# tensorboy/centerpose

Hardware: AMD Instinct MI355X
Metric: images/sec end-to-end (backbone+decode), DLA-34 512x512 (higher is better)
Workload: dtype f32

## Files before the change

### centerpose_amd/csrc/common.h

```cpp
#pragma once
#include <hip/hip_runtime.h>
#include <stdint.h>

#define CP_WAVE 64

extern "C" const char* cp_last_error(void);
void cp_set_error(const char* fmt, ...);
void cp_note_kernel(const char* fmt, ...);

#define CP_CHECK_ARG(cond, ...)              \
    do {                                     \
        if (!(cond)) {                       \
            cp_set_error(__VA_ARGS__);       \
            return 1;                        \
        }                                    \
    } while (0)

#define CP_CHECK_LAUNCH(name)                                                   \
    do {                                                                        \
        hipError_t e_ = hipGetLastError();                                      \
        if (e_ != hipSuccess) {                                                 \
            cp_set_error("%s: kernel launch failed: %s", name, hipGetErrorString(e_)); \
            return 2;                                                           \
        }                                                                       \
    } while (0)

typedef float f32x4 __attribute__((ext_vector_type(4)));
typedef float f32x16 __attribute__((ext_vector_type(16)));

static inline int cp_cdiv(int a, int b) { return (a + b - 1) / b; }

#include <mutex>
struct CpLdsGuard {
    std::mutex mu;
    int have[16] = {};
    hipError_t ensure(const void* kernel, int bytes) {
        int d = 0;
        (void)hipGetDevice(&d);
        std::lock_guard<std::mutex> lock(mu);
        if (have[d & 15] >= bytes) return hipSuccess;
        const hipError_t e = hipFuncSetAttribute(kernel, hipFuncAttributeMaxDynamicSharedMemorySize, bytes);
        if (e == hipSuccess) have[d & 15] = bytes;
        return e;
    }
};

static inline int cp_num_cus()
{
    static std::mutex mu;
    static int cus[16] = {};
    int d = 0;
    (void)hipGetDevice(&d);
    std::lock_guard<std::mutex> lock(mu);
    int& n = cus[d & 15];
    if (n <= 0 && (hipDeviceGetAttribute(&n, hipDeviceAttributeMultiprocessorCount, d) != hipSuccess || n <= 0)) n = 256;
    return n;
}

#define CP_ACT_NONE_ 0
#define CP_ACT_RELU_ 1
#define CP_ACT_SIGMOID_ 2
#define CP_ACT_HSWISH_ 3
#define CP_ACT_HSIGMOID_ 4
__device__ __forceinline__ float cp_relu(float v)
{
    float r;
    asm("v_max_f32 %0, 0, %1" : "=v"(r) : "v"(v));
    return r;
}
typedef float cp_v2f __attribute__((ext_vector_type(2)));
__device__ __forceinline__ float4 cp_scale_shift4(float4 v, float4 sc, float4 sh)
{
    const cp_v2f lo = __builtin_elementwise_fma((cp_v2f){v.x, v.y}, (cp_v2f){sc.x, sc.y}, (cp_v2f){sh.x, sh.y});
    const cp_v2f hi = __builtin_elementwise_fma((cp_v2f){v.z, v.w}, (cp_v2f){sc.z, sc.w}, (cp_v2f){sh.z, sh.w});
    return make_float4(lo.x, lo.y, hi.x, hi.y);
}
__device__ __forceinline__ float4 cp_relu4(float4 v) { return make_float4(cp_relu(v.x), cp_relu(v.y), cp_relu(v.z), cp_relu(v.w)); }

__device__ __forceinline__ float cp_act(float v, int act)
{
    if (act == CP_ACT_RELU_) return cp_relu(v);
    if (act == CP_ACT_SIGMOID_) return 1.0f / (1.0f + __expf(-v));
    if (act == CP_ACT_HSWISH_) return v * fminf(fmaxf(v + 3.f, 0.f), 6.f) / 6.f;
    if (act == CP_ACT_HSIGMOID_) return fminf(fmaxf(v + 3.f, 0.f), 6.f) / 6.f;
    return v;
}
```

### centerpose_amd/csrc/dcn.hip

```cpp
#include <cstdlib>
#include "igemm.h"

#define DCN_MAX_TAPS 121
typedef float dcn_v2 __attribute__((ext_vector_type(2)));

__device__ __forceinline__ void dcn_blend(dcn_v2& r, dcn_v2 wxy, dcn_v2 wzw, dcn_v2 c00, dcn_v2 c01, dcn_v2 c10, dcn_v2 c11)
{
    asm("v_pk_mul_f32 %0, %1, %2 op_sel_hi:[0,1]" : "=v"(r) : "v"(wxy), "v"(c00));
    asm("v_pk_fma_f32 %0, %1, %2, %0 op_sel:[1,0,0] op_sel_hi:[1,1,1]" : "+v"(r) : "v"(wxy), "v"(c01));
    asm("v_pk_fma_f32 %0, %1, %2, %0 op_sel_hi:[0,1,1]" : "+v"(r) : "v"(wzw), "v"(c10));
    asm("v_pk_fma_f32 %0, %1, %2, %0 op_sel:[1,0,0] op_sel_hi:[1,1,1]" : "+v"(r) : "v"(wzw), "v"(c11));
}

template <int BM, int BN, int WAVES_M, int WAVES_N, int MF>
__global__ __launch_bounds__(IG_THREADS, 3) void dcn_igemm_kernel(const ConvArgs a)
{
    using T = IgTile<BM, BN, WAVES_M, WAVES_N, MF>;
    constexpr int QL = 4;
    constexpr int PPP = IG_THREADS / QL;
    constexpr int ASL = BM / PPP;
    static_assert(ASL >= 1, "BM too small for this gather width");
    extern __shared__ __attribute__((aligned(16))) float smem[];
    const int dg = a.dg;
    const int ntap = a.kh * a.kw;
    float4* s_w = reinterpret_cast<float4*>(smem);
    int* s_code = reinterpret_cast<int*>(s_w + dg * ntap * BM);
    float* As0 = smem + dg * ntap * BM * 5;
    float* Bs0 = As0 + 2 * T::A_FLOATS;

    const int tid = threadIdx.x, lane = tid & 63, wid = tid >> 6;
    const int NT = a.ldw / BN;
    int tile = ig_xcd_remap(blockIdx.x, gridDim.x);
    const int S = a.ksplit, sp = tile % S;
    tile /= S;
    const int nt = tile % NT, mt = tile / NT;
    const int m0 = mt * BM, n0 = nt * BN;
    const int wm0 = (wid / WAVES_N) * T::WM, wn0 = (wid % WAVES_N) * T::WN;
    const int HoWo = a.Ho * a.Wo;
    const int tap0 = sp * ntap / S, tap1 = (sp + 1) * ntap / S;
    const int C = a.srcC[0], ld = a.srcLd[0];
    const float* __restrict__ x = a.src[0];

    {
        static_assert(IG_THREADS % BM == 0, "one pixel per thread");
        constexpr int TS = IG_THREADS / BM;
        const int pl = tid % BM, m = m0 + pl;
        const bool live = m < a.M;
        const int b = live ? m / HoWo : 0, p = m - b * HoWo, oy = p / a.Wo, ox = p - oy * a.Wo;
        const float* omp = a.om + (size_t)(live ? m : 0) * a.omLd;
        const int by = oy * a.sy - a.py, bx = ox * a.sx - a.px, bpix = b * a.H * a.W;
        const float fH = (float)a.H, fW = (float)a.W;
        const unsigned ld4 = (unsigned)ld >> 2;
        for (int g = 0; g < dg; ++g) {
        const int og = g * ntap;
        int t = tap0 + __builtin_amdgcn_readfirstlane(tid / BM);
        int ky = t / a.kw, kx = t - ky * a.kw;
        for (; t < tap1; t += TS) {
            const float offh = omp[2 * (og + t)], offw = omp[2 * (og + t) + 1];
            float mk = omp[a.omMaskOff + og + t];
            if (a.omSigmoid) mk = __builtin_amdgcn_rcpf(1.0f + __expf(-mk));
            const float h_im = (float)(by + ky * a.dily) + offh;
            const float w_im = (float)(bx + kx * a.dilx) + offw;
            const bool valid = live && h_im > -1.f && w_im > -1.f && h_im < fH && w_im < fW;
            const float hf = floorf(h_im), wf = floorf(w_im);
            const float lh = h_im - hf, lw = w_im - wf, hh = 1.f - lh, hw = 1.f - lw;
            const int h_low = (int)hf, w_low = (int)wf;
            const bool t_ok = h_low >= 0, b_ok = h_low < a.H - 1, l_ok = w_low >= 0, r_ok = w_low < a.W - 1;
            const bool dyb = t_ok && b_ok, dxb = l_ok && r_ok;
            const float mv = valid ? mk : 0.f;
            const float top = (t_ok ? hh : lh) * mv, bot = (dyb ? lh : 0.f) * mv;
            const float lft = l_ok ? hw : lw, rgt = dxb ? lw : 0.f;
            const int yl = min(max(h_low, 0), a.H - 1), xl = min(max(w_low, 0), a.W - 1);
            s_w[(g * ntap + t) * BM + pl] = make_float4(top * lft, top * rgt, bot * lft, bot * rgt);
            s_code[(g * ntap + t) * BM + pl] = (int)((unsigned)(bpix + yl * a.W + xl) * ld4) | ((dxb ? 1 : 0) << 29) | ((dyb ? 1 : 0) << 30);
            kx += TS;
            while (kx >= a.kw) { kx -= a.kw; ++ky; }
        }
        }
    }

    typename IgAcc<MF>::type acc[T::TM][T::TN];
#pragma unroll
    for (int i = 0; i < T::TM; ++i)
#pragma unroll
        for (int j = 0; j < T::TN; ++j)
#pragma unroll
            for (int r = 0; r < IgAcc<MF>::N; ++r) acc[i][j][r] = 0.f;

    const int ks0 = tap0 * (C / IG_BK), nk = tap1 * (C / IG_BK);
    const int q = tid % QL;
    float4 br[T::B_SLOTS];
    float4 c00[ASL], c01[ASL], c10[ASL], c11[ASL], wq[ASL];
    int tap = tap0, cl = 0;
    const int cpg = C / dg;
    int gnext = 0, grec = 0;
    __syncthreads();

    const unsigned pixb = (unsigned)ld * 4u, rowb = (unsigned)a.W * pixb;
    unsigned o00[ASL], o01[ASL], o10[ASL], o11[ASL];
    auto load_a = [&]() __attribute__((always_inline)) {
        if (cl == gnext) {
            grec = (cl == 0 ? 0 : grec + ntap);
            gnext = cl + cpg;
#pragma unroll
            for (int s = 0; s < ASL; ++s) {
                const int pl = tid / QL + s * PPP;
                const int code = s_code[(grec + tap) * BM + pl];
                wq[s] = s_w[(grec + tap) * BM + pl];
                o00[s] = (((unsigned)code & 0x0FFFFFFFu) << 4) + (unsigned)q * 16u;
                o01[s] = o00[s] + (((unsigned)code >> 29) & 1u) * pixb;
                o10[s] = o00[s] + (((unsigned)code >> 30) & 1u) * rowb;
                o11[s] = o10[s] + (o01[s] - o00[s]);
            }
        }
        const char* xs = reinterpret_cast<const char*>(x) + (size_t)cl * 4;
#pragma unroll
        for (int s = 0; s < ASL; ++s) {
            c00[s] = ig_ldg4(reinterpret_cast<const float*>(xs + o00[s]));
            c01[s] = ig_ldg4(reinterpret_cast<const float*>(xs + o01[s]));
            c10[s] = ig_ldg4(reinterpret_cast<const float*>(xs + o10[s]));
            c11[s] = ig_ldg4(reinterpret_cast<const float*>(xs + o11[s]));
        }
    };
    auto advance = [&]() __attribute__((always_inline)) { cl += IG_BK; if (cl >= C) { cl = 0; gnext = 0; ++tap; } };
    auto store_a = [&](float* As) __attribute__((always_inline)) {
#pragma unroll
        for (int s = 0; s < ASL; ++s) {
            const int pl = tid / QL + s * PPP;
            const float4 w = wq[s];
            const dcn_v2 wxy = {w.x, w.y}, wzw = {w.z, w.w};
            dcn_v2 lo, hi;
            dcn_blend(lo, wxy, wzw, (dcn_v2){c00[s].x, c00[s].y}, (dcn_v2){c01[s].x, c01[s].y}, (dcn_v2){c10[s].x, c10[s].y}, (dcn_v2){c11[s].x, c11[s].y});
            dcn_blend(hi, wxy, wzw, (dcn_v2){c00[s].z, c00[s].w}, (dcn_v2){c01[s].z, c01[s].w}, (dcn_v2){c10[s].z, c10[s].w}, (dcn_v2){c11[s].z, c11[s].w});
            *reinterpret_cast<float4*>(As + pl * IG_LDK + q * 4) = make_float4(lo.x, lo.y, hi.x, hi.y);
        }
    };

    unsigned boff[T::B_SLOTS];
#pragma unroll
    for (int s = 0; s < T::B_SLOTS; ++s) {
        const int idx = tid + s * IG_THREADS;
        boff[s] = ((unsigned)(n0 + (idx >> 2)) * (unsigned)a.K + (unsigned)(idx & 3) * 4u) * 4u;
    }
    auto load_b = [&](int ks) __attribute__((always_inline)) {
        const char* wb = reinterpret_cast<const char*>(a.w) + (size_t)ks * (IG_BK * 4);
#pragma unroll
        for (int s = 0; s < T::B_SLOTS; ++s)
            if (T::B_F4 % IG_THREADS == 0 || tid + s * IG_THREADS < T::B_F4) br[s] = ig_ldg4(reinterpret_cast<const float*>(wb + boff[s]));
    };
    load_a(); advance();
    load_b(ks0);
    store_a(As0);
    ig_store_b<T>(Bs0, tid, br);
    __syncthreads();
    int cur = 0;
    for (int ks = ks0; ks < nk; ++ks) {
        const bool more = ks + 1 < nk;
        ig_compute<T, MF>(As0 + cur * T::A_FLOATS, Bs0 + cur * T::B_FLOATS, wm0, wn0, lane, acc, [&]() __attribute__((always_inline)) {
            if (more) { load_a(); advance(); load_b(ks + 1); }
        });
        __builtin_amdgcn_sched_barrier(0);
        if (more) {
            store_a(As0 + (cur ^ 1) * T::A_FLOATS);
            ig_store_b<T>(Bs0 + (cur ^ 1) * T::B_FLOATS, tid, br);
        }
        __syncthreads();
        cur ^= 1;
    }
    if (S > 1) {
        ConvArgs e = a;
        e.out = a.out + (size_t)sp * a.M * a.outLd;
        ig_epilogue<T, BM, BN, MF>(e, smem, m0, n0, wm0, wn0, lane, tid, acc);
    } else ig_epilogue<T, BM, BN, MF>(a, smem, m0, n0, wm0, wn0, lane, tid, acc);
}


template <int BM, int BN, int WAVES_M, int WAVES_N, int MF>
static int launch_dcn(const ConvArgs& a, hipStream_t s)
{
    using T = IgTile<BM, BN, WAVES_M, WAVES_N, MF>;
    auto kern = dcn_igemm_kernel<BM, BN, WAVES_M, WAVES_N, MF>;
    if (a.srcC[0] % IG_BK != 0) { cp_set_error("dcn: C=%d is not a multiple of %d", a.srcC[0], IG_BK); return 1; }
    if (a.ldw % BN != 0) { cp_set_error("dcn: ldw=%d is not a multiple of the N tile %d", a.ldw, BN); return 1; }
    if ((a.srcC[0] / a.dg) % IG_BK != 0) { cp_set_error("dcn: C / deformable_group = %d is not a multiple of %d", a.srcC[0] / a.dg, IG_BK); return 1; }
    const int main_bytes = T::MAIN_BYTES + a.dg * a.kh * a.kw * BM * 20;
    if (main_bytes > 160 * 1024) { cp_set_error("dcn: %d x %d taps x %d deformable group(s) need %d B of LDS for the sampling records", a.kh, a.kw, a.dg, main_bytes); return 1; }
    const int epi = a.outNCHW ? T::EPI_BYTES : T::EPV_BYTES;
    const int smem = epi > main_bytes ? epi : main_bytes;
    static CpLdsGuard guard;
    if (smem > 64 * 1024) {
        const hipError_t e = guard.ensure((const void*)kern, smem);
        if (e != hipSuccess) { cp_set_error("dcn_v2: cannot reserve %d B LDS: %s", smem, hipGetErrorString(e)); return 2; }
    }
    const int grid = cp_cdiv(a.M, BM) * (a.ldw / BN) * a.ksplit;
    hipLaunchKernelGGL(kern, dim3(grid), dim3(IG_THREADS), smem, s, a);
    cp_note_kernel("dcn_igemm_kernel<%d, %d, %d, %d, %d>", BM, BN, WAVES_M, WAVES_N, MF);
    return 0;
}

struct cp_dcn_desc {
    int B, H, W, C, srcLd;
    int Ho, Wo;
    int kh, kw, sy, sx, py, px, dily, dilx;
    int K, ldw, Cout;
    int omLd, omSigmoid;
    int outLd, outNCHW, act;
    int tile;
    int ksplit;
    int dg;
};

extern "C" int cp_sizeof_dcn_desc(void) { return (int)sizeof(cp_dcn_desc); }

extern "C" int cp_dcn_v2_f32(const cp_dcn_desc* d, const float* x, const float* om, const float* w, const float* scale,
                             const float* shift, float* out, void* stream)
{
    CP_CHECK_ARG(d && x && om && w && scale && shift && out, "dcn_v2: null pointer");
    CP_CHECK_ARG(d->kh > 0 && d->kw > 0 && d->kh * d->kw <= DCN_MAX_TAPS, "dcn_v2: 1..%d taps (kh=%d kw=%d)", DCN_MAX_TAPS, d->kh, d->kw);
    CP_CHECK_ARG(d->sy > 0 && d->sx > 0 && d->dily > 0 && d->dilx > 0 && d->py >= 0 && d->px >= 0, "dcn_v2: stride / dilation > 0, pad >= 0");
    CP_CHECK_ARG(d->C % 16 == 0 && d->srcLd % 4 == 0 && d->srcLd >= d->C, "dcn_v2: C%%16==0, ld%%4==0 required");
    CP_CHECK_ARG(d->K == d->kh * d->kw * d->C, "dcn_v2: K=%d != kh*kw*C", d->K);
    CP_CHECK_ARG(d->ldw % 16 == 0 && d->ldw >= d->Cout, "dcn_v2: ldw=%d Cout=%d", d->ldw, d->Cout);
    const int dgv = d->dg > 1 ? d->dg : 1;
    CP_CHECK_ARG(d->C % dgv == 0 && (d->C / dgv) % 16 == 0, "dcn_v2: C=%d must split into %d deformable groups of a multiple of 16 channels", d->C, dgv);
    CP_CHECK_ARG(d->omLd >= 3 * dgv * d->kh * d->kw, "dcn_v2: omLd=%d too small", d->omLd);
    CP_CHECK_ARG((long long)d->B * d->H * d->W < (1ll << 29) && (long long)d->B * d->H * d->W * d->srcLd * 4 < (1ll << 32),
                 "dcn_v2: input too large (pixel index 29 bits, byte offsets 32 bits)");
    ConvArgs a;
    for (int i = 0; i < IG_MAX_SRC; ++i) { a.src[i] = nullptr; a.srcC[i] = 0; a.srcLd[i] = 0; }
    a.src[0] = x; a.srcC[0] = d->C; a.srcLd[0] = d->srcLd; a.nsrc = 1; a.Ctot = d->C;
    a.B = d->B; a.H = d->H; a.W = d->W; a.Ho = d->Ho; a.Wo = d->Wo; a.M = d->B * d->Ho * d->Wo;
    a.kh = d->kh; a.kw = d->kw; a.sy = d->sy; a.sx = d->sx; a.py = d->py; a.px = d->px;
    a.K = d->K; a.w = w; a.ldw = d->ldw; a.scale = scale; a.shift = shift; a.res = nullptr; a.resLd = 0;
    a.out = out; a.outLd = d->outLd; a.Cout = d->Cout; a.outNCHW = d->outNCHW;
    a.OH = d->Ho; a.OW = d->Wo; a.osy = a.osx = 1; a.ooy = a.oox = 0; a.act = d->act;
    a.om = om; a.omLd = d->omLd; a.omMaskOff = 2 * dgv * d->kh * d->kw; a.omSigmoid = d->omSigmoid; a.dg = dgv;
    a.dily = d->dily; a.dilx = d->dilx; a.nsub = 1;
    a.ksplit = d->ksplit > 1 ? d->ksplit : 1;
    CP_CHECK_ARG(a.ksplit <= d->kh * d->kw, "dcn_v2: ksplit=%d exceeds the %d taps", a.ksplit, d->kh * d->kw);
    CP_CHECK_ARG(a.ksplit == 1 || (!d->outNCHW && d->act == CP_ACT_NONE && d->outLd == d->ldw && d->Cout == d->ldw),
                 "dcn_v2: split-K writes raw NHWC partial sums (outLd == Cout == ldw, no activation)");
    hipStream_t s = (hipStream_t)stream;
    int tile = d->tile;
    if (tile == 0) {
        static const int force = getenv("CP_DCN_TILE") ? atoi(getenv("CP_DCN_TILE")) : 0;
        if (force && a.ksplit == 1) tile = force;
    }
    if (tile == 0) {
        if (d->ldw % 64 != 0) tile = (d->ldw % 32 == 0) ? 128032 : 0;
        else {
            tile = 64064;
            if (d->ldw % 128 == 0 && (long long)cp_cdiv(a.M, 64) * (d->ldw / 128) >= 500) tile = 64128;

        }
    }
    int rc = 0;
    switch (tile) {
        case 128032: rc = launch_dcn<128, 32, 4, 1, 32>(a, s); break;
        case 128064: rc = launch_dcn<128, 64, 2, 2, 32>(a, s); break;
        case 64064: rc = launch_dcn<64, 64, 2, 2, 32>(a, s); break;
        case 64032: rc = launch_dcn<64, 32, 4, 1, 16>(a, s); break;
        case 64128: rc = launch_dcn<64, 128, 2, 2, 32>(a, s); break;
        case 6064128: rc = (d->ldw % 128 == 0) ? launch_dcn<64, 128, 2, 2, 32>(a, s) : launch_dcn<64, 64, 2, 2, 32>(a, s); break;
        default: CP_CHECK_ARG(false, "dcn_v2: unsupported tile %d (ldw=%d)", tile, d->ldw);
    }
    if (rc) return rc;
    CP_CHECK_LAUNCH("dcn_igemm_kernel");
    return 0;
}
```

### centerpose_amd/csrc/elementwise.hip

```cpp
#include <cstdlib>
#include "common.h"

#define EW_THREADS 256
static inline int ew_grid(long long n) { long long g = (n + EW_THREADS - 1) / EW_THREADS; return (int)(g > 8192 ? 8192 : (g < 1 ? 1 : g)); }

struct EwRow { int rows, rowElems, C4; unsigned mC4; };
static inline EwRow ew_row(int rows, int Wo, int C4)
{
    EwRow r; r.rows = rows; r.rowElems = Wo * C4; r.C4 = C4;
    r.mC4 = C4 <= 1 ? 0u : (unsigned)(((1ull << 32) + (unsigned)C4 - 1) / (unsigned)C4);
    return r;
}
static inline dim3 ew_row_grid(const EwRow& r)
{
    return dim3((unsigned)((r.rowElems + EW_THREADS - 1) / EW_THREADS), (unsigned)(r.rows > 65535 ? 65535 : r.rows));
}
__device__ __forceinline__ void ew_split(const EwRow& r, int e, int& x, int& c4)
{
    x = r.C4 == 1 ? e : (int)__umulhi((unsigned)e, r.mC4);
    c4 = e - x * r.C4;
}

__global__ void maxpool_nhwc_kernel(const float* __restrict__ in, int inLd, float* __restrict__ out, int outLd, EwRow r,
                                    int H, int W, int Ho, int Wo, int k, int s, int p)
{
    const int e = blockIdx.x * EW_THREADS + threadIdx.x;
    if (e >= r.rowElems) return;
    int ox, c4;
    ew_split(r, e, ox, c4);
    for (int row = blockIdx.y; row < r.rows; row += gridDim.y) {
        const int b = row / Ho, oy = row - b * Ho;
        float4 m = make_float4(-INFINITY, -INFINITY, -INFINITY, -INFINITY);
        for (int ky = 0; ky < k; ++ky) {
            const int iy = oy * s - p + ky;
            if (iy < 0 || iy >= H) continue;
            for (int kx = 0; kx < k; ++kx) {
                const int ix = ox * s - p + kx;
                if (ix < 0 || ix >= W) continue;
                const float4 v = *reinterpret_cast<const float4*>(in + ((size_t)(b * H + iy) * W + ix) * inLd + c4 * 4);
                m.x = fmaxf(m.x, v.x); m.y = fmaxf(m.y, v.y); m.z = fmaxf(m.z, v.z); m.w = fmaxf(m.w, v.w);
            }
        }
        *reinterpret_cast<float4*>(out + ((size_t)row * Wo + ox) * outLd + c4 * 4) = m;
    }
}

extern "C" int cp_maxpool2d_nhwc_f32(const float* in, int inLd, float* out, int outLd, int B, int H, int W, int C, int k,
                                     int s, int p, void* stream)
{
    CP_CHECK_ARG(in && out && C % 4 == 0 && inLd % 4 == 0 && outLd % 4 == 0, "maxpool: C, ld must be multiples of 4");
    const int Ho = (H + 2 * p - k) / s + 1, Wo = (W + 2 * p - k) / s + 1;
    CP_CHECK_ARG((long long)Wo * (C / 4) * (C / 4) < (1ll << 32) && (long long)B * Ho < (1ll << 31), "maxpool: row too large");
    const EwRow r = ew_row(B * Ho, Wo, C / 4);
    hipLaunchKernelGGL(maxpool_nhwc_kernel, ew_row_grid(r), dim3(EW_THREADS), 0, (hipStream_t)stream, in, inLd, out, outLd, r,
                       H, W, Ho, Wo, k, s, p);
    cp_note_kernel("maxpool_nhwc_kernel");
    CP_CHECK_LAUNCH("maxpool_nhwc_kernel");
    return 0;
}

__global__ void dw_deconv_add_kernel(const float* __restrict__ in, int inLd, const float* __restrict__ w,
                                     const float* add, int addLd, float* out, int outLd, EwRow r,
                                     int H, int W, int f, int p)
{
    const int k = 2 * f, Ho = H * f, Wo = W * f, C = r.C4 * 4;
    const int e = blockIdx.x * EW_THREADS + threadIdx.x;
    if (e >= r.rowElems) return;
    int ox, c4;
    ew_split(r, e, ox, c4);
    const int rx = (ox + p) % f;
    for (int row = blockIdx.y; row < r.rows; row += gridDim.y) {
        const int b = row / Ho, oy = row - b * Ho;
        float4 acc = make_float4(0.f, 0.f, 0.f, 0.f);
        const int ry = (oy + p) % f;
#pragma unroll
        for (int ty = 0; ty < 2; ++ty) {
            const int ky = ry + ty * f, iy = (oy + p - ky) / f;
            if (oy + p - ky < 0 || iy >= H) continue;
#pragma unroll
            for (int tx = 0; tx < 2; ++tx) {
                const int kx = rx + tx * f, ix = (ox + p - kx) / f;
                if (ox + p - kx < 0 || ix >= W) continue;
                const float4 v = *reinterpret_cast<const float4*>(in + ((size_t)(b * H + iy) * W + ix) * inLd + c4 * 4);
                const float4 ww = *reinterpret_cast<const float4*>(w + (size_t)(ky * k + kx) * C + c4 * 4);
                acc.x += v.x * ww.x; acc.y += v.y * ww.y; acc.z += v.z * ww.z; acc.w += v.w * ww.w;
            }
        }
        const size_t opix = (size_t)row * Wo + ox;
        if (add) {
            const float4 rr = *reinterpret_cast<const float4*>(add + opix * addLd + c4 * 4);
            acc.x += rr.x; acc.y += rr.y; acc.z += rr.z; acc.w += rr.w;
        }
        *reinterpret_cast<float4*>(out + opix * outLd + c4 * 4) = acc;
    }
}

__global__ __launch_bounds__(EW_THREADS) void dw_deconv2_add_kernel(const float* __restrict__ in, int inLd, const float* __restrict__ w,
                                                                   const float* add, int addLd, float* out,
                                                                   int outLd, EwRow r, int H, int W)
{
    const int C = r.C4 * 4, Wo = 2 * W;
    const int e = blockIdx.x * EW_THREADS + threadIdx.x;
    if (e >= r.rowElems) return;
    int ix, c4;
    ew_split(r, e, ix, c4);
    float4 wt[16];
#pragma unroll
    for (int t = 0; t < 16; ++t) wt[t] = *reinterpret_cast<const float4*>(w + (size_t)t * C + c4 * 4);
    const bool lok = ix > 0, rok = ix + 1 < W;
    const float4 z = make_float4(0.f, 0.f, 0.f, 0.f);
    for (int row = blockIdx.y; row < r.rows; row += gridDim.y) {
        const int b = row / H, iy = row - b * H;
        const float* base = in + ((size_t)row * W + ix) * inLd + c4 * 4;
        const bool tok = iy > 0, bok = iy + 1 < H;
        const size_t rs = (size_t)W * inLd;
        float4 v[3][3];
#pragma unroll
        for (int dy = -1; dy <= 1; ++dy) {
            const bool yok = dy == 0 || (dy < 0 ? tok : bok);
#pragma unroll
            for (int dx = -1; dx <= 1; ++dx) {
                const bool ok = yok && (dx == 0 || (dx < 0 ? lok : rok));
                v[dy + 1][dx + 1] = ok ? *reinterpret_cast<const float4*>(base + dy * (long long)rs + dx * inLd) : z;
            }
        }
#pragma unroll
        for (int a = 0; a < 2; ++a)
#pragma unroll
            for (int bq = 0; bq < 2; ++bq) {
                float4 acc = z;
#pragma unroll
                for (int ty = 0; ty < 2; ++ty) {
                    const int ky = (a == 0 ? 1 : 0) + 2 * ty, dy = a == 0 ? -ty : 1 - ty;
#pragma unroll
                    for (int tx = 0; tx < 2; ++tx) {
                        const int kx = (bq == 0 ? 1 : 0) + 2 * tx, dx = bq == 0 ? -tx : 1 - tx;
                        const float4 vv = v[dy + 1][dx + 1], ww = wt[ky * 4 + kx];
                        acc.x += vv.x * ww.x; acc.y += vv.y * ww.y; acc.z += vv.z * ww.z; acc.w += vv.w * ww.w;
                    }
                }
                const size_t opix = ((size_t)(b * 2 * H + 2 * iy + a)) * Wo + 2 * ix + bq;
                if (add) {
                    const float4 rr = *reinterpret_cast<const float4*>(add + opix * addLd + c4 * 4);
                    acc.x += rr.x; acc.y += rr.y; acc.z += rr.z; acc.w += rr.w;
                }
                *reinterpret_cast<float4*>(out + opix * outLd + c4 * 4) = acc;
            }
    }
}

extern "C" int cp_dw_deconv_add_nhwc_f32(const float* in, int inLd, const float* w, const float* add, int addLd, float* out,
                                         int outLd, int B, int H, int W, int C, int f, void* stream)
{
    CP_CHECK_ARG(in && w && out && C % 4 == 0 && inLd % 4 == 0 && outLd % 4 == 0 && (!add || addLd % 4 == 0),
                 "dw_deconv_add: C, ld must be multiples of 4");
    CP_CHECK_ARG(f >= 1, "dw_deconv_add: f=%d", f);
    CP_CHECK_ARG((long long)W * f * (C / 4) * (C / 4) < (1ll << 32) && (long long)B * H * f < (1ll << 31), "dw_deconv_add: row too large");
    const char* sw = getenv("CP_DWDECONV2");
    if (f == 2 && !(sw && sw[0] == '0') && (long long)W * (C / 4) * (C / 4) < (1ll << 32)) {
        const EwRow r2 = ew_row(B * H, W, C / 4);
        hipLaunchKernelGGL(dw_deconv2_add_kernel, ew_row_grid(r2), dim3(EW_THREADS), 0, (hipStream_t)stream, in, inLd, w, add, addLd, out,
                           outLd, r2, H, W);
        cp_note_kernel("dw_deconv2_add_kernel");
        CP_CHECK_LAUNCH("dw_deconv2_add_kernel");
        return 0;
    }
    const EwRow r = ew_row(B * H * f, W * f, C / 4);
    hipLaunchKernelGGL(dw_deconv_add_kernel, ew_row_grid(r), dim3(EW_THREADS), 0, (hipStream_t)stream, in, inLd, w, add,
                       addLd, out, outLd, r, H, W, f, f / 2);
    cp_note_kernel("dw_deconv_add_kernel");
    CP_CHECK_LAUNCH("dw_deconv_add_kernel");
    return 0;
}

__global__ void splitk_reduce_kernel(const float* __restrict__ ws, int S, long long slice, int ldw4, const float* __restrict__ scale,
                                     const float* __restrict__ shift, int act, float* __restrict__ out, int outLd, int Cout, long long total4)
{
    const long long i = (long long)blockIdx.x * EW_THREADS + threadIdx.x;
    if (i >= total4) return;
    const long long m = i / ldw4;
    const int n = (int)(i - m * ldw4) * 4;
    if (n >= Cout) return;
    float4 acc = *reinterpret_cast<const float4*>(ws + i * 4);
    for (int s = 1; s < S; ++s) {
        const float4 v = *reinterpret_cast<const float4*>(ws + (size_t)s * slice + i * 4);
        acc.x += v.x; acc.y += v.y; acc.z += v.z; acc.w += v.w;
    }
    const float4 sc = *reinterpret_cast<const float4*>(scale + n), sh = *reinterpret_cast<const float4*>(shift + n);
    acc.x = cp_act(acc.x * sc.x + sh.x, act); acc.y = cp_act(acc.y * sc.y + sh.y, act);
    acc.z = cp_act(acc.z * sc.z + sh.z, act); acc.w = cp_act(acc.w * sc.w + sh.w, act);
    *reinterpret_cast<float4*>(out + (size_t)m * outLd + n) = acc;
}

extern "C" int cp_splitk_reduce_f32(const float* ws, int splits, int M, int ldw, const float* scale, const float* shift, int act, float* out,
                                    int outLd, int Cout, void* stream)
{
    CP_CHECK_ARG(ws && scale && shift && out && splits >= 1 && M > 0, "splitk_reduce: bad arguments");
    CP_CHECK_ARG(ldw % 4 == 0 && Cout % 4 == 0 && outLd % 4 == 0 && Cout <= ldw && Cout <= outLd, "splitk_reduce: ldw, Cout, outLd must be multiples of 4 (ldw=%d Cout=%d outLd=%d)", ldw, Cout, outLd);
    const long long total4 = (long long)M * (ldw / 4);
    hipLaunchKernelGGL(splitk_reduce_kernel, dim3((unsigned)((total4 + EW_THREADS - 1) / EW_THREADS)), dim3(EW_THREADS), 0, (hipStream_t)stream,
                       ws, splits, (long long)M * ldw, ldw / 4, scale, shift, act, out, outLd, Cout, total4);
    cp_note_kernel("splitk_reduce_kernel");
    CP_CHECK_LAUNCH("splitk_reduce_kernel");
    return 0;
}

struct SumUpArgs { const float* src[4]; int ld[4]; int sh[4]; int n; };
__global__ void sum_up_kernel(SumUpArgs a, float* __restrict__ out, int outLd, EwRow r, int H, int W, int relu)
{
    const int e = blockIdx.x * EW_THREADS + threadIdx.x;
    if (e >= r.rowElems) return;
    int x, c4;
    ew_split(r, e, x, c4);
    for (int row = blockIdx.y; row < r.rows; row += gridDim.y) {
        const int b = row / H, y = row - b * H;
        float4 acc = make_float4(0.f, 0.f, 0.f, 0.f);
        for (int j = 0; j < a.n; ++j) {
            const int sh = a.sh[j], hs = H >> sh, ws = W >> sh;
            const float4 v = *reinterpret_cast<const float4*>(a.src[j] + ((size_t)(b * hs + (y >> sh)) * ws + (x >> sh)) * a.ld[j] + c4 * 4);
            if (j == 0) acc = v;
            else { acc.x += v.x; acc.y += v.y; acc.z += v.z; acc.w += v.w; }
        }
        if (relu) { acc.x = fmaxf(acc.x, 0.f); acc.y = fmaxf(acc.y, 0.f); acc.z = fmaxf(acc.z, 0.f); acc.w = fmaxf(acc.w, 0.f); }
        *reinterpret_cast<float4*>(out + ((size_t)row * W + x) * outLd + c4 * 4) = acc;
    }
}

extern "C" int cp_sum_up_nhwc_f32(int n, const float* const* src, const int* ld, const int* shift, float* out, int outLd,
                                  int B, int H, int W, int C, int relu, void* stream)
{
    CP_CHECK_ARG(n >= 1 && n <= 4 && src && ld && shift && out && C % 4 == 0, "sum_up: bad arguments");
    SumUpArgs a;
    for (int i = 0; i < 4; ++i) { a.src[i] = i < n ? src[i] : nullptr; a.ld[i] = i < n ? ld[i] : 0; a.sh[i] = i < n ? shift[i] : 0; }
    a.n = n;
    CP_CHECK_ARG((long long)W * (C / 4) * (C / 4) < (1ll << 32) && (long long)B * H < (1ll << 31), "sum_up: row too large");
    const EwRow r = ew_row(B * H, W, C / 4);
    hipLaunchKernelGGL(sum_up_kernel, ew_row_grid(r), dim3(EW_THREADS), 0, (hipStream_t)stream, a, out, outLd, r, H, W, relu);
    cp_note_kernel("sum_up_kernel");
    CP_CHECK_LAUNCH("sum_up_kernel");
    return 0;
}

struct SumUpMember { SumUpArgs a; float* out; int outLd; EwRow r; int H, W, xblocks; };
struct SumUpGroup { SumUpMember m[4]; int first[5]; int n, relu; };
__global__ void sum_up_group_kernel(const SumUpGroup g)
{
    int t = blockIdx.x, k = 0;
    while (k + 1 < g.n && t >= g.first[k + 1]) ++k;
    const SumUpMember& m = g.m[k];
    t -= g.first[k];
    const int row = t / m.xblocks, e = (t - row * m.xblocks) * EW_THREADS + threadIdx.x;
    if (e >= m.r.rowElems) return;
    int x, c4;
    ew_split(m.r, e, x, c4);
    const int H = m.H, W = m.W;
    const int b = row / H, y = row - b * H;
    float4 acc = make_float4(0.f, 0.f, 0.f, 0.f);
    for (int j = 0; j < m.a.n; ++j) {
        const int sh = m.a.sh[j], hs = H >> sh, ws = W >> sh;
        const float4 v = *reinterpret_cast<const float4*>(m.a.src[j] + ((size_t)(b * hs + (y >> sh)) * ws + (x >> sh)) * m.a.ld[j] + c4 * 4);
        if (j == 0) acc = v;
        else { acc.x += v.x; acc.y += v.y; acc.z += v.z; acc.w += v.w; }
    }
    if (g.relu) { acc.x = fmaxf(acc.x, 0.f); acc.y = fmaxf(acc.y, 0.f); acc.z = fmaxf(acc.z, 0.f); acc.w = fmaxf(acc.w, 0.f); }
    *reinterpret_cast<float4*>(m.out + ((size_t)row * W + x) * m.outLd + c4 * 4) = acc;
}

extern "C" int cp_sum_up_group_nhwc_f32(int n, const float* const* src, const int* meta, float* const* out, int relu, void* stream)
{
    CP_CHECK_ARG(n >= 1 && n <= 4 && src && meta && out, "sum_up_group: 1..4 members (got %d)", n);
    SumUpGroup g;
    g.n = n; g.relu = relu;
    long long total = 0;
    for (int k = 0; k < 4; ++k) {
        const int kk = k < n ? k : 0;
        const int* mt = meta + 14 * kk;
        SumUpMember& m = g.m[k];
        const int ns = mt[0], B = mt[10], H = mt[11], W = mt[12], C = mt[13];
        if (k < n) {
            CP_CHECK_ARG(ns >= 1 && ns <= 4 && out[k] && C > 0 && C % 4 == 0 && mt[9] % 4 == 0, "sum_up_group: member %d: bad arguments", k);
            CP_CHECK_ARG((long long)W * (C / 4) * (C / 4) < (1ll << 32) && (long long)B * H < (1ll << 31), "sum_up_group: member %d: row too large", k);
        }
        for (int i = 0; i < 4; ++i) {
            m.a.src[i] = i < ns ? src[4 * kk + i] : nullptr; m.a.ld[i] = i < ns ? mt[1 + i] : 0; m.a.sh[i] = i < ns ? mt[5 + i] : 0;
            if (k < n && i < ns) CP_CHECK_ARG(m.a.src[i] && m.a.ld[i] % 4 == 0, "sum_up_group: member %d source %d", k, i);
        }
        m.a.n = ns;
        m.out = out[kk]; m.outLd = mt[9]; m.H = H; m.W = W;
        m.r = ew_row(B * H, W, C / 4);
        m.xblocks = (m.r.rowElems + EW_THREADS - 1) / EW_THREADS;
        g.first[k] = (int)total;
        if (k < n) total += (long long)m.r.rows * m.xblocks;
    }
    g.first[4] = (int)total;
    for (int k = n; k < 4; ++k) g.first[k] = (int)total;
    CP_CHECK_ARG(total > 0 && total < (1ll << 31), "sum_up_group: grid %lld", total);
    hipLaunchKernelGGL(sum_up_group_kernel, dim3((unsigned)total), dim3(EW_THREADS), 0, (hipStream_t)stream, g);
    cp_note_kernel("sum_up_group_kernel");
    CP_CHECK_LAUNCH("sum_up_group_kernel");
    return 0;
}

__global__ void nchw_to_nhwc_kernel(const float* __restrict__ in, float* __restrict__ out, int C, int HW, int outLd, int cOff)
{
    __shared__ float t[32][33];
    const int b = blockIdx.z, c0 = blockIdx.y * 32, p0 = blockIdx.x * 32;
    const int tx = threadIdx.x & 31, ty = threadIdx.x >> 5;
    for (int r = ty; r < 32; r += 8) {
        const int c = c0 + r, p = p0 + tx;
        t[r][tx] = (c < C && p < HW) ? in[((size_t)b * C + c) * HW + p] : 0.f;
    }
    __syncthreads();
    for (int r = ty; r < 32; r += 8) {
        const int p = p0 + r, c = c0 + tx;
        if (c < C && p < HW) out[((size_t)b * HW + p) * outLd + cOff + c] = t[tx][r];
    }
}
__global__ void nhwc_to_nchw_kernel(const float* __restrict__ in, int inLd, int cOff, float* __restrict__ out, int C, int HW)
{
    __shared__ float t[32][33];
    const int b = blockIdx.z, c0 = blockIdx.y * 32, p0 = blockIdx.x * 32;
    const int tx = threadIdx.x & 31, ty = threadIdx.x >> 5;
    for (int r = ty; r < 32; r += 8) {
        const int p = p0 + r, c = c0 + tx;
        t[r][tx] = (c < C && p < HW) ? in[((size_t)b * HW + p) * inLd + cOff + c] : 0.f;
    }
    __syncthreads();
    for (int r = ty; r < 32; r += 8) {
        const int c = c0 + r, p = p0 + tx;
        if (c < C && p < HW) out[((size_t)b * C + c) * HW + p] = t[tx][r];
    }
}

extern "C" int cp_nchw_to_nhwc_f32(const float* in, float* out, int B, int C, int H, int W, int outLd, int cOff, void* stream)
{
    CP_CHECK_ARG(in && out && outLd >= cOff + C, "nchw_to_nhwc: bad arguments");
    const int HW = H * W;
    hipLaunchKernelGGL(nchw_to_nhwc_kernel, dim3(cp_cdiv(HW, 32), cp_cdiv(C, 32), B), dim3(256), 0, (hipStream_t)stream, in, out,
                       C, HW, outLd, cOff);
    CP_CHECK_LAUNCH("nchw_to_nhwc_kernel");
    return 0;
}
extern "C" int cp_nhwc_to_nchw_f32(const float* in, int inLd, int cOff, float* out, int B, int C, int H, int W, void* stream)
{
// ... 213 lines not shown
```

### centerpose_amd/csrc/igemm.h

```cpp
#pragma once
#include "common.h"

#define IG_BK 16
#define IG_LDK 20
#define IG_THREADS 256
#define IG_MAX_SRC 4

enum { CP_ACT_NONE = 0, CP_ACT_RELU = 1, CP_ACT_SIGMOID = 2 };

struct ConvArgs {
    const float* src[IG_MAX_SRC];
    int srcC[IG_MAX_SRC];
    int srcLd[IG_MAX_SRC];
    int nsrc, Ctot;
    int B, H, W;
    int Ho, Wo, M;
    int kh, kw, sy, sx, py, px;
    int K;
    const float* w;
    int ldw;
    const float* scale;
    const float* shift;
    const float* res;
    int resLd;
    float* out;
    int outLd;
    int Cout;
    int outNCHW;
    int OH, OW;
    int osy, osx, ooy, oox;
    int act;
    const float* om;
    int omLd;
    int omMaskOff;
    int omSigmoid;
    int dily, dilx;
    int ksplit;
    int dg;
    int nsub;
};

int cp_launch_conv3x3_patch(const ConvArgs& a, int in_nchw, hipStream_t s, int variant = 0);
int cp_launch_stem3x3(const ConvArgs& a, hipStream_t s);
int cp_launch_conv3x3_c16(const ConvArgs& a, int in_nchw, hipStream_t s);
int cp_launch_conv3x3_wino(const ConvArgs& a, hipStream_t s, int variant = 0);
int cp_launch_conv3x3_wino24_group(const ConvArgs* a, int n, hipStream_t s);
int cp_launch_head3x3_1x1_w24(const ConvArgs& a, const float* w2, const float* b2, float* out2, int n2, int ld2, int act2, hipStream_t s);
int cp_launch_conv3x3_wino24(const ConvArgs& a, hipStream_t s);
int cp_launch_head3x3_1x1(const ConvArgs& a, const float* w2, const float* b2, float* out2, int n2, int ld2, int act2, hipStream_t s);

int cp_launch_conv_pointwise(const ConvArgs& a, hipStream_t s);
int cp_launch_conv_bf16x3(const ConvArgs& a, int tile, hipStream_t s);

typedef float ig_v4f __attribute__((ext_vector_type(4)));
__device__ __forceinline__ float4 ig_ldg4(const float* p)
{
    const ig_v4f v = *(const __attribute__((address_space(1))) ig_v4f*)(p);
    return make_float4(v.x, v.y, v.z, v.w);
}

__device__ __forceinline__ int ig_xcd_remap(int id, int n)
{
    const int q = n >> 3, r = n & 7, x = id & 7, j = id >> 3;
    return (x < r ? x * (q + 1) : r * (q + 1) + (x - r) * q) + j;
}

template <int MF> struct IgAcc;
template <> struct IgAcc<32> { typedef f32x16 type; static constexpr int N = 16; };
template <> struct IgAcc<16> { typedef f32x4 type; static constexpr int N = 4; };

template <int MF>
__device__ __forceinline__ typename IgAcc<MF>::type ig_mfma(float a, float b, typename IgAcc<MF>::type c)
{
    if constexpr (MF == 32) return __builtin_amdgcn_mfma_f32_32x32x2f32(a, b, c, 0, 0, 0);
    else return __builtin_amdgcn_mfma_f32_16x16x4f32(a, b, c, 0, 0, 0);
}

template <int MF> __device__ __forceinline__ int ig_row(int r, int lane)
{
    if constexpr (MF == 32) return (r & 3) + 8 * (r >> 2) + 4 * (lane >> 5);
    else return (lane >> 4) * 4 + r;
}

template <int BM, int BN, int WAVES_M, int WAVES_N, int MF>
struct IgTile {
    static constexpr int WM = BM / WAVES_M, WN = BN / WAVES_N;
    static constexpr int TM = WM / MF, TN = WN / MF;
    static constexpr int A_SLOTS = BM * 4 / IG_THREADS;
    static constexpr int B_F4 = BN * 4;
    static constexpr int B_SLOTS = (B_F4 + IG_THREADS - 1) / IG_THREADS;
    static constexpr int A_FLOATS = BM * IG_LDK, B_FLOATS = BN * IG_LDK;
    static constexpr int MAIN_BYTES = 2 * (A_FLOATS + B_FLOATS) * 4;
    static constexpr int EPI_BYTES = BN * (BM + 1) * 4;
    static constexpr int EPV_BYTES = BM * (BN + 4) * 4;
    static constexpr int NHWC_BYTES = MAIN_BYTES > EPV_BYTES ? MAIN_BYTES : EPV_BYTES;
    static constexpr int SMEM = MAIN_BYTES > EPI_BYTES ? MAIN_BYTES : EPI_BYTES;
    static_assert(WAVES_M * WAVES_N * 64 == IG_THREADS, "4 waves");
    static_assert(TM >= 1 && TN >= 1, "tile");
    static_assert(A_SLOTS >= 1, "BM >= 64");
};

template <class T>
__device__ __forceinline__ void ig_load_b(const ConvArgs& a, int k0, int n0, int tid, float4 (&br)[T::B_SLOTS], const float* w = nullptr)
{
    if (!w) w = a.w;
#pragma unroll
    for (int s = 0; s < T::B_SLOTS; ++s) {
        const int idx = tid + s * IG_THREADS;
        if constexpr (T::B_F4 % IG_THREADS == 0) br[s] = ig_ldg4(w + (size_t)(n0 + (idx >> 2)) * a.K + k0 + (idx & 3) * 4);
        else if (idx < T::B_F4) br[s] = ig_ldg4(w + (size_t)(n0 + (idx >> 2)) * a.K + k0 + (idx & 3) * 4);
    }
}
template <class T>
__device__ __forceinline__ void ig_store_b(float* Bs, int tid, const float4 (&br)[T::B_SLOTS])
{
#pragma unroll
    for (int s = 0; s < T::B_SLOTS; ++s) {
        const int idx = tid + s * IG_THREADS;
        if (T::B_F4 % IG_THREADS == 0 || idx < T::B_F4) *reinterpret_cast<float4*>(Bs + (idx >> 2) * IG_LDK + (idx & 3) * 4) = br[s];
    }
}

template <class T, int MF, class F>
__device__ __forceinline__ void ig_compute(const float* As, const float* Bs, int wm0, int wn0, int lane,
                                           typename IgAcc<MF>::type (&acc)[T::TM][T::TN], F&& mid)
{
    constexpr int G = 64 / MF;
    constexpr int NH = IG_BK / (4 * G);
    const int g = lane / MF, il = lane % MF;
    float4 af[NH][T::TM], bf[NH][T::TN];
#pragma unroll
    for (int h = 0; h < NH; ++h) {
#pragma unroll
        for (int i = 0; i < T::TM; ++i)
            af[h][i] = *reinterpret_cast<const float4*>(As + (wm0 + i * MF + il) * IG_LDK + h * 4 * G + g * 4);
#pragma unroll
        for (int j = 0; j < T::TN; ++j)
            bf[h][j] = *reinterpret_cast<const float4*>(Bs + (wn0 + j * MF + il) * IG_LDK + h * 4 * G + g * 4);
    }
    constexpr int HALF = NH * T::TM * T::TN / 2;
    __builtin_amdgcn_sched_barrier(0);
#pragma unroll
    for (int h = 0; h < NH; ++h) {
#pragma unroll
        for (int i = 0; i < T::TM; ++i)
#pragma unroll
            for (int j = 0; j < T::TN; ++j) {
                if ((h * T::TM + i) * T::TN + j == HALF) {
                    __builtin_amdgcn_sched_barrier(0);
                    mid();
                    __builtin_amdgcn_sched_barrier(0);
                }
                acc[i][j] = ig_mfma<MF>(af[h][i].x, bf[h][j].x, acc[i][j]);
                acc[i][j] = ig_mfma<MF>(af[h][i].y, bf[h][j].y, acc[i][j]);
                acc[i][j] = ig_mfma<MF>(af[h][i].z, bf[h][j].z, acc[i][j]);
                acc[i][j] = ig_mfma<MF>(af[h][i].w, bf[h][j].w, acc[i][j]);
            }
    }
}

template <class T, int MF>
__device__ __forceinline__ void ig_compute(const float* As, const float* Bs, int wm0, int wn0, int lane,
                                           typename IgAcc<MF>::type (&acc)[T::TM][T::TN])
{
    ig_compute<T, MF>(As, Bs, wm0, wn0, lane, acc, [] {});
}

__device__ __forceinline__ float ig_act(float v, int act) { return cp_act(v, act); }

template <class T, int BM, int BN, int MF>
__device__ __forceinline__ void ig_epilogue(const ConvArgs& a, float* smem, int m0, int n0, int wm0, int wn0,
                                            int lane, int tid, typename IgAcc<MF>::type (&acc)[T::TM][T::TN],
                                            int ooy_add = 0, int oox_add = 0)
{
    const int HoWo = a.Ho * a.Wo;
    const int ooy = a.ooy + ooy_add, oox = a.oox + oox_add;
    const int cl = lane & (MF - 1);
    const bool vec_ok = !a.outNCHW && ((a.outLd | a.Cout) & 3) == 0 && (((size_t)a.out) & 15) == 0 &&
                        (!a.res || ((a.resLd & 3) == 0 && (((size_t)a.res) & 15) == 0));
    if (vec_ok) {
        const bool dense = (a.osy == 1 && a.osx == 1 && ooy == 0 && oox == 0 && a.OH == a.Ho && a.OW == a.Wo);
        const bool relu = a.act == CP_ACT_RELU, sigm = a.act == CP_ACT_SIGMOID;
        float* Cs = smem;
        constexpr int LDC = BN + 4;
        __syncthreads();
#pragma unroll
        for (int i = 0; i < T::TM; ++i)
#pragma unroll
            for (int j = 0; j < T::TN; ++j)
#pragma unroll
                for (int r = 0; r < IgAcc<MF>::N; ++r)
                    Cs[(wm0 + i * MF + ig_row<MF>(r, lane)) * LDC + wn0 + j * MF + cl] = acc[i][j][r];
// ... 83 lines not shown
```

### centerpose_amd/csrc/plan_runtime.cpp

```cpp
#include <cstdio>
#include <cstring>
#include <memory>
#include <string>
#include <vector>
#include "common.h"

extern "C" {
struct cp_conv_desc;
struct cp_dcn_desc;
int cp_abi_version(void);
int cp_conv2d_f32(const cp_conv_desc*, const float* const*, const float*, const float*, const float*, const float*, float*, void*);
int cp_conv3x3_winograd_f32(const cp_conv_desc*, const float*, const float*, const float*, const float*, const float*, float*, void*);
int cp_dcn_v2_f32(const cp_dcn_desc*, const float*, const float*, const float*, const float*, const float*, float*, void*);
int cp_conv3x3_winograd24_group_f32(const cp_conv_desc*, int, const float* const*, const float* const*, const float* const*, const float* const*,
                                    const float* const*, float* const*, void*);
int cp_conv2d_group_f32(const cp_conv_desc*, int, const float* const*, const float* const*, const float* const*, const float* const*,
                        const float* const*, float* const*, void*);
int cp_stem7x7_f32(const float*, const float*, const float*, const float*, float*, int, int, int, int, int, int, int, void*);
int cp_maxpool2d_nhwc_f32(const float*, int, float*, int, int, int, int, int, int, int, int, void*);
int cp_dw_deconv_add_nhwc_f32(const float*, int, const float*, const float*, int, float*, int, int, int, int, int, int, void*);
int cp_sum_up_nhwc_f32(int, const float* const*, const int*, const int*, float*, int, int, int, int, int, int, void*);
int cp_sum_up_group_nhwc_f32(int, const float* const*, const int*, float* const*, int, void*);
int cp_head3x3_1x1_f32(const cp_conv_desc*, const float*, const float*, const float*, const float*, const float*, const float*, float*, int,
                       int, int, void*);
int cp_dwconv2d_nhwc_f32(const float*, int, const float*, const float*, const float*, float*, int, int, int, int, int, int, int, int, int, void*);
int cp_global_avgpool_nhwc_f32(const float*, int, float*, int, int, int, int, void*);
int cp_scale_add_nhwc_f32(const float*, int, const float*, int, const float*, int, float*, int, int, int, int, int, void*);
int cp_shuffle_concat_nhwc_f32(const float*, int, const float*, int, float*, int, long long, int, int, void*);
int cp_multi_pose_decode_f32(const float*, const float*, const float*, const float*, const float*, const float*, int, int, int, int,
                             int, int, float*, float*, int*, void*);
int cp_splitk_reduce_f32(const float*, int, int, int, const float*, const float*, int, float*, int, int, void*);
int cp_sizeof_conv_desc(void);
int cp_sizeof_dcn_desc(void);
int cp_decode_topk_f32(const float*, const float*, int, int, int, int, int, int, float*, int*, void*);
int cp_decode_assign_f32(const float*, const float*, const float*, const float*, const float*, const int*, int, int, int, int, int, float*,
                         void*);
int cp_head_points_f32(const float*, int, const int*, const float*, const float*, const float*, const float*, float*, int, int, int, int, int,
                       int, int, void*);
int cp_flip_merge_pairs_f32(int, const float* const*, float* const*, const int*, int, int, int, int, const int*, void*);
}

namespace {

enum { FN_CONV = 1, FN_WINO = 2, FN_DCN = 3, FN_STEM7 = 4, FN_POOL = 5, FN_UPADD = 6, FN_SUMUP = 7, FN_DWCONV = 8, FN_AVGPOOL = 9,
       FN_SCALEADD = 10, FN_SHUFFLE = 11, FN_HEAD = 12, FN_TOPK = 13, FN_ASSIGN = 14, FN_SPLITK = 15, FN_WINO24G = 16, FN_CONVG = 17, FN_SUMUPG = 18,
       FN_POINTS = 19, FN_FLIPPAIRS = 20 };
enum { REF_NULL = 0, REF_BUF = 1, REF_CONST = 2 };

struct Op {
    uint32_t fn = 0, out_index = 0, stream = 0;
    std::vector<unsigned char> desc;
    std::vector<float*> ptrs;
    std::vector<int> bufid;
    std::vector<int> ints;
};

struct Out { float* p; int shape[4]; int bufid; };

struct ConstPool {
    std::vector<float*> p;
    ~ConstPool() { for (float* q : p) if (q) (void)hipFree(q); }
};

}

struct cp_plan {
    int B = 0, H = 0, W = 0;
    std::vector<float*> bufs;
    std::vector<uint64_t> buf_numel;
    std::shared_ptr<ConstPool> cpool;
    float* input = nullptr;
    int input_buf = -1;
    std::vector<Out> outs;
    std::vector<Op> ops;
    bool use_graph = false, warmed = false;
    hipGraph_t graph = nullptr;
    hipGraphExec_t exec = nullptr;
    hipStream_t cap_stream = nullptr, side_stream = nullptr;
    float* ws_scores = nullptr;
    int* ws_inds = nullptr;
    int ws_K = 0;
};

namespace {

struct Reader {
    const unsigned char* b;
    size_t n, p = 0;
    bool ok = true;
    bool take(void* dst, size_t k) {
        if (p + k > n) { ok = false; return false; }
        memcpy(dst, b + p, k);
        p += k;
        return true;
    }
    uint32_t u32() { uint32_t v = 0; take(&v, 4); return v; }
    uint64_t u64() { uint64_t v = 0; take(&v, 8); return v; }
    void skip_pad8() { p += (8 - (p & 7)) & 7; }
};

struct Ref { uint32_t kind, id; uint64_t off, numel; };

int run_op(const Op& o, hipStream_t s)
{
    const std::vector<float*>& P = o.ptrs;
    const int* I = o.ints.data();
    switch (o.fn) {
        case FN_CONV:
            return cp_conv2d_f32(reinterpret_cast<const cp_conv_desc*>(o.desc.data()), reinterpret_cast<const float* const*>(P.data()), P[4],
                                 P[5], P[6], P[7], P[8], s);
        case FN_WINO:
            return cp_conv3x3_winograd_f32(reinterpret_cast<const cp_conv_desc*>(o.desc.data()), P[0], P[1], P[2], P[3], P[4], P[5], s);
        case FN_DCN:
            return cp_dcn_v2_f32(reinterpret_cast<const cp_dcn_desc*>(o.desc.data()), P[0], P[1], P[2], P[3], P[4], P[5], s);
        case FN_WINO24G:
            return cp_conv3x3_winograd24_group_f32(reinterpret_cast<const cp_conv_desc*>(o.desc.data()), I[0], reinterpret_cast<const float* const*>(P.data()),
                                                   reinterpret_cast<const float* const*>(P.data() + 4), reinterpret_cast<const float* const*>(P.data() + 8),
                                                   reinterpret_cast<const float* const*>(P.data() + 12), reinterpret_cast<const float* const*>(P.data() + 16),
                                                   reinterpret_cast<float* const*>(P.data() + 20), s);
        case FN_CONVG:
            return cp_conv2d_group_f32(reinterpret_cast<const cp_conv_desc*>(o.desc.data()), I[0], reinterpret_cast<const float* const*>(P.data()),
                                       reinterpret_cast<const float* const*>(P.data() + 8), reinterpret_cast<const float* const*>(P.data() + 16),
                                       reinterpret_cast<const float* const*>(P.data() + 24), reinterpret_cast<const float* const*>(P.data() + 32),
                                       reinterpret_cast<float* const*>(P.data() + 40), s);
        case FN_STEM7:
            return cp_stem7x7_f32(P[0], P[1], P[2], P[3], P[4], I[0], I[1], I[2], I[3], I[4], I[5], I[6], s);
        case FN_POOL:
            return cp_maxpool2d_nhwc_f32(P[0], I[0], P[1], I[1], I[2], I[3], I[4], I[5], I[6], I[7], I[8], s);
        case FN_UPADD:
            return cp_dw_deconv_add_nhwc_f32(P[0], I[0], P[1], P[2], I[1], P[3], I[2], I[3], I[4], I[5], I[6], I[7], s);
        case FN_SUMUP:
            return cp_sum_up_nhwc_f32(I[0], reinterpret_cast<const float* const*>(P.data()), I + 1, I + 5, P[4], I[9], I[10], I[11], I[12],
                                      I[13], I[14], s);
        case FN_SUMUPG:
            return cp_sum_up_group_nhwc_f32(I[0], reinterpret_cast<const float* const*>(P.data()), I + 2, reinterpret_cast<float* const*>(P.data() + 16), I[1], s);
        case FN_HEAD:
            return cp_head3x3_1x1_f32(reinterpret_cast<const cp_conv_desc*>(o.desc.data()), P[0], P[1], P[2], P[3], P[4], P[5], P[6], I[0], I[1],
                                      I[2], s);
        case FN_DWCONV:
            return cp_dwconv2d_nhwc_f32(P[0], I[0], P[1], P[2], P[3], P[4], I[1], I[2], I[3], I[4], I[5], I[6], I[7], I[8], I[9], s);
        case FN_AVGPOOL:
            return cp_global_avgpool_nhwc_f32(P[0], I[0], P[1], I[1], I[2], I[3], I[4], s);
        case FN_SCALEADD:
            return cp_scale_add_nhwc_f32(P[0], I[0], P[1], I[1], P[2], I[2], P[3], I[3], I[4], I[5], I[6], I[7], s);
        case FN_SHUFFLE:
            return cp_shuffle_concat_nhwc_f32(P[0], I[0], P[1], I[1], P[2], I[2], (long long)I[3], I[4], I[5], s);
        case FN_SPLITK:
            return cp_splitk_reduce_f32(P[0], I[0], I[1], I[2], P[1], P[2], I[3], P[3], I[4], I[5], s);
        case FN_TOPK:
            return cp_decode_topk_f32(P[0], P[1], I[0], I[1], I[2], I[3], I[4], I[5], P[2], reinterpret_cast<int*>(P[3]), s);
        case FN_ASSIGN:
            return cp_decode_assign_f32(P[0], P[1], P[2], P[3], P[4], reinterpret_cast<const int*>(P[5]), I[0], I[1], I[2], I[3], I[4], P[6], s);
        case FN_POINTS:
            return cp_head_points_f32(P[0], I[0], reinterpret_cast<const int*>(P[1]), P[2], P[3], P[4], P[5], P[6], I[1], I[2], I[3], I[4], I[5],
                                      I[6], I[7], s);
        case FN_FLIPPAIRS:
            return cp_flip_merge_pairs_f32(I[0], reinterpret_cast<const float* const*>(P.data()), reinterpret_cast<float* const*>(P.data() + 4), I + 5,
                                           I[1], I[2], I[3], I[4], reinterpret_cast<const int*>(P[8]), s);
    }
    cp_set_error("plan: unknown launch function %u", o.fn);
    return 1;
}

bool arity_ok(const Op& o)
{
    switch (o.fn) {
        case FN_CONV: return o.ptrs.size() == 9 && (int)o.desc.size() == cp_sizeof_conv_desc();
        case FN_WINO: return o.ptrs.size() == 6 && (int)o.desc.size() == cp_sizeof_conv_desc();
        case FN_DCN: return o.ptrs.size() == 6 && (int)o.desc.size() == cp_sizeof_dcn_desc();
        case FN_WINO24G: return o.ptrs.size() == 25 && o.ints.size() == 1 && o.ints[0] >= 1 && o.ints[0] <= 4 && (int)o.desc.size() == 4 * cp_sizeof_conv_desc();
        case FN_CONVG: return o.ptrs.size() == 49 && o.ints.size() == 1 && o.ints[0] >= 1 && o.ints[0] <= 8 && (int)o.desc.size() == 8 * cp_sizeof_conv_desc();
        case FN_STEM7: return o.ptrs.size() == 5 && o.ints.size() == 7;
        case FN_POOL: return o.ptrs.size() == 2 && o.ints.size() == 9;
        case FN_UPADD: return o.ptrs.size() == 4 && o.ints.size() == 8;
        case FN_SUMUP: return o.ptrs.size() == 5 && o.ints.size() == 15;
        case FN_SUMUPG: return o.ptrs.size() == 21 && o.ints.size() == 58 && o.ints[0] >= 1 && o.ints[0] <= 4;
        case FN_HEAD: return o.ptrs.size() == 7 && o.ints.size() == 3 && (int)o.desc.size() == cp_sizeof_conv_desc();
        case FN_DWCONV: return o.ptrs.size() == 5 && o.ints.size() == 10;
        case FN_AVGPOOL: return o.ptrs.size() == 2 && o.ints.size() == 5;
        case FN_SCALEADD: return o.ptrs.size() == 4 && o.ints.size() == 8;
        case FN_SHUFFLE: return o.ptrs.size() == 3 && o.ints.size() == 6;
        case FN_SPLITK: return o.ptrs.size() == 4 && o.ints.size() == 6;
        case FN_TOPK: return o.ptrs.size() == 4 && o.ints.size() == 6;
        case FN_ASSIGN: return o.ptrs.size() == 7 && o.ints.size() == 5;
        case FN_POINTS: return o.ptrs.size() == 7 && o.ints.size() == 8;
        case FN_FLIPPAIRS: return o.ptrs.size() == 10 && o.ints.size() == 13 && o.ints[0] >= 1 && o.ints[0] <= 4;
    }
    return false;
}

int run_all(cp_plan* pl, hipStream_t s)
{
    for (const Op& o : pl->ops)
        if (int rc = run_op(o, s)) return rc;
    return 0;
}

struct SchedOp { const Op* op; int stream; int buf_base; };

int run_schedule(const std::vector<SchedOp>& ops, size_t nb, hipStream_t main, hipStream_t side, std::vector<hipEvent_t>& ev)
{
    const size_t n = ops.size();
    std::vector<int> last_writer(nb, -1);
    std::vector<std::vector<int>> readers(nb);
    hipStream_t st[2] = {main, side};
    int waited[2] = {-1, -1}, tail[2] = {-1, -1};
    ev.assign(n + 1, nullptr);
    if (hipEventCreateWithFlags(&ev[n], hipEventDisableTiming) != hipSuccess || hipEventRecord(ev[n], main) != hipSuccess ||
        hipStreamWaitEvent(side, ev[n], 0) != hipSuccess) { cp_set_error("plan: fork of the side stream failed"); return 2; }
    for (size_t i = 0; i < n; ++i) {
        const Op& o = *ops[i].op;
        const int me = ops[i].stream ? 1 : 0, other = me ^ 1, base = ops[i].buf_base;
        int need = -1;
        auto follow = [&](int j) { if (j >= 0 && (ops[j].stream ? 1 : 0) == other && j > need) need = j; };
        for (size_t k = 0; k < o.ptrs.size(); ++k) {
            if (o.bufid[k] < 0) continue;
            const int b = base + o.bufid[k];
            follow(last_writer[b]);
            if (k == o.out_index) for (int j : readers[b]) follow(j);
        }
        if (need > waited[me]) {
            if (hipStreamWaitEvent(st[me], ev[need], 0) != hipSuccess) { cp_set_error("plan: event wait failed"); return 2; }
            waited[me] = need;
        }
        if (int rc = run_op(o, st[me])) return rc;
        if (hipEventCreateWithFlags(&ev[i], hipEventDisableTiming) != hipSuccess || hipEventRecord(ev[i], st[me]) != hipSuccess) {
            cp_set_error("plan: event record failed");
            return 2;
        }
        tail[me] = (int)i;
        for (size_t k = 0; k < o.ptrs.size(); ++k) {
            if (o.bufid[k] < 0) continue;
            const int b = base + o.bufid[k];
            if (k == o.out_index) { last_writer[b] = (int)i; readers[b].clear(); }
            else readers[b].push_back((int)i);
        }
    }
    if (tail[1] >= 0 && hipStreamWaitEvent(main, ev[tail[1]], 0) != hipSuccess) { cp_set_error("plan: join of the side stream failed"); return 2; }
    return 0;
}

int run_two_streams(cp_plan* pl, hipStream_t main, hipStream_t side, std::vector<hipEvent_t>& ev)
{
    std::vector<SchedOp> ops;
    for (const Op& o : pl->ops) ops.push_back(SchedOp{&o, (int)o.stream, 0});
    return run_schedule(ops, pl->bufs.size(), main, side, ev);
}

void free_plan(cp_plan* pl)
{
    if (!pl) return;
    if (pl->exec) (void)hipGraphExecDestroy(pl->exec);
    if (pl->graph) (void)hipGraphDestroy(pl->graph);
    if (pl->cap_stream) (void)hipStreamDestroy(pl->cap_stream);
    if (pl->side_stream) (void)hipStreamDestroy(pl->side_stream);
    for (float* p : pl->bufs) if (p) (void)hipFree(p);
    pl->cpool.reset();
    if (pl->ws_scores) (void)hipFree(pl->ws_scores);
    if (pl->ws_inds) (void)hipFree(pl->ws_inds);
    delete pl;
}

#define PLAN_FAIL(...)            \
    do {                          \
        cp_set_error(__VA_ARGS__); \
        free_plan(pl);            \
        return 1;                 \
    } while (0)

}

extern "C" uint32_t cp_fnv1a32(const void* data, size_t bytes)
{
    uint32_t h = 2166136261u;
    const unsigned char* p = static_cast<const unsigned char*>(data);
    for (size_t i = 0; i < bytes; ++i) { h ^= p[i]; h *= 16777619u; }
    return h;
}

extern "C" int cp_plan_create(const void* blob, size_t bytes, int use_graph, cp_plan** out)
{
    CP_CHECK_ARG(blob && out, "plan_create: null pointer");
    *out = nullptr;
    Reader r{static_cast<const unsigned char*>(blob), bytes};
    const bool v4 = bytes >= 48 && memcmp(blob, "CPPLAN04", 8) == 0;
    CP_CHECK_ARG(bytes >= 48 && (v4 || memcmp(blob, "CPPLAN03", 8) == 0 || memcmp(blob, "CPPLAN02", 8) == 0),
                 "plan_create: not a centerpose_amd plan (bad magic)");
    r.p = 8;
    const uint32_t abi = r.u32(), B = r.u32(), H = r.u32(), W = r.u32(), nbuf = r.u32(), nconst = r.u32(), nops = r.u32(),
                   nout = r.u32(), mlen = r.u32();
    const uint32_t want_sum = r.u32();
    if (v4) {
        const uint32_t h = cp_fnv1a32(static_cast<const unsigned char*>(blob) + 48, bytes - 48);
        CP_CHECK_ARG(h == want_sum, "plan_create: checksum mismatch (file %08x, computed %08x): truncated or corrupted plan", want_sum, h);
    }
    CP_CHECK_ARG((int)abi == cp_abi_version(), "plan_create: plan was written for ABI %u, library has %d", abi, cp_abi_version());
    CP_CHECK_ARG(nbuf < (1u << 20) && nconst < (1u << 20) && nops < (1u << 20) && nout <= 64 && mlen < bytes,
                 "plan_create: corrupt header");
    r.p += mlen;
    r.skip_pad8();
    cp_plan* pl = new cp_plan();
    pl->B = (int)B; pl->H = (int)H; pl->W = (int)W;
    pl->use_graph = use_graph != 0;
    std::vector<uint64_t>& buf_numel = pl->buf_numel;
    buf_numel.resize(nbuf);
    for (uint32_t i = 0; i < nbuf; ++i) buf_numel[i] = r.u64();
    struct CI { uint64_t numel, off; };
    std::vector<CI> ci(nconst);
    for (uint32_t i = 0; i < nconst; ++i) { ci[i].numel = r.u64(); ci[i].off = r.u64(); }
    if (!r.ok) PLAN_FAIL("plan_create: truncated file (tables)");
    for (uint32_t i = 0; i < nconst; ++i)
        if (ci[i].off > bytes || ci[i].numel * 4 > bytes - ci[i].off) PLAN_FAIL("plan_create: constant %u lies outside the file", i);
    pl->bufs.assign(nbuf, nullptr);
    pl->cpool = std::make_shared<ConstPool>();
    std::vector<float*>& consts = pl->cpool->p;
    consts.assign(nconst, nullptr);
    for (uint32_t i = 0; i < nbuf; ++i) {
        if (hipMalloc((void**)&pl->bufs[i], buf_numel[i] * 4 + 16) != hipSuccess) PLAN_FAIL("plan_create: hipMalloc of %llu floats failed", (unsigned long long)buf_numel[i]);
        (void)hipMemset(pl->bufs[i], 0, buf_numel[i] * 4);
    }
    for (uint32_t i = 0; i < nconst; ++i) {
        if (hipMalloc((void**)&consts[i], ci[i].numel * 4 + 16) != hipSuccess) PLAN_FAIL("plan_create: hipMalloc (constant) failed");
// ... 313 lines not shown
```

### centerpose_amd/engine.py

```python
import os
import warnings
import weakref

import torch

from . import _lib, nets, ops
from .nets import Act


DECODE_TOPK = "decode.nms_topk"
SPARSE_HEADS = ("wh", "hps", "reg", "hp_offset")
FLIP_PEAKS = "flip.merge_peaks"
FLIP_IDX = ((1, 2), (3, 4), (5, 6), (7, 8), (9, 10), (11, 12), (13, 14), (15, 16))


def normalize_state_dict(sd, arch=None):
    out = {}
    for k, v in sd.items():
        if k.startswith("module") and not k.startswith("module_list"):
            k = k[7:]
        out[nets.internal_key(arch, k) if arch is not None else k] = v
    return out


class BufferPool:

    def __init__(self, device, clock=lambda: 0):
        self.device = device
        self.reuse = os.environ.get("CP_BUFFER_REUSE", "1") != "0"
        self.min_age = int(os.environ.get("CP_BUFFER_MIN_AGE", "12"))
        self.clock = clock
        self.free = []
        self.bytes = 0
        self.bytes_requested = 0

    def take(self, numel):
        self.bytes_requested += numel * 4
        if self.reuse:
            now, best = self.clock(), None
            for i, (t, slot) in enumerate(self.free):
                if now - t >= self.min_age and numel <= slot.numel() <= 2 * numel and \
                        (best is None or slot.numel() < self.free[best][1].numel()):
                    best = i
            if best is not None:
                return self.free.pop(best)[1]
        self.bytes += numel * 4
        return torch.empty((numel,), dtype=torch.float32, device=self.device)

    def give(self, slot):
        if self.reuse:
            self.free.append((self.clock(), slot))


class PlanBuilder(nets.Graph):
    def __init__(self, sd, B, device, sigmoid_heads=True, const_cache=None, dets_only=False):
        super().__init__()
        self.dets_only = dets_only
        self.points = None
        self.sd, self.B, self.dev = sd, B, device
        self.const_cache = const_cache if const_cache is not None else {}
        self.pool = BufferPool(device, lambda: len(self.launches))
        if isinstance(sigmoid_heads, bool):
            sigmoid_heads = ("hm", "hm_hp") if sigmoid_heads else ()
        self.sigmoid_heads = tuple(sigmoid_heads)
        self.launches = []
        self.winograd = os.environ.get("CP_WINOGRAD", "1") != "0"
        self.dcn_splitk = os.environ.get("CP_DCN_SPLITK", "1") != "0"
        self.wino_splitc = os.environ.get("CP_WINO_SPLITC", "1") != "0"
        self.conv_splitk = os.environ.get("CP_CONV_SPLITK", "1") != "0"
        self.fuse_heads = os.environ.get("CP_FUSE_HEADS", "1") != "0"
        self._pool_cache = {}
        self.outputs = None

    @property
    def bytes_alloc(self):
        return self.pool.bytes

    def buf(self, H, W, C, split=None):
        Cp = 2 * split[1] if split else ops.round_up(C, 16)
        slot = self.pool.take(self.B * H * W * Cp)
        act = Act(H, W, C, slot[: self.B * H * W * Cp].view(self.B, H, W, Cp), split)
        weakref.finalize(act, self.pool.give, slot)
        return act

    @staticmethod
    def cmap(a):
        if a.split:
            h, hp = a.split
            return list(range(h)) + list(range(hp, hp + h))
        return list(range(a.C))

    def expand_in(self, w, xs):
        if all(a.t.shape[3] == a.C and not a.split for a in xs):
            return w
        out = torch.zeros((w.shape[0], sum(a.t.shape[3] for a in xs)) + tuple(w.shape[2:]), dtype=w.dtype, device=w.device)
        lo = po = 0
        for a in xs:
            idx = torch.tensor(self.cmap(a), device=w.device) + po
            out[:, idx] = w[:, lo:lo + a.C]
            lo, po = lo + a.C, po + a.t.shape[3]
        return out

    def expand_vec(self, v, a, fill=0.0):
        out = torch.full((a.t.shape[3],), fill, dtype=torch.float32, device=v.device)
        out[torch.tensor(self.cmap(a), device=v.device)] = v.float()
        return out

    @staticmethod
    def act_code(relu):
        return {False: ops.ACT_NONE, None: ops.ACT_NONE, True: ops.ACT_RELU, "relu": ops.ACT_RELU, "hswish": ops.ACT_HSWISH,
                "hsigmoid": ops.ACT_HSIGMOID}[relu]

    def w(self, key):
        hit = self.const_cache.get(("w", key))
        if hit is None:
            hit = self.const_cache[("w", key)] = self.sd[key].to(self.dev, torch.float32)
        return hit

    def bn(self, name):
        return tuple(self.w("%s.%s" % (name, s)) for s in ("weight", "bias", "running_mean", "running_var"))

    def wino(self, wp, cin, cout, k=3, stride=1, pad=1, nsrc=1, key=None, hw=None):
        if self.winograd and hw is not None and ops.wino_eligible(cin, k, stride, pad, nsrc) and \
                ops.wino24_wanted(self.B, hw[0], hw[1], cin, cout):
            ck = ("u24", key, cin, cout)
            hit = self.const_cache.get(ck) if key is not None else None
            if hit is None:
                hit = ops.pack_wino24_weight(wp, cin, cout)
                if key is not None:
                    self.const_cache[ck] = hit
            return ("wino24", hit)
        if self.winograd and ops.wino_eligible(cin, k, stride, pad, nsrc):
            ck = ("u", key, cin, cout)
            hit = self.const_cache.get(ck) if key is not None else None
            if hit is None:
                hit = ops.pack_wino_weight(wp, cin, cout)
                if key is not None:
                    self.const_cache[ck] = hit
            return hit
        return None

    def add(self, kind, name, flops, launch):
        self.launches.append((kind, name, flops * self.B, launch))

    def unit_scale(self, n):
        hit = self.const_cache.get(("unit", n))
        if hit is None:
            hit = self.const_cache[("unit", n)] = (torch.ones(n, device=self.dev), torch.zeros(n, device=self.dev))
        return hit

    def add_wino(self, name, flops, x, wp, u, sc, sh, out, cout, act, res=None):
        B, H, W, cin = x.shape
        if isinstance(u, tuple):
            self.add("wino24", name, flops, ops.conv2d_launch([x], wp, sc, sh, out, kh=3, kw=3, stride=1, pad=1, cout=cout, act=act,
                                                              res=res, wino=u[1], tile=ops.WINO24))
            return
        S = ops.wino_ksplit(B, H, W, cin, cout) if (self.wino_splitc and res is None) else 1
        if S > 1:
            ld, M = out.shape[3], B * H * W
            ws = self.pool.take(S * M * ld)
            wst = ws[: S * M * ld].view(S, M, ld)
            ones, zeros = self.unit_scale(sc.numel())
            self.add("wino", name, flops, ops.conv2d_launch([x], wp, ones, zeros, wst, kh=3, kw=3, stride=1, pad=1, cout=cout, wino=u,
                                                            ksplit=S))
            self.add("sum", name + ".splitc", 0, ops.splitk_reduce_launch(wst, sc, sh, out, cout=cout, act=act))
            self.pool.give(ws)
            return
        self.add("wino", name, flops, ops.conv2d_launch([x], wp, sc, sh, out, kh=3, kw=3, stride=1, pad=1, cout=cout, act=act, res=res,
                                                        wino=u))

    def emit_conv(self, xs, conv, bn, bias, co, k, stride, pad, relu, res, stem):
        x = xs[0]
        Ho, Wo = (x.H + 2 * pad - k) // stride + 1, (x.W + 2 * pad - k) // stride + 1
        out = self.buf(Ho, Wo, co)
        if stem and k == 7 and pad == 3 and co in (16, 64) and res is None and bn and relu in (True, False):
            wp7 = ops.pack_stem7_weight(self.w(conv + ".weight"))
            sc7, sh7 = ops.fold_bn(co, self.bn(bn), self.w(conv + ".bias") if bias else None, self.dev)
            self.add("conv", conv, 2 * Ho * Wo * co * 3 * 49, ops.stem7x7_launch(xs[0].t, wp7, sc7, sh7, out.t, stride, relu))
            return out
        w = self.w(conv + ".weight")
        wp = ops.pack_conv_weight(w if stem else self.expand_in(w, xs), stem=stem)
        sc, sh = ops.fold_bn(co, self.bn(bn) if bn else None, self.w(conv + ".bias") if bias else None, self.dev)
        srcs = [a.t for a in xs]
        rt = res.t if res is not None else None
        ci = sum(a.C for a in xs)
        cip = ci if stem else sum(a.t.shape[3] for a in xs)
        u = None if stem else self.wino(wp, cip, co, k, stride, pad, len(xs), key=conv, hw=(x.H, x.W))
        flops = 2 * Ho * Wo * co * ci * k * k
        if u is not None:
            self.add_wino(conv, flops, srcs[0], wp, u, sc, sh, out.t, out.t.shape[3], self.act_code(relu), rt)
            return out
        S = ops.conv_ksplit(ops.rule_batch(self.B) * Ho * Wo, wp.shape[0], wp.shape[1]) \
            if (self.conv_splitk and not stem and len(xs) == 1 and res is None and not (k == 3 and stride == 1 and pad == 1)) else 1
        if S > 1:
            ldw, M = wp.shape[0], self.B * Ho * Wo
            ws = self.pool.take(S * M * ldw)
            wst = ws[: S * M * ldw].view(S, M, ldw)
            ones, zeros = self.unit_scale(ldw)
            self.add("conv", conv, flops, ops.conv2d_launch(srcs, wp, ones, zeros, wst, kh=k, kw=k, stride=stride, pad=pad, cout=ldw, ksplit=S))
            self.add("sum", conv + ".splitk", 0, ops.splitk_reduce_launch(wst, sc, sh, out.t, cout=out.t.shape[3], act=self.act_code(relu)))
            self.pool.give(ws)
            return out
        self.add("conv", conv, flops,
                 ops.conv2d_launch(srcs, wp, sc, sh, out.t, kh=k, kw=k, stride=stride, pad=pad, cout=out.t.shape[3],
                                   act=self.act_code(relu), res=rt, in_nchw=stem))
        return out

    def emit_conv_group(self, members):
        ok = self.winograd and os.environ.get("CP_GROUP", "1") != "0" and os.environ.get("CP_WINO24", "1") != "0" and 2 <= len(members) <= 4 and \
            all(ops.wino_eligible(x.t.shape[3], 3, 1, 1, 1) and not x.split for x, *_ in members)
        if not ok:
            return super().emit_conv_group(members)
        sizes = [self.B * x.H * x.W * ops.round_up(co, 16) for x, _, _, co, _, _ in members]
        slot = self.pool.take(sum(sizes))
        holder = Act(1, 1, 1, slot)
        weakref.finalize(holder, self.pool.give, slot)
        outs, recs, off, flops = [], [], 0, 0
        for (x, conv, bn, co, relu, res), n in zip(members, sizes):
            cp = ops.round_up(co, 16)
            out = Act(x.H, x.W, co, slot[off:off + n].view(self.B, x.H, x.W, cp), parent=holder)
            off += n
            wp = ops.pack_conv_weight(self.expand_in(self.w(conv + ".weight"), [x]))
            sc, sh = ops.fold_bn(co, self.bn(bn), None, self.dev)
            cin = x.t.shape[3]
            ck = ("u24", conv, cin, co)
            u24 = self.const_cache.get(ck)
            if u24 is None:
                u24 = self.const_cache[ck] = ops.pack_wino24_weight(wp, cin, co)
            recs.append(dict(x=x.t, wp=wp, u24=u24, scale=sc, shift=sh, out=out.t, cout=cp, act=self.act_code(relu),
                             res=res.t if res is not None else None))
            flops += 2 * x.H * x.W * co * x.C * 9
            outs.append(out)
        self.add("wino24", "group:" + members[0][1], flops, ops.conv3x3_group_launch(recs, slot[:off]))
        return outs

    def emit_conv_batch(self, members):
        ok = os.environ.get("CP_GROUP", "1") != "0" and os.environ.get("CP_FUSE_GROUP", "1") != "0" and len(members) >= 2 and \
            all(not x.split and x.t.shape[3] % 16 == 0 and not ops.wino_eligible(x.t.shape[3], k, stride, pad, 1) and not (k == 3 and x.t.shape[3] == 16)
                for x, _, _, _, k, stride, pad, _ in members)
        if not ok:
            return super().emit_conv_batch(members)
        outs = []
        for c0 in range(0, len(members), ops.GROUP_MAX):
            chunk = members[c0:c0 + ops.GROUP_MAX]
            if len(chunk) == 1:
                outs += super().emit_conv_batch(chunk)
                continue
            dims = [((x.H + 2 * pad - k) // stride + 1, (x.W + 2 * pad - k) // stride + 1) for x, _, _, _, k, stride, pad, _ in chunk]
            sizes = [self.B * h * w * ops.round_up(m[3], 16) for (h, w), m in zip(dims, chunk)]
            slot = self.pool.take(sum(sizes))
            holder = Act(1, 1, 1, slot)
            weakref.finalize(holder, self.pool.give, slot)
            recs, off, flops = [], 0, 0
            for (x, conv, bn, co, k, stride, pad, relu), (h, w), n in zip(chunk, dims, sizes):
                cp = ops.round_up(co, 16)
                out = Act(h, w, co, slot[off:off + n].view(self.B, h, w, cp), parent=holder)
                off += n
                wp = ops.pack_conv_weight(self.expand_in(self.w(conv + ".weight"), [x]))
                sc, sh = ops.fold_bn(co, self.bn(bn), None, self.dev)
                ldw = ops.round_up(wp.shape[0], 64)
                recs.append(dict(x=x.t, wp=ops.pad_rows(wp, ldw), scale=ops.pad_vec(sc, ldw), shift=ops.pad_vec(sh, ldw), out=out.t, cout=cp,
                                 k=k, stride=stride, pad=pad, act=self.act_code(relu)))
                flops += 2 * h * w * co * x.C * k * k
                outs.append(out)
            self.add("conv", "group:" + chunk[0][1], flops, ops.conv2d_group_launch(recs, slot[:off]))
        return outs

    def emit_maxpool(self, x, k, s, p):
        key = (id(x), k, s, p)
        hit = self._pool_cache.get(key)
        if hit is not None and hit[0]() is x and hit[1]() is not None:
            return hit[1]()
        out = self.buf((x.H + 2 * p - k) // s + 1, (x.W + 2 * p - k) // s + 1, x.C)
        self.add("pool", "maxpool%dx%d" % (k, k), 0, ops.maxpool2d_launch(x.t, out.t, k, s, p))
        self._pool_cache[key] = (weakref.ref(x), weakref.ref(out))
        return out

    def emit_dcn(self, x, conv, bn, co):
        om = self.buf(x.H, x.W, 32)
        wom = ops.pack_conv_weight(self.expand_in(self.w(conv + ".conv_offset_mask.weight"), [x]))
        som, hom = ops.fold_bn(27, None, self.w(conv + ".conv_offset_mask.bias"), self.dev)
        som[27:] = 0.0
        out = self.buf(x.H, x.W, co)
        wp = ops.pack_conv_weight(self.expand_in(self.w(conv + ".weight"), [x]))
        sc, sh = ops.fold_bn(co, self.bn(bn), self.w(conv + ".bias"), self.dev)
        uom = self.wino(wom, x.t.shape[3], 32, key=conv + ".conv_offset_mask", hw=(x.H, x.W))
        if uom is not None:
            self.add_wino(conv + ".conv_offset_mask", 2 * x.H * x.W * 27 * x.C * 9, x.t, wom, uom, som, hom, om.t, 32, ops.ACT_NONE)
        else:
            self.add("conv", conv + ".conv_offset_mask", 2 * x.H * x.W * 27 * x.C * 9,
                     ops.conv2d_launch([x.t], wom, som, hom, om.t, kh=3, kw=3, stride=1, pad=1, cout=32))
        flops = 2 * x.H * x.W * co * x.C * 9
        S = ops.dcn_ksplit(ops.rule_batch(self.B) * x.H * x.W, wp.shape[0]) if self.dcn_splitk else 1
        if S > 1:
            ldw = wp.shape[0]
            ws = self.pool.take(S * self.B * x.H * x.W * ldw)
            wst = ws[: S * self.B * x.H * x.W * ldw].view(S, self.B * x.H * x.W, ldw)
            ones, zeros = self.unit_scale(ldw)
            self.add("dcn", conv, flops, ops.dcn_v2_launch(x.t, om.t, wp, ones, zeros, wst, cout=ldw, om_sigmoid=True, ksplit=S))
            self.add("sum", conv + ".splitk", 0, ops.splitk_reduce_launch(wst, sc, sh, out.t, cout=out.t.shape[3], act=ops.ACT_RELU))
            self.pool.give(ws)
            return out
        self.add("dcn", conv, flops,
                 ops.dcn_v2_launch(x.t, om.t, wp, sc, sh, out.t, cout=out.t.shape[3], om_sigmoid=True, act=ops.ACT_RELU))
        return out

    def emit_up_add(self, x, wname, f, add):
        out = self.buf(x.H * f, x.W * f, x.C)
        wk = ops.pack_dw_deconv_weight(self.w(wname + ".weight"))
        if wk.shape[1] != x.t.shape[3]:
            wk = torch.cat([wk, wk.new_zeros((wk.shape[0], x.t.shape[3] - wk.shape[1]))], 1).contiguous()
        self.add("up", wname, 2 * out.H * out.W * x.C * 4, ops.dw_deconv_add_launch(x.t, wk, add.t, out.t, f))
        return out

    def emit_dwconv(self, x, conv, bn, k, stride, act):
        Ho, Wo = (x.H + 2 * (k // 2) - k) // stride + 1, (x.W + 2 * (k // 2) - k) // stride + 1
        out = self.buf(Ho, Wo, x.C, x.split)
        g, b, mean, var = self.bn(bn)
        scale = g / torch.sqrt(var + ops.BN_EPS)
        shift = b - mean * scale
        wk = ops.pack_dw_weight(self.w(conv + ".weight"))
        wkp = torch.stack([self.expand_vec(row, x) for row in wk], 0).contiguous()
        self.add("dw", conv, 2 * Ho * Wo * x.C * k * k,
                 ops.dwconv2d_launch(x.t, wkp, self.expand_vec(scale, x), self.expand_vec(shift, x), out.t, k, stride, k // 2,
                                     self.act_code(act)))
        return out

    def emit_se(self, x, p, red):
        pooled = self.buf(1, 1, x.C)
        self.add("pool", p + ".0", 0, ops.global_avgpool_launch(x.t, pooled.t))
        mid = self.emit_conv([pooled], p + ".1", p + ".2", False, red, 1, 1, 0, True, None, False)
        return self.emit_conv([mid], p + ".4", p + ".5", False, x.C, 1, 1, 0, "hsigmoid", None, False)

    def emit_scale_add(self, x, se, add):
        out = self.buf(x.H, x.W, x.C)
        self.add("se", "se.scale", 0, ops.scale_add_launch(x.t, se.t, add.t if add is not None else None, out.t))
        return out

    def emit_half(self, x, which):
        h, hp = x.split
        return Act(x.H, x.W, h, x.t[..., which * hp:(which + 1) * hp], parent=x)

    def emit_shuffle(self, x1, x2):
        h = x1.C
        hp = ops.round_up(h, 16)
        out = self.buf(x1.H, x1.W, 2 * h, (h, hp))
        self.add("shuffle", "channel_shuffle", 0, ops.shuffle_concat_launch(x1.t, x2.t, out.t, h, hp))
        return out

    def emit_deconv4(self, x, wname, bn, co):
        out = self.buf(x.H * 2, x.W * 2, co)
        w = self.w(wname + ".weight")
        sc, sh = ops.fold_bn(co, self.bn(bn), None, self.dev)
        H, W = x.H, x.W
        wp = torch.cat([ops.pack_deconv4_subpixel(w, py, px) for py in range(2) for px in range(2)], 0).contiguous()
        self.add("conv", wname, 4 * 2 * H * W * co * x.C * 4,
                 ops.conv2d_launch([x.t], wp, sc, sh, out.t, kh=2, kw=2, stride=1, pad=0, pad_yx=(1, 1), cout=co, act=ops.ACT_RELU,
                                   Ho=H, Wo=W, out_scatter=(2, 2, 0, 0), nsub=4))
        return out

    def emit_sum_up(self, xs, shifts, relu):
        out = self.buf(xs[0].H, xs[0].W, xs[0].C)
        self.add("sum", "fuse", 0, ops.sum_up_launch([a.t for a in xs], shifts, out.t, relu))
        return out

    def emit_sum_up_batch(self, members, relu):
        ok = os.environ.get("CP_GROUP", "1") != "0" and os.environ.get("CP_SUM_GROUP", "1") != "0" and 2 <= len(members) <= 4 and \
            all(len(xs) <= 4 and not any(a.split for a in xs) for xs, _ in members)
        if not ok:
            return super().emit_sum_up_batch(members, relu)
        sizes = [self.B * xs[0].H * xs[0].W * xs[0].t.shape[3] for xs, _ in members]
        slot = self.pool.take(sum(sizes))
        holder = Act(1, 1, 1, slot)
        weakref.finalize(holder, self.pool.give, slot)
        outs, recs, off = [], [], 0
        for (xs, shifts), n in zip(members, sizes):
            out = Act(xs[0].H, xs[0].W, xs[0].C, slot[off:off + n].view(self.B, xs[0].H, xs[0].W, xs[0].t.shape[3]), parent=holder)
            off += n
            recs.append(([a.t for a in xs], shifts, out.t))
            outs.append(out)
        self.add("sum", "group:fuse", 0, ops.sum_up_group_launch(recs, slot[:off], relu))
        return outs

    def emit_head(self, feat, p, hc):
        H, W = feat.H, feat.W
        if self.dets_only:
            self.points = self.head_points_consts(feat, p, hc)
        per_head = ops.rule_batch(self.B) * H * W * hc * 4 <= 300 * (1 << 20) and hc >= 64
        ft = feat.t
        outs = []
        if per_head:
            mid = self.buf(H, W, hc)
        else:
            mid = self.buf(H, W, 6 * hc)
            w3 = self.expand_in(torch.cat([self.w("%s.%s.0.weight" % (p, h)) for h, _ in nets.HEADS], 0), [feat])
            b3 = torch.cat([self.w("%s.%s.0.bias" % (p, h)) for h, _ in nets.HEADS], 0)
            wp3 = ops.pack_conv_weight(w3)
            sc3, sh3 = ops.fold_bn(6 * hc, None, b3, self.dev)
            u3 = self.wino(wp3, feat.t.shape[3], 6 * hc, key=p + ".*.0")
            self.add("wino" if u3 is not None else "conv", p + ".*.0", 2 * H * W * 6 * hc * feat.C * 9,
                     ops.conv2d_launch([ft], wp3, sc3, sh3, mid.t, kh=3, kw=3, stride=1, pad=1, cout=6 * hc, act=ops.ACT_RELU, wino=u3))
        for i, (h, n) in enumerate(nets.HEADS):
            if self.dets_only and h in SPARSE_HEADS:
                outs.append(None)
                continue
            o = torch.empty((self.B, n, H, W), dtype=torch.float32, device=self.dev)
            wp = ops.pack_conv_weight(self.w("%s.%s.2.weight" % (p, h)))
            sc, sh = ops.fold_bn(n, None, self.w("%s.%s.2.bias" % (p, h)), self.dev)
            act = ops.ACT_SIGMOID if h in self.sigmoid_heads else ops.ACT_NONE
            if per_head:
                wp3h = ops.pack_conv_weight(self.expand_in(self.w("%s.%s.0.weight" % (p, h)), [feat]))
                sc3h, sh3h = ops.fold_bn(hc, None, self.w("%s.%s.0.bias" % (p, h)), self.dev)
                fused_ok = self.fuse_heads and ops.head3x3_1x1_eligible(ft, hc, n)
                u3h = self.wino(wp3h, feat.t.shape[3], hc, key="%s.%s.0" % (p, h), hw=None if fused_ok else (H, W))
                if u3h is not None and fused_ok:
                    h24 = ops.head_wino24_wanted(ft, n)
                    if h24:
                        ck = ("u24", "%s.%s.0" % (p, h), feat.t.shape[3], hc)
                        u3h = self.const_cache.get(ck)
                        if u3h is None:
                            u3h = self.const_cache[ck] = ops.pack_wino24_weight(wp3h, feat.t.shape[3], hc)
                    w2 = self.w("%s.%s.2.weight" % (p, h)).reshape(n, hc).contiguous()
                    self.add("wino24" if h24 else "wino", "%s.%s.0+2" % (p, h), 2 * H * W * (hc * feat.C * 9 + n * hc),
                             ops.head3x3_1x1_launch(ft, u3h, sc3h, sh3h, w2, self.w("%s.%s.2.bias" % (p, h)), o, hc=hc, act2=act, wino24=h24))
                    outs.append(o)
                    continue
                if isinstance(u3h, tuple):
                    self.add("wino24", "%s.%s.0" % (p, h), 2 * H * W * hc * feat.C * 9,
                             ops.conv2d_launch([ft], wp3h, sc3h, sh3h, mid.t, kh=3, kw=3, stride=1, pad=1, cout=hc, act=ops.ACT_RELU,
                                               wino=u3h[1], tile=ops.WINO24))
                else:
                    self.add("wino" if u3h is not None else "conv", "%s.%s.0" % (p, h), 2 * H * W * hc * feat.C * 9,
                             ops.conv2d_launch([ft], wp3h, sc3h, sh3h, mid.t, kh=3, kw=3, stride=1, pad=1, cout=hc, act=ops.ACT_RELU,
                                               wino=u3h))
                sl = mid.t
            else:
                sl = mid.t[..., i * hc:(i + 1) * hc]
            self.add("conv", "%s.%s.2" % (p, h), 2 * H * W * n * hc,
                     ops.conv2d_launch([sl], wp, sc, sh, o, kh=1, kw=1, cout=n, act=act, out_nchw=True))
            outs.append(o)
        self.outputs = outs
        return outs

    def head_points_consts(self, feat, p, hc):
        if hc % 32 or hc > 512 or feat.t.shape[3] > 512:
            raise ValueError("dets_only: the points kernel needs head_conv % 32 == 0 and <= 512 (got %d) and <= 512 head input channels" % hc)
        w1 = torch.cat([ops.pack_head_points_weight(self.expand_in(self.w("%s.%s.0.weight" % (p, h)), [feat])) for h in SPARSE_HEADS])
        b1 = torch.cat([self.w("%s.%s.0.bias" % (p, h)).float() for h in SPARSE_HEADS]).contiguous()
        w2 = torch.cat([self.w("%s.%s.2.weight" % (p, h)).reshape(-1, hc).float() for h in SPARSE_HEADS]).contiguous()
        b2 = torch.cat([self.w("%s.%s.2.bias" % (p, h)).float() for h in SPARSE_HEADS]).contiguous()
        return dict(feat=feat, hc=hc, w1=w1, b1=b1, w2=w2, b2=b2)


def list_schedule(deps, durations, nstreams=2, prefer=None):
    n = len(deps)
    assert len(durations) == n and all(all(0 <= j < i for j in d) for i, d in enumerate(deps))
    children = [[] for _ in range(n)]
    for i, d in enumerate(deps):
        for j in d:
            children[j].append(i)
    blevel = [0.0] * n
    for i in reversed(range(n)):
        blevel[i] = durations[i] + max([blevel[c] for c in children[i]], default=0.0)
    indeg = [len(set(d)) for d in deps]
    ready = [i for i in range(n) if indeg[i] == 0]
    free = [0.0] * nstreams
    start, finish, assign = [0.0] * n, [0.0] * n, [0] * n
    for _ in range(n):
        best = None
        for i in ready:
            est = max([finish[j] for j in deps[i]], default=0.0)
            for p in range(nstreams):
                key = (max(est, free[p]), 0 if prefer is not None and prefer[i] else 1, -blevel[i], p)
                if best is None or key < best[0]:
                    best = (key, i, p)
        (t, _, _, _), i, p = best
        ready.remove(i)
        start[i], finish[i], free[p], assign[i] = t, t + durations[i], t + durations[i], p
        for c in set(children[i]):
            indeg[c] -= 1
            if indeg[c] == 0:
                ready.append(c)
    order = sorted(range(n), key=lambda i: (start[i], i))
    return order, assign, (max(finish) if n else 0.0)


def order_is_topological(deps, order):
    n = len(deps)
    if len(order) != n or sorted(order) != list(range(n)):
        return False
    pos = [0] * n
    for p, i in enumerate(order):
        pos[i] = p
    return all(pos[j] < pos[i] for i, d in enumerate(deps) for j in d)


class Engine:

    def __init__(self, arch, state_dict, batch, height=512, width=512, device="cuda", head_conv=None,
                 sigmoid_heads=True, use_graph=True, decode_k=None, const_cache=None, sched_cache=None, dets_only=False,
                 flip_test=False):
        if dets_only and not decode_k:
            raise ValueError("dets_only=True needs decode_k: the sparse heads are evaluated at the peaks of the plan's own decode")
        if flip_test:
            if batch % 2:
                raise ValueError("flip_test=True needs image / mirrored-twin pairs: an even batch [img0, twin0, img1, twin1, ...], got %d"
                                 % batch)
            if not decode_k:
                raise ValueError("flip_test=True needs decode_k: the merged maps exist only inside the plan, for its own decode")
            if dets_only:
                raise ValueError("flip_test=True does not combine with dets_only=True (the flip merge needs the dense maps)")
        if not torch.cuda.is_available():
            raise _lib.CenterposeHipError("Engine needs a HIP device; there is no CPU fallback")
        _lib.lib()
        self.arch = nets.canonical_arch(arch)
        self.B, self.H, self.W = batch, height, width
        self.device = torch.device(device)
        sd = normalize_state_dict(state_dict, self.arch)
        spec, _ = nets.param_spec(self.arch, height, width, head_conv, internal=True)
        missing = [k for k in spec if k not in sd and not k.endswith("num_batches_tracked")]
        if missing:
            raise KeyError("checkpoint is missing %d parameters, e.g. %s" % (len(missing), missing[:3]))
        for k, shp in spec.items():
            if k in sd and not k.endswith("num_batches_tracked") and tuple(sd[k].shape) != tuple(shp):
                raise ValueError("parameter %s has shape %s, expected %s" % (k, tuple(sd[k].shape), shp))
        with torch.cuda.device(self.device):
            self.input = torch.zeros((batch, 3, height, width), dtype=torch.float32, device=self.device)
            pb = PlanBuilder(sd, batch, self.device, sigmoid_heads, const_cache, dets_only=bool(dets_only))
            pb.network(self.arch, Act(height, width, 3, self.input), head_conv)
        self.launches = pb.launches
        self.emission = pb.launches
        self.outputs = pb.outputs
        self.head_maps = pb.outputs
        self.dets_only = bool(dets_only)
        self.flip_test = bool(flip_test)
        self._points = pb.points
        self.flops_per_image = pb.flops
        self.activation_bytes = pb.bytes_alloc
        self.graph = None
        self.sched_cache = sched_cache
        self.capture_mode = None
        self.use_graph = use_graph
        self.dets, self.decode_k = None, None
        if decode_k:
            self._add_decode(int(decode_k), sigmoid_heads)
        self._points = None

    def _add_decode(self, K, sigmoid_heads):
        if sigmoid_heads is not True and set(sigmoid_heads) != {"hm", "hm_hp"}:
            raise ValueError("decode inside the schedule needs the sigmoided hm and hm_hp heads")
        hm, wh, hps, reg, hm_hp, hp_offset = self.outputs
        B, J, H, W = hm.shape[0], hm_hp.shape[1], hm.shape[2], hm.shape[3]
        merges = []
        if self.flip_test:
            hm, wh, hps, reg, hm_hp, hp_offset, merges = self._flip_merges(J)
            B = B // 2
        with torch.cuda.device(self.device):
            ws = torch.zeros((2, B, 1 + J, K), dtype=torch.float32, device=self.device)
            self.dets = torch.zeros((B, K, 5 + 3 * J), dtype=torch.float32, device=self.device)
            if self.dets_only:
                sparse = torch.zeros((B * H * W * (6 + 2 * J),), dtype=torch.float32, device=self.device)
                views, off = [], 0
                for n in (2, 2 * J, 2, 2):
                    views.append(sparse[off:off + B * n * H * W].view(B, n, H, W))
                    off += B * n * H * W
                wh, hps, reg, hp_offset = views
                self.head_maps = [hm, wh, hps, reg, hm_hp, hp_offset]
                self.activation_bytes += 4 * sparse.numel()
        topk, assign = ops.decode_launches(hm, wh, hps, reg, hm_hp, hp_offset, K, ws, self.dets)
        tail = merges[:1] + [("decode", DECODE_TOPK, 0, topk)] + merges[1:]
        if self.dets_only:
            pt = self._points
            hc, C = pt["hc"], pt["feat"].C
            points = ops.head_points_launch(pt["feat"].t, ws[1], pt["w1"], pt["b1"], pt["w2"], pt["b2"], sparse, hc=hc, J=J, K=K)
            flops = K * 2 * (3 * hc * C * 9 + (4 + 2 * J) * hc) + J * K * 2 * (hc * C * 9 + 2 * hc)
            tail.append(("points", "head_points", flops * B, points))
        tail.append(("decode", "decode.pose_assign", 0, assign))
        self.launches = self.emission = self.launches + tail
        self.activation_bytes += 4 * (ws.numel() + self.dets.numel())
        self.decode_k = K

    def _flip_merges(self, J):
        if J != 17:
            raise ValueError("flip_test=True swaps the 17 COCO joints (FLIP_IDX); this plan has %d" % J)
        perm = list(range(J))
        for a, b in FLIP_IDX:
            perm[a], perm[b] = b, a
        modes = ops.FLIP_MODES
        groups = (((0, modes["flip"]), (4, modes["joints"])),
                  ((1, modes["flip"]), (2, modes["offsets"]), (3, modes["copy"]), (5, modes["copy"])))
        merged = [None] * 6
        launches = []
        with torch.cuda.device(self.device):
            permt = torch.tensor(perm, dtype=torch.int32, device=self.device).view(torch.float32)
            for gi, group in enumerate(groups):
                srcs = [self.outputs[i] for i, _ in group]
                N, H, W = srcs[0].shape[0] // 2, srcs[0].shape[2], srcs[0].shape[3]
                whole = torch.zeros((sum(N * s.shape[1] * H * W for s in srcs),), dtype=torch.float32, device=self.device)
                maps, off = [], 0
                for (i, mode), s in zip(group, srcs):
                    n = N * s.shape[1] * H * W
                    merged[i] = whole[off:off + n].view(N, s.shape[1], H, W)
                    maps.append((s, merged[i], mode))
                    off += n
                self.activation_bytes += 4 * whole.numel()
                launches.append(("flip", FLIP_PEAKS if gi == 0 else "flip.merge_regress", 0, ops.flip_pairs_launch(maps, whole, permt)))
        return tuple(merged) + (launches,)

    def process(self, images):
        if self.dets is None:
            raise _lib.CenterposeHipError("this engine was built without decode_k: call forward() and multi_pose_decode()")
        outs = self.forward(images)
        return outs, self.dets

    def save_plan(self, path, deterministic=False):
        from . import plan
        return plan.save_plan(self, path, deterministic)

    @classmethod
    def from_plan(cls, path, device="cuda", use_graph=True):
        from . import plan
        return plan.load_plan(path, device=device, use_graph=use_graph)

    def run_eager(self):
        for _, _, _, launch in self.launches:
            launch.run()

    def dependencies(self, launches=None):
        deps = []
        last_writer, readers = {}, {}
        for i, (_, _, _, launch) in enumerate(self.launches if launches is None else launches):
            rd = {t.untyped_storage().data_ptr() for t in launch.reads}
            wr = {launch.out.untyped_storage().data_ptr()}
            d = set()
            for k in rd:
                if k in last_writer:
                    d.add(last_writer[k])
            for k in wr:
                if k in last_writer:
                    d.add(last_writer[k])
                d.update(readers.get(k, ()))
            d.discard(i)
            for k in rd:
                readers.setdefault(k, []).append(i)
            for k in wr:
                last_writer[k] = i
                readers[k] = []
            deps.append(sorted(d))
        return deps

    def schedule(self, durations=None, nstreams=2):
        order, assign, makespan = self.plan_schedule(durations, nstreams)
        self.launches = [self.launches[i] for i in order]
        self.stream_plan = [assign[i] for i in order]
        return makespan

    def plan_schedule(self, durations=None, nstreams=2, launches=None):
        if durations is None:
            if launches is not None:
                raise ValueError("measured durations belong to the engine's current launch order")
            durations = [r["ms"] for r in self.profile_in_sequence(iters=3)]
        elif isinstance(durations, str) and durations == "model":
            ll = self.launches if launches is None else launches
            durations = [max(f / 100e12, nb / 4e12) * 1e3 + 5e-3 for (_, _, f, _), nb in zip(ll, self.launch_bytes(ll))]
        ll = self.launches if launches is None else launches
        prefer = [(kind, name) in (("decode", DECODE_TOPK), ("flip", FLIP_PEAKS)) for (kind, name, _, _) in ll] if os.environ.get("CP_SCHED_PREFER", "1") != "0" else None
        return list_schedule(self.dependencies(launches), durations, nstreams, prefer)

    def _run_branches(self, main, nstreams, deps, assign=None):
        streams = [main] + [torch.cuda.Stream(device=self.device) for _ in range(nstreams - 1)]
        n = len(self.launches)
        has_child = [False] * n
        for d in deps:
            for j in d:
                has_child[j] = True
        where, tail, events = [0] * n, [None] * len(streams), [None] * n
        fork = torch.cuda.Event()
        fork.record(main)
        joined = [True] + [False] * (len(streams) - 1)
        waited = [[-1] * len(streams) for _ in streams]
        for i, (_, _, _, launch) in enumerate(self.launches):
# ... 188 lines not shown
```

### centerpose_amd/nets.py

```python
from collections import OrderedDict

HEADS = (("hm", 1), ("wh", 2), ("hps", 34), ("reg", 2), ("hm_hp", 17), ("hp_offset", 2))
ARCH_HEAD = {"dla_34": (64, 256), "res_50": (256, 64), "hrnet": (32, 64), "mobilenetv3": (24, 256), "shufflenetV2": (256, 256),
             "resdcn_18": (64, 64), "resdcn_34": (64, 64), "resdcn_50": (64, 64), "resdcn_101": (64, 64)}
RESDCN_SPEC = {18: ("basic", [2, 2, 2, 2]), 34: ("basic", [3, 4, 6, 3]), 50: ("bottleneck", [3, 4, 6, 3]),
               101: ("bottleneck", [3, 4, 23, 3])}


class Act:
    __slots__ = ("H", "W", "C", "t", "split", "parent", "__weakref__")

    def __init__(self, H, W, C, t=None, split=None, parent=None):
        self.H, self.W, self.C, self.t, self.split = H, W, C, t, split
        self.parent = parent


class Graph:

    def __init__(self):
        self.spec = OrderedDict()
        self.flops = 0

    def p_conv(self, name, co, ci, k, bias=False, kw=None):
        self.spec[name + ".weight"] = (co, ci, k, kw or k)
        if bias:
            self.spec[name + ".bias"] = (co,)

    def p_bn(self, name, c):
        for s in ("weight", "bias", "running_mean", "running_var"):
            self.spec["%s.%s" % (name, s)] = (c,)
        self.spec[name + ".num_batches_tracked"] = ()

    def emit_conv(self, xs, conv, bn, bias, co, k, stride, pad, relu, res, stem):
        x = xs[0]
        return Act((x.H + 2 * pad - k) // stride + 1, (x.W + 2 * pad - k) // stride + 1, co)

    def emit_maxpool(self, x, k, s, p):
        return Act((x.H + 2 * p - k) // s + 1, (x.W + 2 * p - k) // s + 1, x.C)

    def emit_conv_group(self, members):
        return [self.emit_conv([x], conv, bn, False, co, 3, 1, 1, relu, res, False) for x, conv, bn, co, relu, res in members]

    def emit_conv_batch(self, members):
        return [self.emit_conv([x], conv, bn, False, co, k, stride, pad, relu, None, False) for x, conv, bn, co, k, stride, pad, relu in members]

    def emit_dcn(self, x, conv, bn, co):
        return Act(x.H, x.W, co)

    def emit_up_add(self, x, wname, f, add):
        return Act(x.H * f, x.W * f, x.C)

    def emit_deconv4(self, x, wname, bn, co):
        return Act(x.H * 2, x.W * 2, co)

    def emit_sum_up(self, xs, shifts, relu):
        return Act(xs[0].H, xs[0].W, xs[0].C)

    def emit_sum_up_batch(self, members, relu):
        return [self.emit_sum_up(xs, shifts, relu) for xs, shifts in members]

    def emit_head(self, feat, p, hc):
        return None

    def emit_dwconv(self, x, conv, bn, k, stride, act):
        return Act((x.H + 2 * (k // 2) - k) // stride + 1, (x.W + 2 * (k // 2) - k) // stride + 1, x.C, split=x.split)

    def emit_se(self, x, p, red):
        return Act(1, 1, x.C)

    def emit_scale_add(self, x, se, add):
        return Act(x.H, x.W, x.C)

    def emit_shuffle(self, x1, x2):
        return Act(x1.H, x1.W, 2 * x1.C, split=(x1.C, (x1.C + 15) // 16 * 16))

    def emit_half(self, x, which):
        return Act(x.H, x.W, x.split[0])

    def conv(self, xs, name, bn, co, k, stride=1, pad=0, relu=False, res=None, bias=False, stem=False):
        xs = xs if isinstance(xs, (list, tuple)) else [xs]
        ci = sum(x.C for x in xs)
        self.p_conv(name, co, ci, k, bias)
        if bn:
            self.p_bn(bn, co)
        out = self.emit_conv(xs, name, bn, bias, co, k, stride, pad, relu, res, stem)
        self.flops += 2 * out.H * out.W * co * ci * k * k
        return out

    def deform(self, x, name, co):
        return self.dcn_bn_relu(x, name + ".conv", name + ".actf.0", co)

    def dcn_bn_relu(self, x, conv, bn, co):
        self.p_bn(bn, co)
        self.p_conv(conv, co, x.C, 3, True)
        self.p_conv(conv + ".conv_offset_mask", 27, x.C, 3, True)
        out = self.emit_dcn(x, conv, bn, co)
        self.flops += 2 * x.H * x.W * x.C * 9 * (27 + co)
        return out

    def dwconv(self, x, name, bn, k, stride, act=None):
        self.spec[name + ".weight"] = (x.C, 1, k, k)
        self.p_bn(bn, x.C)
        out = self.emit_dwconv(x, name, bn, k, stride, act)
        self.flops += 2 * out.H * out.W * x.C * k * k
        return out

    def up_add(self, x, wname, f, add):
        self.spec[wname + ".weight"] = (x.C, 1, 2 * f, 2 * f)
        out = self.emit_up_add(x, wname, f, add)
        self.flops += 2 * out.H * out.W * x.C * 4
        return out

    def _dla_block(self, x, p, ci, co, stride, residual):
        h = self.conv(x, p + ".conv1", p + ".bn1", co, 3, stride, 1, relu=True)
        return self.conv(h, p + ".conv2", p + ".bn2", co, 3, 1, 1, relu=True, res=residual)

    def _dla_tree(self, x, p, levels, ci, co, stride, level_root, root_dim=0, children=None, top=True):
        children = [] if children is None else children
        if root_dim == 0:
            root_dim = 2 * co
        if level_root:
            root_dim += ci
        bottom = self.emit_maxpool(x, stride, stride, 0) if stride > 1 else x
        if ci != co:
            self.p_conv(p + ".project.0", co, ci, 1)
            self.p_bn(p + ".project.1", co)
        if level_root:
            children.append(bottom)
        if levels == 1:
            residual = bottom
            if ci != co:
                residual = self.emit_conv([bottom], p + ".project.0", p + ".project.1", False, co, 1, 1, 0, False, None, False)
                self.flops += 2 * residual.H * residual.W * co * ci
            x1 = self._dla_block(x, p + ".tree1", ci, co, stride, residual)
            x2 = self._dla_block(x1, p + ".tree2", co, co, 1, x1)
            return self.conv([x2, x1] + children, p + ".root.conv", p + ".root.bn", co, 1, relu=True)
        x1 = self._dla_tree(x, p + ".tree1", levels - 1, ci, co, stride, False)
        children.append(x1)
        return self._dla_tree(x1, p + ".tree2", levels - 1, co, co, 1, False, root_dim + co, children)

    def dla34(self, x, p="backbone_model"):
        ch, lv = [16, 32, 64, 128, 256, 512], [1, 1, 1, 2, 2, 1]
        b = p + ".base"
        y = []
        x = self.conv(x, b + ".base_layer.0", b + ".base_layer.1", 16, 7, 1, 3, relu=True, stem=True)
        x = self.conv(x, b + ".level0.0", b + ".level0.1", 16, 3, 1, 1, relu=True)
        y.append(x)
        x = self.conv(x, b + ".level1.0", b + ".level1.1", 32, 3, 2, 1, relu=True)
        y.append(x)
        for i in range(2, 6):
            x = self._dla_tree(x, "%s.level%d" % (b, i), lv[i], ch[i - 1], ch[i], 2, i > 2)
            y.append(x)
        layers = list(y)
        out = [layers[-1]]
        for i in range(3):
            o = ch[-i - 2]
            self._ida_up("%s.dla_up.ida_%d" % (p, i), layers, len(layers) - i - 2, len(layers), o)
            out.insert(0, layers[-1])
        yy = [out[0], out[1], out[2]]
        self._ida_up(p + ".ida_up", yy, 0, 3, 64, up_f=[1, 2, 4])
        return yy[-1]

    def _ida_up(self, p, layers, startp, endp, o, up_f=None):
        for i in range(startp + 1, endp):
            j = i - startp
            f = 2 if up_f is None else up_f[j]
            t = self.deform(layers[i], "%s.proj_%d" % (p, j), o)
            u = self.up_add(t, "%s.up_%d" % (p, j), f, layers[i - 1])
            layers[i] = self.deform(u, "%s.node_%d" % (p, j), o)

    def res50(self, x, p="backbone_model"):
        x = self.conv(x, p + ".conv1", p + ".bn1", 64, 7, 2, 3, relu=True, stem=True)
        x = self.emit_maxpool(x, 3, 2, 1)
        inpl = 64
        for li, (planes, n, stride) in enumerate(zip([64, 128, 256, 512], [3, 4, 6, 3], [1, 2, 2, 2]), start=1):
            for b in range(n):
                q = "%s.layer%d.%d" % (p, li, b)
                s = stride if b == 0 else 1
                res = x
                if b == 0:
                    res = self.conv(x, q + ".downsample.0", q + ".downsample.1", planes * 4, 1, s, 0)
                h = self.conv(x, q + ".conv1", q + ".bn1", planes, 1, relu=True)
                h = self.conv(h, q + ".conv2", q + ".bn2", planes, 3, s, 1, relu=True)
                x = self.conv(h, q + ".conv3", q + ".bn3", planes * 4, 1, relu=True, res=res)
                inpl = planes * 4
        for i in range(3):
            wname, bn = "%s.deconv_layers.%d" % (p, 3 * i), "%s.deconv_layers.%d" % (p, 3 * i + 1)
            self.spec[wname + ".weight"] = (inpl, 256, 4, 4)
            self.p_bn(bn, 256)
            x_in = x
            x = self.emit_deconv4(x, wname, bn, 256)
            self.flops += 2 * x_in.H * x_in.W * inpl * 256 * 16
            inpl = 256
        return x

    def resdcn(self, x, num_layers, p="backbone_model"):
        kind, reps = RESDCN_SPEC[num_layers]
        exp = 1 if kind == "basic" else 4
        x = self.conv(x, p + ".conv1", p + ".bn1", 64, 7, 2, 3, relu=True, stem=True)
        x = self.emit_maxpool(x, 3, 2, 1)
        inpl = 64
        for li, (planes, n, stride) in enumerate(zip([64, 128, 256, 512], reps, [1, 2, 2, 2]), start=1):
            for b in range(n):
                q = "%s.layer%d.%d" % (p, li, b)
                s = stride if b == 0 else 1
                res = x
                if b == 0 and (s != 1 or inpl != planes * exp):
                    res = self.conv(x, q + ".downsample.0", q + ".downsample.1", planes * exp, 1, s, 0)
                if kind == "basic":
                    h = self.conv(x, q + ".conv1", q + ".bn1", planes, 3, s, 1, relu=True)
                    x = self.conv(h, q + ".conv2", q + ".bn2", planes, 3, 1, 1, relu=True, res=res)
                else:
                    h = self.conv(x, q + ".conv1", q + ".bn1", planes, 1, relu=True)
                    h = self.conv(h, q + ".conv2", q + ".bn2", planes, 3, s, 1, relu=True)
                    x = self.conv(h, q + ".conv3", q + ".bn3", planes * exp, 1, relu=True, res=res)
                inpl = planes * exp
        for d, planes in enumerate([256, 128, 64]):
            q = "%s.deconv_layers." % p
            x = self.dcn_bn_relu(x, q + str(6 * d), q + str(6 * d + 1), planes)
            self.spec[q + str(6 * d + 3) + ".weight"] = (planes, planes, 4, 4)
            self.p_bn(q + str(6 * d + 4), planes)
            x_in = x
            x = self.emit_deconv4(x, q + str(6 * d + 3), q + str(6 * d + 4), planes)
            self.flops += 2 * x_in.H * x_in.W * planes * planes * 16
        return x

    def _hr_basic(self, x, p):
        h = self.conv(x, p + ".conv1", p + ".bn1", x.C, 3, 1, 1, relu=True)
        return self.conv(h, p + ".conv2", p + ".bn2", x.C, 3, 1, 1, relu=True, res=x)

    def _hr_module(self, xs, p, chans, multi_scale_output):
        nb = len(chans)
        xs = list(xs)
        for i in range(nb):
            for b in range(4):
                q = "%s.branches.%d.%d" % (p, i, b)
                for cv, bn in ((".conv1", ".bn1"), (".conv2", ".bn2")):
                    self.p_conv(q + cv, chans[i], chans[i], 3)
                    self.p_bn(q + bn, chans[i])
                    self.flops += 2 * xs[i].H * xs[i].W * chans[i] * chans[i] * 9
        for b in range(4):
            q = ["%s.branches.%d.%d" % (p, i, b) for i in range(nb)]
            hs = self.emit_conv_group([(xs[i], q[i] + ".conv1", q[i] + ".bn1", chans[i], True, None) for i in range(nb)])
            xs = self.emit_conv_group([(hs[i], q[i] + ".conv2", q[i] + ".bn2", chans[i], True, xs[i]) for i in range(nb)])
        nout = nb if multi_scale_output else 1
        chains = {}
        for i in range(nout):
            for j in range(nb):
                if j > i:
                    q = "%s.fuse_layers.%d.%d" % (p, i, j)
                    chains[(i, j)] = [(q + ".0", q + ".1", chans[j], chans[i], 1, 1, 0, False)]
                elif j < i:
                    chains[(i, j)] = []
                    for k in range(i - j):
                        q = "%s.fuse_layers.%d.%d.%d" % (p, i, j, k)
                        last = k == i - j - 1
                        chains[(i, j)].append((q + ".0", q + ".1", chans[j], chans[i] if last else chans[j], 3, 2, 1, not last))
                if (i, j) in chains:
                    h, w = xs[j].H, xs[j].W
                    for conv, bn, ci, co, k, st, pd, _ in chains[(i, j)]:
                        self.p_conv(conv, co, ci, k)
                        self.p_bn(bn, co)
                        h, w = (h + 2 * pd - k) // st + 1, (w + 2 * pd - k) // st + 1
                        self.flops += 2 * h * w * co * ci * k * k
        cur = {ij: xs[ij[1]] for ij in chains}
        for lvl in range(max([len(c) for c in chains.values()] or [0])):
            todo = [ij for ij in sorted(chains) if len(chains[ij]) > lvl]
            res = self.emit_conv_batch([(cur[ij],) + tuple(chains[ij][lvl][q] for q in (0, 1, 3, 4, 5, 6, 7)) for ij in todo])
            for ij, r in zip(todo, res):
                cur[ij] = r
        return self.emit_sum_up_batch([([xs[j] if j == i else cur[(i, j)] for j in range(nb)], [j - i if j > i else 0 for j in range(nb)])
                                       for i in range(nout)], True)

    def hrnet_w32(self, x, p="backbone_model"):
        x = self.conv(x, p + ".conv1", p + ".bn1", 64, 3, 2, 1, relu=True, stem=True)
        x = self.conv(x, p + ".conv2", p + ".bn2", 64, 3, 2, 1, relu=True)
        for b in range(4):
            q = "%s.layer1.%d" % (p, b)
            res = x if b else self.conv(x, q + ".downsample.0", q + ".downsample.1", 256, 1)
            h = self.conv(x, q + ".conv1", q + ".bn1", 64, 1, relu=True)
            h = self.conv(h, q + ".conv2", q + ".bn2", 64, 3, 1, 1, relu=True)
            x = self.conv(h, q + ".conv3", q + ".bn3", 256, 1, relu=True, res=res)
        pre, ys = [256], [x]
        for si, (nmod, chans) in enumerate([(1, [32, 64]), (4, [32, 64, 128]), (3, [32, 64, 128, 256])], start=1):
            xs = []
            for i, c in enumerate(chans):
                q = "%s.transition%d.%d" % (p, si, i)
                if i < len(pre):
                    xs.append(self.conv(ys[i], q + ".0", q + ".1", c, 3, 1, 1, relu=True) if c != pre[i] else ys[i])
                else:
                    t = ys[-1]
                    for j in range(i + 1 - len(pre)):
                        co = c if j == i - len(pre) else pre[-1]
                        t = self.conv(t, "%s.%d.0" % (q, j), "%s.%d.1" % (q, j), co, 3, 2, 1, relu=True)
                    xs.append(t)
            for m in range(nmod):
                last = (si == 3 and m == nmod - 1)
                xs = self._hr_module(xs, "%s.stage%d.%d" % (p, si + 1, m), chans, not last)
            ys, pre = xs, chans
        return ys[0]

    def _mb_block(self, x, p, k, cin, cexp, cout, act, se, stride):
        h = self.conv(x, p + ".conv1", p + ".bn1", cexp, 1, relu=act)
        h = self.dwconv(h, p + ".conv2", p + ".bn2", k, stride, act)
        sc = None
        if stride == 1:
            sc = x if cin == cout else self.conv(x, p + ".shortcut.0", p + ".shortcut.1", cout, 1)
        if not se:
            return self.conv(h, p + ".conv3", p + ".bn3", cout, 1, res=sc)
        h = self.conv(h, p + ".conv3", p + ".bn3", cout, 1)
        red = cout // 4
        self.p_conv(p + ".se.se.1", red, cout, 1); self.p_bn(p + ".se.se.2", red)
        self.p_conv(p + ".se.se.4", cout, red, 1); self.p_bn(p + ".se.se.5", cout)
        self.flops += 2 * 2 * cout * red
        g = self.emit_se(h, p + ".se.se", red)
        return self.emit_scale_add(h, g, sc)

    def mobilenetv3(self, x, p="backbone_model"):
        x = self.conv(x, p + ".conv1", p + ".bn1", 16, 3, 2, 1, relu="hswish", stem=True)
        R, HS = "relu", "hswish"
# ... 109 lines not shown
```

### centerpose_amd/ops.py

```python
import ctypes
import os

import torch

from . import _lib

ACT_NONE, ACT_RELU, ACT_SIGMOID, ACT_HSWISH, ACT_HSIGMOID = 0, 1, 2, 3, 4
BN_EPS = 1e-5


class ConvDesc(ctypes.Structure):
    _fields_ = [(n, ctypes.c_int) for n in ("nsrc",)] + [("srcC", ctypes.c_int * 4), ("srcLd", ctypes.c_int * 4)] + \
        [(n, ctypes.c_int) for n in ("B", "H", "W", "Ho", "Wo", "kh", "kw", "sy", "sx", "py", "px", "K", "ldw", "Cout",
                                     "resLd", "outLd", "outNCHW", "OH", "OW", "osy", "osx", "ooy", "oox", "act",
                                     "inNCHW", "tile", "nsub", "ksplit")]


class DcnDesc(ctypes.Structure):
    _fields_ = [(n, ctypes.c_int) for n in ("B", "H", "W", "C", "srcLd", "Ho", "Wo", "kh", "kw", "sy", "sx", "py", "px",
                                            "dily", "dilx", "K", "ldw", "Cout", "omLd", "omSigmoid", "outLd",
                                            "outNCHW", "act", "tile", "ksplit", "dg")]


def round_up(x, m):
    return (x + m - 1) // m * m


class Launch:
    __slots__ = ("fn", "desc", "tensors", "ints", "out_index", "kernel", "_cfn", "_args")

    def __init__(self, fn, desc, tensors, ints=(), out_index=-1):
        self.fn, self.desc, self.tensors, self.ints = fn, desc, list(tensors), [int(i) for i in ints]
        self.out_index = out_index % len(self.tensors)
        self.kernel = None
        self._cfn = None
        self._args = None

    @property
    def out(self):
        return self.tensors[self.out_index]

    @property
    def reads(self):
        return [t for i, t in enumerate(self.tensors) if t is not None and i != self.out_index]

    def bind(self):
        L = _lib.lib()
        self._cfn = getattr(L, self.fn)
        ptrs = [_lib.vptr(t) if t is not None else _lib.c_void_p(0) for t in self.tensors]
        self._args = marshal(self.fn, self.desc, ptrs, self.ints)

    def run(self, stream=None):
        if self._cfn is None:
            self.bind()
        _lib.check(self._cfn(*self._args, stream if stream is not None else _lib.stream()), self.fn)
        if self.kernel is None:
            self.kernel = _lib.lib().cp_last_kernel().decode()


def marshal(fn, desc, ptrs, ints):
    d = ctypes.byref(desc) if desc is not None else None
    if fn == "cp_conv2d_f32":
        srcs = (ctypes.c_void_p * 4)(*[p.value for p in ptrs[:4]])
        return [d, srcs] + ptrs[4:]
    if fn in ("cp_conv3x3_winograd_f32", "cp_dcn_v2_f32"):
        return [d] + ptrs
    if fn == "cp_conv3x3_winograd24_group_f32":
        arr = lambda k: (ctypes.c_void_p * 4)(*[p.value for p in ptrs[4 * k:4 * k + 4]])
        return [d, ints[0]] + [arr(k) for k in range(6)]
    if fn == "cp_conv2d_group_f32":
        arr = lambda k: (ctypes.c_void_p * 8)(*[p.value for p in ptrs[8 * k:8 * k + 8]])
        return [d, ints[0]] + [arr(k) for k in range(6)]
    if fn == "cp_head3x3_1x1_f32":
        return [d] + ptrs + ints
    if fn == "cp_stem7x7_f32":
        return ptrs + ints
    if fn == "cp_maxpool2d_nhwc_f32":
        return [ptrs[0], ints[0], ptrs[1]] + ints[1:]
    if fn == "cp_dw_deconv_add_nhwc_f32":
        return [ptrs[0], ints[0], ptrs[1], ptrs[2], ints[1], ptrs[3]] + ints[2:]
    if fn == "cp_sum_up_nhwc_f32":
        srcs = (ctypes.c_void_p * 4)(*[p.value for p in ptrs[:4]])
        lds = (ctypes.c_int * 4)(*ints[1:5])
        shs = (ctypes.c_int * 4)(*ints[5:9])
        return [ints[0], srcs, lds, shs, ptrs[4]] + ints[9:]
    if fn == "cp_sum_up_group_nhwc_f32":
        srcs = (ctypes.c_void_p * 16)(*[p.value for p in ptrs[:16]])
        outs = (ctypes.c_void_p * 4)(*[p.value for p in ptrs[16:20]])
        meta = (ctypes.c_int * 56)(*ints[2:58])
        return [ints[0], srcs, meta, outs, ints[1]]
    if fn == "cp_dwconv2d_nhwc_f32":
        return [ptrs[0], ints[0], ptrs[1], ptrs[2], ptrs[3], ptrs[4]] + ints[1:]
    if fn == "cp_global_avgpool_nhwc_f32":
        return [ptrs[0], ints[0], ptrs[1]] + ints[1:]
    if fn == "cp_scale_add_nhwc_f32":
        return [ptrs[0], ints[0], ptrs[1], ints[1], ptrs[2], ints[2], ptrs[3]] + ints[3:]
    if fn == "cp_shuffle_concat_nhwc_f32":
        return [ptrs[0], ints[0], ptrs[1], ints[1], ptrs[2], ints[2], ctypes.c_longlong(ints[3]), ints[4], ints[5]]
    if fn == "cp_splitk_reduce_f32":
        return [ptrs[0], ints[0], ints[1], ints[2], ptrs[1], ptrs[2], ints[3], ptrs[3], ints[4], ints[5]]
    if fn == "cp_decode_topk_f32":
        return ptrs[:2] + ints + ptrs[2:]
    if fn == "cp_decode_assign_f32":
        return ptrs[:6] + ints + [ptrs[6]]
    if fn == "cp_head_points_f32":
        return [ptrs[0], ints[0]] + ptrs[1:] + ints[1:]
    if fn == "cp_flip_merge_pairs_f32":
        ins = (ctypes.c_void_p * 4)(*[p.value for p in ptrs[:4]])
        outs = (ctypes.c_void_p * 4)(*[p.value for p in ptrs[4:8]])
        meta = (ctypes.c_int * 8)(*ints[5:13])
        return [ints[0], ins, outs, meta] + ints[1:5] + [ptrs[8]]
    raise ValueError("unknown launch function %r" % fn)


FN_IDS = {"cp_conv2d_f32": 1, "cp_conv3x3_winograd_f32": 2, "cp_dcn_v2_f32": 3, "cp_stem7x7_f32": 4,
          "cp_maxpool2d_nhwc_f32": 5, "cp_dw_deconv_add_nhwc_f32": 6, "cp_sum_up_nhwc_f32": 7, "cp_dwconv2d_nhwc_f32": 8,
          "cp_global_avgpool_nhwc_f32": 9, "cp_scale_add_nhwc_f32": 10, "cp_shuffle_concat_nhwc_f32": 11, "cp_head3x3_1x1_f32": 12,
          "cp_decode_topk_f32": 13, "cp_decode_assign_f32": 14, "cp_splitk_reduce_f32": 15, "cp_conv3x3_winograd24_group_f32": 16, "cp_conv2d_group_f32": 17,
          "cp_sum_up_group_nhwc_f32": 18, "cp_head_points_f32": 19,
          "cp_flip_merge_pairs_f32": 20}


def pad_rows(t, ldw):
    Co, K = t.shape
    if Co == ldw:
        return t.contiguous()
    out = torch.zeros((ldw, K), dtype=t.dtype, device=t.device)
    out[:Co] = t
    return out


def pad_vec(v, ldw, fill=0.0):
    out = torch.full((ldw,), fill, dtype=torch.float32, device=v.device)
    out[: v.numel()] = v
    return out


def ldw_for(cout):
    if cout <= 16:
        return 16
    if cout <= 32:
        return 32
    return round_up(cout, 64)


def pack_conv_weight(w, stem=False):
    Co, Ci, kh, kw = w.shape
    if stem:
        wp = w.reshape(Co, Ci * kh * kw)
        K = round_up(Ci * kh * kw, 16)
        if K != wp.shape[1]:
            wp = torch.cat([wp, torch.zeros((Co, K - wp.shape[1]), dtype=w.dtype, device=w.device)], 1)
    else:
        wp = w.permute(0, 2, 3, 1).reshape(Co, kh * kw * Ci)
    return pad_rows(wp.float(), ldw_for(Co))


def fold_bn(cout, bn=None, bias=None, device=None):
    if bn is not None:
        g, b, mean, var = bn
        scale = g / torch.sqrt(var + BN_EPS)
        shift = b - mean * scale
        if bias is not None:
            shift = shift + bias * scale
    else:
        device = bias.device if bias is not None else device
        scale = torch.ones(cout, dtype=torch.float32, device=device)
        shift = bias.clone() if bias is not None else torch.zeros(cout, dtype=torch.float32, device=device)
    ldw = ldw_for(cout)
    return pad_vec(scale.float(), ldw, 0.0), pad_vec(shift.float(), ldw, 0.0)


def _ld(t):
    assert t.dim() == 4 and t.stride(3) == 1 and t.stride(1) == t.shape[2] * t.stride(2) and \
        t.stride(0) == t.shape[1] * t.stride(1), "NHWC tensor with dense pixels expected"
    return t.stride(2)


BATCH_INVARIANT = os.environ.get("CP_BATCH_INVARIANT", "0") == "1"


def rule_batch(B):
    return 1 if BATCH_INVARIANT else B


SPLIT_BF16 = os.environ.get("CP_SPLIT_BF16", "0") == "1"
SPLIT_BF16_TILES = ((128, 128), (128, 64), (64, 128), (64, 64))


def split_bf16_weight(wp, ldw):
    L = _lib.lib()
    rows, K = wp.shape
    assert rows % ldw == 0 and K % 16 == 0 and wp.is_contiguous()
    L.cp_split_bf16_weight_floats.restype = ctypes.c_size_t
    wb = torch.empty((L.cp_split_bf16_weight_floats(rows, K),), dtype=torch.float32, device=wp.device)
    _lib.check(L.cp_split_bf16_weights_f32(_lib.ptr(wp), rows, ldw, K, _lib.ptr(wb), _lib.stream()), "cp_split_bf16_weights_f32")
    return wb


def split_bf16_tile(M, ldw, nsub=1, ksplit=1, force=False, K=None):
    if ldw % 64:
        return None
    code = lambda bm, bn: 3000000 + bm * 1000 + bn
    forced = os.environ.get("CP_SPLIT_BF16_TILE")
    if forced:
        bm, bn = (int(v) for v in forced.split("x")) if "x" in forced else (128, int(forced))
        return code(bm, bn if ldw % bn == 0 else 64)
    blocks = lambda bm, bn: ((M + bm - 1) // bm) * max(1, nsub) * max(1, ksplit) * (ldw // bn)
    floor = 0 if force else int(os.environ.get("CP_SPLIT_BF16_MINBLOCKS", "512"))
    if floor == 0:
        return code(128, 128) if ldw % 128 == 0 and blocks(128, 128) >= 256 else code(128, 64)
    if ksplit > 1:
        return None
    order = ((64, 64),) if K is not None and K <= 64 else ((128, 128), (64, 128), (64, 64))
    for bm, bn in order:
        if ldw % bn == 0 and blocks(bm, bn) >= floor:
            return code(bm, bn)
    return None


def conv2d(srcs, wp, scale, shift, out, **kw):
    conv2d_launch(srcs, wp, scale, shift, out, **kw).run()
    return out


def conv2d_launch(srcs, wp, scale, shift, out, *, kh, kw, stride=1, pad=0, cout, act=ACT_NONE, res=None, out_nchw=False,
                  in_nchw=False, Ho=None, Wo=None, pad_yx=None, out_scatter=None, tile=0, wino=None, nsub=1, ksplit=0, split_bf16=None):
    d = ConvDesc()
    d.nsrc = len(srcs)
    if in_nchw:
        x = srcs[0]
        B, C, H, W = x.shape
        d.srcC[0], d.srcLd[0] = C, 0
        assert x.is_contiguous()
    else:
        B, H, W, _ = srcs[0].shape
        for i, s in enumerate(srcs):
            assert s.shape[:3] == srcs[0].shape[:3]
            d.srcC[i], d.srcLd[i] = s.shape[3], _ld(s)
    py, px = pad_yx if pad_yx is not None else (pad, pad)
    if Ho is None:
        Ho = (H + 2 * py - kh) // stride + 1
        Wo = (W + 2 * px - kw) // stride + 1
    d.B, d.H, d.W, d.Ho, d.Wo = B, H, W, Ho, Wo
    d.kh, d.kw, d.sy, d.sx, d.py, d.px = kh, kw, stride, stride, py, px
    assert wp.shape[0] % nsub == 0
    d.K, d.ldw, d.Cout, d.nsub = wp.shape[1], wp.shape[0] // nsub, cout, nsub
    d.resLd = _ld(res) if res is not None else 0
    d.outNCHW = 1 if out_nchw else 0
    d.ksplit = ksplit
    if ksplit > 1:
        assert res is None and act == ACT_NONE and not out_nchw and out.is_contiguous() and (wino is not None or (len(srcs) == 1 and not in_nchw and nsub == 1))
        assert tuple(out.shape[:2]) == (ksplit, B * Ho * Wo) and out.shape[2] >= cout and out.shape[2] % 4 == 0
        d.OH, d.OW, d.outLd = Ho, Wo, out.shape[2]
    elif out_nchw:
        d.OH, d.OW, d.outLd = out.shape[2], out.shape[3], 0
        assert out.is_contiguous() and out.shape[1] == cout
    else:
        d.OH, d.OW, d.outLd = out.shape[1], out.shape[2], _ld(out)
    d.osy, d.osx, d.ooy, d.oox = out_scatter if out_scatter is not None else (1, 1, 0, 0)
    d.act, d.inNCHW, d.tile = act, 1 if in_nchw else 0, tile
    for t in (wp, scale, shift, wino):
        assert t is None or t.is_contiguous()
    if wino is not None:
        assert len(srcs) == 1 and not in_nchw
        return Launch("cp_conv3x3_winograd_f32", d, [srcs[0], wino, scale, shift, res, out])
    if (SPLIT_BF16 if split_bf16 is None else split_bf16) and tile == 0 and not in_nchw:
        code = split_bf16_tile(rule_batch(B) * Ho * Wo, d.ldw, nsub, ksplit, force=split_bf16 is True, K=d.K)
        c16 = kh == 3 and kw == 3 and len(srcs) == 1 and srcs[0].shape[3] == 16 and cout <= 32
        if code is not None and not c16 and all(s.data_ptr() % 16 == 0 for s in srcs):
            d.tile = code
            wp = split_bf16_weight(wp, d.ldw)
    return Launch("cp_conv2d_f32", d, list(srcs) + [None] * (4 - len(srcs)) + [wp, scale, shift, res, out])


ConvDesc4 = ConvDesc * 4


def conv3x3_group_launch(members, whole):
    assert 1 <= len(members) <= 4
    members = sorted(members, key=lambda mm: -mm["x"].shape[3])
    d = ConvDesc4()
    cols = [[None] * 4 for _ in range(6)]
    for i, mm in enumerate(members):
        one = conv2d_launch([mm["x"]], mm["wp"], mm["scale"], mm["shift"], mm["out"], kh=3, kw=3, stride=1, pad=1, cout=mm["cout"],
                            act=mm["act"], res=mm["res"], wino=mm["u24"], tile=WINO24)
        ctypes.memmove(ctypes.addressof(d[i]), ctypes.addressof(one.desc), ctypes.sizeof(ConvDesc))
        for k, t in enumerate((mm["x"], mm["u24"], mm["scale"], mm["shift"], mm["res"], mm["out"])):
            cols[k][i] = t
            assert t is None or k in (0, 4, 5) or t.is_contiguous()
        assert mm["out"].untyped_storage().data_ptr() == whole.untyped_storage().data_ptr()
    return Launch("cp_conv3x3_winograd24_group_f32", d, [t for col in cols for t in col] + [whole], [len(members)])


ConvDesc8 = ConvDesc * 8
GROUP_MAX = 8


def conv2d_group_launch(members, whole):
    assert 1 <= len(members) <= GROUP_MAX
    members = sorted(members, key=lambda mm: -mm["wp"].shape[1])
    d = ConvDesc8()
    cols = [[None] * GROUP_MAX for _ in range(6)]
    for i, mm in enumerate(members):
        assert mm["wp"].shape[0] % 64 == 0
        one = conv2d_launch([mm["x"]], mm["wp"], mm["scale"], mm["shift"], mm["out"], kh=mm["k"], kw=mm["k"], stride=mm["stride"],
                            pad=mm["pad"], cout=mm["cout"], act=mm["act"], res=mm.get("res"), split_bf16=False)
        ctypes.memmove(ctypes.addressof(d[i]), ctypes.addressof(one.desc), ctypes.sizeof(ConvDesc))
        for k, t in enumerate((mm["x"], mm["wp"], mm["scale"], mm["shift"], mm.get("res"), mm["out"])):
            cols[k][i] = t
            assert t is None or k in (0, 4, 5) or t.is_contiguous()
        assert mm["out"].untyped_storage().data_ptr() == whole.untyped_storage().data_ptr()
    return Launch("cp_conv2d_group_f32", d, [t for col in cols for t in col] + [whole], [len(members)])


def head3x3_1x1_eligible(x, hc, n2):
    B, H, W, C = x.shape
    B = rule_batch(B)
    return C == 64 and hc % 32 == 0 and hc >= 128 and 1 <= n2 <= 34 and B * ((H + 7) // 8) * ((W + 15) // 16) >= 512


def head_wino24_wanted(x, n2):
    B, H, W, _ = x.shape
    B = rule_batch(B)
    mode = os.environ.get("CP_HEAD24", "1")
    if mode == "0" or B * ((H + 15) // 16) * ((W + 15) // 16) < 256:
        return False
    return mode == "all" or n2 <= 32


def head3x3_1x1_launch(x, u, scale, shift, w2, b2, out2, *, hc, act2=ACT_NONE, wino24=False):
    B, H, W, C = x.shape
    n2, ld2 = w2.shape
    assert out2.is_contiguous() and tuple(out2.shape) == (B, n2, H, W) and w2.is_contiguous() and b2.numel() >= n2
    d = ConvDesc()
    d.nsrc = 1
    d.srcC[0], d.srcLd[0] = C, _ld(x)
    d.B, d.H, d.W, d.Ho, d.Wo = B, H, W, H, W
    d.kh, d.kw, d.sy, d.sx, d.py, d.px = 3, 3, 1, 1, 1, 1
    d.K, d.ldw, d.Cout = 9 * C, round_up(hc, 64), hc
    d.resLd, d.outLd, d.outNCHW = 0, hc, 0
    d.OH, d.OW, d.osy, d.osx, d.ooy, d.oox = H, W, 1, 1, 0, 0
    d.act, d.inNCHW, d.tile, d.nsub = ACT_RELU, 0, WINO24 if wino24 else 0, 1
    return Launch("cp_head3x3_1x1_f32", d, [x, u, scale, shift, w2, b2, out2], [n2, ld2, act2])


def wino_eligible(cin, k, stride, pad, nsrc=1):
    return k == 3 and stride == 1 and pad == 1 and nsrc == 1 and cin % 16 == 0 and cin >= 32


def pack_wino_weight(wp, cin, cout):
    L = _lib.lib()
    assert wp.shape[1] == 9 * cin and wp.shape[0] >= cout and wp.is_contiguous()
    L.cp_winograd_weight_floats.restype = ctypes.c_size_t
    n = L.cp_winograd_weight_floats(cin, cout)
    assert n > 0, "winograd: C must be a multiple of 16"
    u = torch.empty((n,), dtype=torch.float32, device=wp.device)
    _lib.check(L.cp_winograd_pack_f32(_lib.ptr(wp), _lib.ptr(u), cin, cout, _lib.stream()), "cp_winograd_pack_f32")
    return u


def pack_wino24_weight(wp, cin, cout):
    L = _lib.lib()
    assert wp.shape[1] == 9 * cin and wp.shape[0] >= cout and wp.is_contiguous()
    L.cp_winograd24_weight_floats.restype = ctypes.c_size_t
    n = L.cp_winograd24_weight_floats(cin, cout)
    assert n > 0, "winograd: C must be a multiple of 16"
    u = torch.empty((n,), dtype=torch.float32, device=wp.device)
    _lib.check(L.cp_winograd24_pack_f32(_lib.ptr(wp), _lib.ptr(u), cin, cout, _lib.stream()), "cp_winograd24_pack_f32")
    return u


WINO24 = 24


def wino24_wanted(B, H, W, cin, cout):
    if os.environ.get("CP_WINO24", "1") == "0" or cin % 16 or cin < 32:
        return False
    minc, mincout, minblocks = (int(v) for v in os.environ.get("CP_WINO24_RULE", "32,16,256").split(","))
    blocks = rule_batch(B) * ((H + 15) // 16) * ((W + 15) // 16) * ((cout + 31) // 32)
    return cin >= minc and cout >= mincout and blocks >= minblocks


def dcn_v2(x, om, wp, scale, shift, out, **kw):
    dcn_v2_launch(x, om, wp, scale, shift, out, **kw).run()
    return out


def _pair(v):
    return (int(v[0]), int(v[1])) if isinstance(v, (tuple, list)) else (int(v), int(v))


def dcn_v2_launch(x, om, wp, scale, shift, out, *, cout, kh=3, kw=3, stride=1, pad=1, dil=1, om_sigmoid=True,
                  act=ACT_NONE, out_nchw=False, tile=0, ksplit=0, dg=1):
    B, H, W, C = x.shape
    d = DcnDesc()
    (sy, sx), (py, px), (dy, dx) = _pair(stride), _pair(pad), _pair(dil)
    Ho = (H + 2 * py - (dy * (kh - 1) + 1)) // sy + 1
    Wo = (W + 2 * px - (dx * (kw - 1) + 1)) // sx + 1
    assert om.shape[:3] == (B, Ho, Wo)
    d.B, d.H, d.W, d.C, d.srcLd, d.Ho, d.Wo = B, H, W, C, _ld(x), Ho, Wo
    d.kh, d.kw, d.sy, d.sx, d.py, d.px, d.dily, d.dilx = kh, kw, sy, sx, py, px, dy, dx
    d.K, d.ldw, d.Cout = wp.shape[1], wp.shape[0], cout
    d.omLd, d.omSigmoid = _ld(om), 1 if om_sigmoid else 0
    d.outNCHW = 1 if out_nchw else 0
    d.act, d.tile, d.ksplit, d.dg = act, tile, ksplit, dg
    if ksplit > 1:
        assert tuple(out.shape) == (ksplit, B * Ho * Wo, wp.shape[0]) and out.is_contiguous() and cout == wp.shape[0] and act == ACT_NONE
        d.outLd = wp.shape[0]
    else:
        d.outLd = 0 if out_nchw else _ld(out)
    return Launch("cp_dcn_v2_f32", d, [x, om, wp, scale, shift, out])


def wino_ksplit(B, H, W, cin, cout):
    blocks = rule_batch(B) * ((H + 7) // 8) * ((W + 15) // 16) * ((cout + 31) // 32)
    stages = cin // 16
    S = 1
    while blocks * S < 512 and stages // (2 * S) >= 4:
        S *= 2
    return S if blocks < 256 else 1


def conv_ksplit(M, ldw, K):
    if ldw % 64 != 0:
        return 1
    blocks = ((M + 63) // 64) * (ldw // 64)
    if blocks >= 400:
        return 1
    for S in (2, 3, 4):
        if blocks * S >= 512 and (K // 16) // S >= 16:
            return S
    return 1


def dcn_ksplit(M, ldw, taps=9):
    if ldw % 64 != 0 or taps < 3:
        return 1
    blocks = -(-M // 64) * (ldw // 64)
    return 3 if blocks < 512 else 1


def splitk_reduce_launch(ws, scale, shift, out, *, cout, act=ACT_NONE):
    S, M, ldw = ws.shape
    assert ws.is_contiguous() and out.shape[0] * out.shape[1] * out.shape[2] == M and scale.numel() >= ldw and shift.numel() >= ldw
    return Launch("cp_splitk_reduce_f32", None, [ws, scale, shift, out], [S, M, ldw, act, _ld(out), cout])


def maxpool2d_launch(x, out, k, s, p):
    B, H, W, C = x.shape
    return Launch("cp_maxpool2d_nhwc_f32", None, [x, out], [_ld(x), _ld(out), B, H, W, C, k, s, p])


def maxpool2d(x, out, k, s, p):
    maxpool2d_launch(x, out, k, s, p).run()
    return out


def pack_dw_deconv_weight(w):
    C, _, k, _ = w.shape
    return w.reshape(C, k * k).t().contiguous().float()


def dw_deconv_add_launch(x, wk, add, out, f):
    B, H, W, C = x.shape
    assert wk.is_contiguous()
    return Launch("cp_dw_deconv_add_nhwc_f32", None, [x, wk, add, out],
                  [_ld(x), _ld(add) if add is not None else 0, _ld(out), B, H, W, C, f])


def dw_deconv_add(x, wk, add, out, f):
    dw_deconv_add_launch(x, wk, add, out, f).run()
    return out


def pack_dw_weight(w):
    C, _, k, _ = w.shape
    return w.reshape(C, k * k).t().contiguous().float()


def dwconv2d_launch(x, wk, scale, shift, out, k, stride, pad, act=ACT_NONE):
    B, H, W, C = x.shape
    assert wk.shape == (k * k, C) and wk.is_contiguous() and scale.numel() >= C and shift.numel() >= C
    return Launch("cp_dwconv2d_nhwc_f32", None, [x, wk, scale, shift, out], [_ld(x), _ld(out), B, H, W, C, k, stride, pad, act])


def dwconv2d(x, wk, scale, shift, out, k, stride, pad, act=ACT_NONE):
    dwconv2d_launch(x, wk, scale, shift, out, k, stride, pad, act).run()
    return out


def global_avgpool_launch(x, out):
    B, H, W, C = x.shape
    return Launch("cp_global_avgpool_nhwc_f32", None, [x, out], [_ld(x), _ld(out), B, H * W, C])


def global_avgpool(x, out):
    global_avgpool_launch(x, out).run()
    return out


def scale_add_launch(x, se, add, out):
    B, H, W, C = x.shape
    return Launch("cp_scale_add_nhwc_f32", None, [x, se, add, out], [_ld(x), _ld(se), _ld(add) if add is not None else 0, _ld(out), B, H, W, C])


def scale_add(x, se, add, out):
    scale_add_launch(x, se, add, out).run()
    return out


def shuffle_concat_launch(x1, x2, out, h, hp):
    B, H, W, _ = out.shape
    assert out.shape[3] >= 2 * hp and x1.shape[:3] == out.shape[:3] == x2.shape[:3]
    return Launch("cp_shuffle_concat_nhwc_f32", None, [x1, x2, out], [_ld(x1), _ld(x2), _ld(out), B * H * W, h, hp])


def shuffle_concat(x1, x2, out, h, hp):
    shuffle_concat_launch(x1, x2, out, h, hp).run()
    return out


def sum_up_launch(srcs, shifts, out, relu):
    B, H, W, C = out.shape
    n = len(srcs)
    return Launch("cp_sum_up_nhwc_f32", None, list(srcs) + [None] * (4 - n) + [out],
                  [n] + [_ld(s) for s in srcs] + [0] * (4 - n) + list(shifts) + [0] * (4 - n) + [_ld(out), B, H, W, C, 1 if relu else 0])


def sum_up_group_launch(members, whole, relu):
    n = len(members)
    assert 1 <= n <= 4
    ptrs, outs, meta = [], [], []
    for srcs, shifts, out in members:
        B, H, W, C = out.shape
        k = len(srcs)
        assert 1 <= k <= 4 and out.untyped_storage().data_ptr() == whole.untyped_storage().data_ptr()
        ptrs += list(srcs) + [None] * (4 - k)
        outs.append(out)
        meta += [k] + [_ld(t) for t in srcs] + [0] * (4 - k) + list(shifts) + [0] * (4 - k) + [_ld(out), B, H, W, C]
    ptrs += [None] * (4 * (4 - n))
    outs += [None] * (4 - n)
    meta += [0] * (14 * (4 - n))
    return Launch("cp_sum_up_group_nhwc_f32", None, ptrs + outs + [whole], [n, 1 if relu else 0] + meta)


def sum_up(srcs, shifts, out, relu):
    sum_up_launch(srcs, shifts, out, relu).run()
    return out


def nchw_to_nhwc(x, out=None, c_off=0):
    B, C, H, W = x.shape
    if out is None:
        out = torch.empty((B, H, W, C), dtype=torch.float32, device=x.device)
    rc = _lib.lib().cp_nchw_to_nhwc_f32(_lib.ptr(_lib.f32(x.contiguous())), _lib.vptr(out), B, C, H, W, _ld(out), c_off,
                                        _lib.stream())
    _lib.check(rc, "cp_nchw_to_nhwc_f32")
    return out


def nhwc_to_nchw(x, C=None, c_off=0):
    B, H, W, Cx = x.shape
    C = Cx if C is None else C
    out = torch.empty((B, C, H, W), dtype=torch.float32, device=x.device)
    rc = _lib.lib().cp_nhwc_to_nchw_f32(_lib.vptr(x), _ld(x), c_off, _lib.ptr(out), B, C, H, W, _lib.stream())
    _lib.check(rc, "cp_nhwc_to_nchw_f32")
    return out


def pack_deconv4_subpixel(w, py, px):
    Ci, Co = w.shape[:2]
    kys = [3 - py - 2 * t for t in range(2)]
    kxs = [3 - px - 2 * t for t in range(2)]
    sub = w[:, :, kys][:, :, :, kxs]
    wp = sub.permute(1, 2, 3, 0).reshape(Co, 4 * Ci)
    return pad_rows(wp.float().contiguous(), ldw_for(Co))


def pack_stem7_weight(w):
    Co, Ci, kh, kw = w.shape
    assert (Ci, kh, kw) == (3, 7, 7)
    wp = torch.zeros((Co, 22, 8), dtype=torch.float32, device=w.device)
    wp[:, :21, :7] = w.reshape(Co, 21, 7)
    return wp.reshape(Co, 176).contiguous()


def stem7x7_launch(x, wp, scale, shift, out, stride, relu=True):
    B, C, H, W = x.shape
    assert C == 3 and x.is_contiguous() and wp.is_contiguous()
    return Launch("cp_stem7x7_f32", None, [x, wp, scale, shift, out], [B, H, W, wp.shape[0], stride, _ld(out), 1 if relu else 0])


def stem7x7(x, wp, scale, shift, out, stride, relu=True):
    stem7x7_launch(x, wp, scale, shift, out, stride, relu).run()
    return out


def decode_launches(hm, wh, hps, reg, hm_hp, hp_offset, K, ws, dets):
    B, cat, H, W = hm.shape
    J = hps.shape[1] // 2
    assert ws.dtype == torch.float32 and tuple(ws.shape) == (2, B, 1 + J, K) and tuple(dets.shape) == (B, K, 5 + 3 * J)
    for t in (hm, wh, hps, reg, hm_hp, hp_offset, ws, dets):
        assert t is None or t.is_contiguous()
    topk = Launch("cp_decode_topk_f32", None, [hm, hm_hp, ws[0], ws[1]], [B, cat, J, H, W, K], out_index=2)
    assign = Launch("cp_decode_assign_f32", None, [wh, hps, reg, hp_offset, ws[0], ws[1], dets], [B, J, H, W, K], out_index=6)
    return topk, assign


def pack_head_points_weight(w3):
    hc, C = w3.shape[:2]
    assert C % 16 == 0 and hc % 32 == 0
    wk = w3.float().permute(2, 3, 1, 0).reshape(9 * C // 8, 2, 4, hc)
    return wk.permute(0, 1, 3, 2).contiguous().reshape(-1)


def head_points_launch(feat, inds, w1, b1, w2, b2, out, *, hc, J, K):
    B, H, W, C = feat.shape
    assert tuple(inds.shape) == (B, 1 + J, K) and inds.is_contiguous() and out.is_contiguous() and out.numel() == B * H * W * (6 + 2 * J)
    assert w1.numel() == 4 * 9 * C * hc and b1.numel() == 4 * hc and tuple(w2.shape) == (6 + 2 * J, hc) and b2.numel() == 6 + 2 * J
    for t in (w1, b1, w2, b2):
# ... 26 lines not shown
```

### centerpose_amd/plan.py

```python
import ctypes
import json
import struct

import numpy as np
import torch

from . import _lib, ops

MAGIC = b"CPPLAN04"
MAGIC_V3 = b"CPPLAN03"
MAGIC_V2 = b"CPPLAN02"


def checksum(data):
    mv = memoryview(data).cast("B")
    n = len(mv)
    if n == 0:
        return 2166136261
    buf = (ctypes.c_ubyte * n).from_buffer_copy(mv) if mv.readonly else (ctypes.c_ubyte * n).from_buffer(mv)
    L = _lib.lib()
    L.cp_fnv1a32.restype = ctypes.c_uint32
    L.cp_fnv1a32.argtypes = [ctypes.c_void_p, ctypes.c_size_t]
    return int(L.cp_fnv1a32(ctypes.addressof(buf), n))


REF_NULL, REF_BUF, REF_CONST = 0, 1, 2
FN_NAMES = {v: k for k, v in ops.FN_IDS.items()}
DESC_TYPES = {"cp_conv2d_f32": ops.ConvDesc, "cp_conv3x3_winograd_f32": ops.ConvDesc, "cp_dcn_v2_f32": ops.DcnDesc,
              "cp_conv3x3_winograd24_group_f32": ops.ConvDesc4, "cp_conv2d_group_f32": ops.ConvDesc8,
              "cp_head3x3_1x1_f32": ops.ConvDesc}


def _pad8(b):
    return b + b"\0" * (-len(b) % 8)


def _storage_key(t):
    return t.untyped_storage().data_ptr()


class _Encoder:

    def __init__(self, buffer_storages):
        self.buf_ids = {}
        self.buf_numel = []
        self.const_ids = {}
        self.consts = []
        self.buffer_storages = buffer_storages

    def ref(self, t):
        if t is None:
            return (REF_NULL, 0, 0, 0)
        assert t.dtype == torch.float32, "plan tensors are float32"
        key = _storage_key(t)
        if key in self.buffer_storages:
            if key not in self.buf_ids:
                self.buf_ids[key] = len(self.buf_numel)
                self.buf_numel.append(t.untyped_storage().nbytes() // 4)
            return (REF_BUF, self.buf_ids[key], (t.data_ptr() - key) // 4, t.numel())
        assert t.is_contiguous(), "plan constants are contiguous"
        ck = (t.data_ptr(), t.numel())
        if ck not in self.const_ids:
            self.const_ids[ck] = len(self.consts)
            self.consts.append(t.detach().reshape(-1).cpu())
        return (REF_CONST, self.const_ids[ck], 0, t.numel())


def _pack_ref(r):
    return struct.pack("<IIQQ", *r)


def serialize(launches, meta, inp, outputs, abi, streams=None):
    streams = list(streams) if streams is not None else [0] * len(launches)
    assert len(streams) == len(launches) and all(x in (0, 1) for x in streams)
    written = {_storage_key(inp)} | {_storage_key(l.out) for _, _, _, l in launches}
    enc = _Encoder(written)
    in_ref = enc.ref(inp)
    op_blobs = []
    for (_, _, _, l), st in zip(launches, streams):
        desc = bytes(l.desc) if l.desc is not None else b""
        refs = b"".join(_pack_ref(enc.ref(t)) for t in l.tensors)
        ints = _pad8(struct.pack("<%di" % len(l.ints), *l.ints))
        op_blobs.append(struct.pack("<IIIIII", ops.FN_IDS[l.fn], len(desc), len(l.tensors), len(l.ints), l.out_index, st)
                        + _pad8(desc) + refs + ints)
    out_blob = b"".join(_pack_ref(enc.ref(o)) + struct.pack("<4I", *o.shape) for o in outputs)
    mj = dict(meta)
    mj["ops"] = [{"kind": k, "name": n, "flops": int(f)} for k, n, f, _ in launches]
    mjs = json.dumps(mj).encode()
    B, _, H, W = inp.shape
    head = MAGIC + struct.pack("<IIIIIIIIII", abi, B, H, W, len(enc.buf_numel), len(enc.consts), len(launches), len(outputs), len(mjs), 0)
    assert len(head) == 48
    head += _pad8(mjs) + struct.pack("<%dQ" % len(enc.buf_numel), *enc.buf_numel)
    body = _pack_ref(in_ref) + out_blob + b"".join(op_blobs)
    table_len = 16 * len(enc.consts)
    pos = len(head) + table_len + len(body)
    table, data = b"", []
    for c in enc.consts:
        pos += -pos % 64
        table += struct.pack("<QQ", c.numel(), pos)
        data.append((pos, c))
        pos += 4 * c.numel()
    out = bytearray(head + table + body)
    for off, c in data:
        out += b"\0" * (off - len(out))
        out += c.numpy().tobytes()
    struct.pack_into("<I", out, 44, checksum(memoryview(out)[48:]))
    return bytes(out)


def plan_blob(engine, deterministic=False):
    import os
    launches, streams = engine.launches, getattr(engine, "stream_plan", None)
    can_schedule = os.environ.get("CP_SCHED", "1") != "0" and os.environ.get("CP_STREAMS", "2") == "2"
    if deterministic:
        if not can_schedule:
            raise ValueError("save_plan(deterministic=True) writes the two-stream model schedule: unset CP_SCHED=0 / CP_STREAMS")
        base = getattr(engine, "emission", None)
        if base is None:
            raise ValueError("save_plan(deterministic=True): this engine was loaded from a plan file and has no emission order")
        order, assign, _ = engine.plan_schedule("model", launches=base)
        launches, streams = [base[i] for i in order], [assign[i] for i in order]
    elif streams is None and can_schedule:
        if engine.graph is None:
            engine.schedule()
            launches, streams = engine.launches, engine.stream_plan
        else:
            order, assign, _ = engine.plan_schedule(None)
            launches, streams = [engine.launches[i] for i in order], [assign[i] for i in order]
    meta = {"arch": engine.arch, "flops_per_image": int(engine.flops_per_image)}
    if getattr(engine, "dets_only", False):
        meta["dets_only"] = True
    if getattr(engine, "flip_test", False):
        meta["flip_test"] = True
    return serialize(launches, meta, engine.input, getattr(engine, "head_maps", engine.outputs), int(_lib.lib().cp_abi_version()), streams)


def save_plan(engine, path, deterministic=False):
    blob = plan_blob(engine, deterministic)
    with open(path, "wb") as f:
        f.write(blob)
    return len(blob)


def compile_state_dict(arch, state_dict, B, H, W, head_conv=None, decode_k=None):
    from . import engine as _engine
    sd = {k: (v if torch.is_tensor(v) else torch.as_tensor(v)) for k, v in dict(state_dict).items()}
    eng = _engine.Engine(arch, sd, int(B), int(H), int(W), head_conv=head_conv, sigmoid_heads=("hm", "hm_hp"), use_graph=False,
                         decode_k=int(decode_k) if decode_k else None)
    return plan_blob(eng, deterministic=True)


class _Reader:
    def __init__(self, blob):
        self.b, self.p = blob, 0

    def take(self, fmt):
        v = struct.unpack_from(fmt, self.b, self.p)
        self.p += struct.calcsize(fmt)
        return v

    def raw(self, n, pad=True):
        v = bytes(self.b[self.p:self.p + n])
        self.p += n + ((-n % 8) if pad else 0)
        return v

    def ref(self):
        return self.take("<IIQQ")


def parse(blob):
    if len(blob) < 48 or bytes(blob[:8]) not in (MAGIC, MAGIC_V3, MAGIC_V2):
        raise ValueError("not a centerpose_amd plan file (magic %r)" % bytes(blob[:8]))
    r = _Reader(blob)
    r.p = 8
    abi, B, H, W, nbuf, nconst, nops, nout, mlen, csum = r.take("<IIIIIIIIII")
    if bytes(blob[:8]) == MAGIC and checksum(memoryview(blob)[48:]) != csum:
        raise ValueError("plan file: checksum mismatch (truncated or corrupted)")
    try:
        meta = json.loads(r.raw(mlen).decode())
    except ValueError:
        raise ValueError("plan file: corrupt meta block")
# ... 86 lines not shown
```

### include/centerpose_hip.h

```cpp
#ifndef CENTERPOSE_HIP_H
#define CENTERPOSE_HIP_H
#include <stddef.h>
#ifdef __cplusplus
extern "C" {
#endif

int cp_abi_version(void);
const char* cp_target_arch(void);
const char* cp_last_error(void);
const char* cp_last_kernel(void);

enum { CP_ACT_NONE = 0, CP_ACT_RELU = 1, CP_ACT_SIGMOID = 2,
       CP_ACT_HSWISH = 3, CP_ACT_HSIGMOID = 4 };

typedef struct cp_conv_desc {
    int nsrc;
    int srcC[4], srcLd[4];
    int B, H, W;
    int Ho, Wo;
    int kh, kw, sy, sx, py, px;
    int K, ldw;
    int Cout;
    int resLd, outLd;
    int outNCHW;
    int OH, OW, osy, osx, ooy, oox;
    int act;
    int inNCHW;
    int tile;
    int nsub;
    int ksplit;
} cp_conv_desc;
int cp_conv2d_f32(const cp_conv_desc* d, const float* const* src, const float* w, const float* scale, const float* shift,
                  const float* res, float* out, void* stream);

int cp_conv2d_group_f32(const cp_conv_desc* d, int n, const float* const* src, const float* const* w, const float* const* scale,
                        const float* const* shift, const float* const* res, float* const* out, void* stream);

size_t cp_split_bf16_weight_floats(int rows, int K);
int cp_split_bf16_weights_f32(const float* w, int rows, int ldw, int K, float* wb, void* stream);

size_t cp_winograd_weight_floats(int C, int Cout);
int cp_winograd_pack_f32(const float* w, float* u, int C, int Cout, void* stream);
size_t cp_winograd24_weight_floats(int C, int Cout);
int cp_winograd24_pack_f32(const float* w, float* u, int C, int Cout, void* stream);
int cp_conv3x3_winograd_f32(const cp_conv_desc* d, const float* src, const float* u, const float* scale, const float* shift,
                            const float* res, float* out, void* stream);

int cp_conv3x3_winograd24_group_f32(const cp_conv_desc* d, int n, const float* const* src, const float* const* u,
                                    const float* const* scale, const float* const* shift, const float* const* res,
                                    float* const* out, void* stream);

int cp_head3x3_1x1_f32(const cp_conv_desc* d, const float* src, const float* u, const float* scale, const float* shift,
                       const float* w2, const float* b2, float* out2, int n2, int ld2, int act2, void* stream);

typedef struct cp_dcn_desc {
    int B, H, W, C, srcLd;
    int Ho, Wo;
    int kh, kw, sy, sx, py, px, dily, dilx;
    int K, ldw, Cout;
    int omLd, omSigmoid;
    int outLd, outNCHW, act;
    int tile;
    int ksplit;
    int dg;
} cp_dcn_desc;
int cp_dcn_v2_f32(const cp_dcn_desc* d, const float* x, const float* om, const float* w, const float* scale,
                  const float* shift, float* out, void* stream);
int cp_dcn_pack_weights_f32(const float* w, const float* bias, int Co, int C, int kh, int kw, int dg, int Cp, int ldw, float* wp,
                            float* scale, float* shift, void* stream);
int cp_sizeof_conv_desc(void);
int cp_sizeof_dcn_desc(void);

int cp_splitk_reduce_f32(const float* ws, int splits, int M, int ldw, const float* scale, const float* shift, int act, float* out,
                         int outLd, int Cout, void* stream);

int cp_stem7x7_f32(const float* x, const float* w, const float* scale, const float* shift, float* out, int B, int H, int W,
                   int Cout, int stride, int outLd, int relu, void* stream);

int cp_maxpool2d_nhwc_f32(const float* in, int inLd, float* out, int outLd, int B, int H, int W, int C, int k, int s, int p,
                          void* stream);
int cp_dw_deconv_add_nhwc_f32(const float* in, int inLd, const float* w, const float* add, int addLd, float* out, int outLd,
                              int B, int H, int W, int C, int f, void* stream);
int cp_sum_up_nhwc_f32(int n, const float* const* src, const int* ld, const int* shift, float* out, int outLd, int B, int H,
                       int W, int C, int relu, void* stream);
int cp_sum_up_group_nhwc_f32(int n, const float* const* src, const int* meta, float* const* out, int relu, void* stream);
int cp_dwconv2d_nhwc_f32(const float* in, int inLd, const float* w, const float* scale, const float* shift, float* out, int outLd,
                         int B, int H, int W, int C, int k, int s, int p, int act, void* stream);
int cp_global_avgpool_nhwc_f32(const float* in, int inLd, float* out, int outLd, int B, int HW, int C, void* stream);
int cp_scale_add_nhwc_f32(const float* x, int xLd, const float* se, int seLd, const float* add, int addLd, float* out, int outLd,
                          int B, int H, int W, int C, void* stream);
int cp_shuffle_concat_nhwc_f32(const float* x1, int ld1, const float* x2, int ld2, float* out, int outLd, long long npix, int h, int hp,
                               void* stream);
int cp_nchw_to_nhwc_f32(const float* in, float* out, int B, int C, int H, int W, int outLd, int cOff, void* stream);
int cp_nhwc_to_nchw_f32(const float* in, int inLd, int cOff, float* out, int B, int C, int H, int W, void* stream);
int cp_fill_f32(float* p, float v, long long n, void* stream);
int cp_flip_merge_f32(const float* in, float* out, int C, int H, int W, int mode, const int* perm, void* stream);
int cp_flip_merge_pairs_f32(int n, const float* const* in, float* const* out, const int* meta, int N, int H, int W, int J,
                            const int* perm, void* stream);

int cp_resize_u8(const unsigned char* src, int H, int W, unsigned char* dst, int NH, int NW, void* stream);
int cp_preprocess_u8_f32(const unsigned char* img, int H, int W, const double* M, float* out, int OH, int OW, const float* mean,
                         const float* std_, int flip, void* stream);
int cp_transform_dets_f32(const float* dets, float* out, const double* trans, int B, int K, int J, float scale, void* stream);

int cp_decode_workspace_bytes(int B, int J, int K, size_t* scores_bytes, size_t* inds_bytes);
int cp_multi_pose_decode_f32(const float* heat, const float* wh, const float* kps, const float* reg,
                             const float* hm_hp, const float* hp_offset, int B, int cat, int J, int H,
                             int W, int K, float* dets, float* ws_scores, int* ws_inds, void* stream);
int cp_decode_topk_f32(const float* heat, const float* hm_hp, int B, int cat, int J, int H, int W, int K, float* ws_scores,
                       int* ws_inds, void* stream);
int cp_decode_assign_f32(const float* wh, const float* kps, const float* reg, const float* hp_offset, const float* ws_scores,
                         const int* ws_inds, int B, int J, int H, int W, int K, float* dets, void* stream);

int cp_head_points_f32(const float* feat, int featLd, const int* ws_inds, const float* w1, const float* b1, const float* w2,
                       const float* b2, float* out, int B, int H, int W, int C, int J, int K, int hc, void* stream);

typedef struct cp_plan cp_plan;
unsigned int cp_fnv1a32(const void* data, size_t bytes);
int cp_plan_load(const char* path, int use_graph, cp_plan** out);
int cp_plan_create(const void* blob, size_t bytes, int use_graph, cp_plan** out);
int cp_plan_info(const cp_plan* plan, int* B, int* H, int* W, int* n_outputs, int* n_launches);
float* cp_plan_input(const cp_plan* plan);
int cp_plan_output(const cp_plan* plan, int i, float** dev_ptr, int shape[4]);
int cp_plan_forward(cp_plan* plan, const float* images, void* stream);
int cp_plan_process(cp_plan* plan, const float* images, int K, float* dets, void* stream);
int cp_plan_destroy(cp_plan* plan);
int cp_plan_dets_only(const cp_plan* plan);
int cp_plan_flip_test(const cp_plan* plan);

typedef struct cp_pipeline cp_pipeline;
int cp_plan_clone(const cp_plan* plan, cp_plan** out);
int cp_pipeline_create(cp_plan* const* plans, int depth, cp_pipeline** out);
int cp_pipeline_process(cp_pipeline* pipe, const float* const* images, int K, float* const* dets, void* stream);
int cp_pipeline_destroy(cp_pipeline* pipe);
int cp_memcpy_d2d(void* dst, const void* src, size_t bytes, void* stream);

int cp_soft_nms_39(float* boxes, int N, float sigma, float Nt, float threshold, int method, int* keep, int* n_keep);

#ifdef __cplusplus
}
#endif
#endif
```

Baseline: 2237.

## Fold split-K partial-sum reduction into DCN offset gather and depthwise deconv consumers

When the offset/mask convolution runs split-K, the DCN kernel can now read the raw partial slices itself, sum them, and apply the offset conv's scale and shift, so the separate split-K reduce pass is skipped. The depthwise deconv-add kernels get a templated split mode that sums partial slices and applies scale, shift and activation at load time, which lets a split-K DCN output feed the up-add directly. This removes reduce launches and a round trip of the intermediate through memory, in exchange for repeated slice reads where consumers touch the same pixel several times (the 3x3 deconv neighbourhood). It also lowers the DCN max-tap limit to match the LDS budget.

```diff
diff --git a/centerpose_amd/csrc/common.h b/centerpose_amd/csrc/common.h
--- a/centerpose_amd/csrc/common.h
+++ b/centerpose_amd/csrc/common.h
@@ -85,3 +85,57 @@
     if (act == CP_ACT_HSIGMOID_) return fminf(fmaxf(v + 3.f, 0.f), 6.f) / 6.f;
     return v;
 }
+
+template <int S>
+__device__ __forceinline__ float cp_splitk_sum_n(const float* p, size_t slice)
+{
+    float v[S];
+#pragma unroll
+    for (int s = 0; s < S; ++s) v[s] = p[(size_t)s * slice];
+    float acc = v[0];
+#pragma unroll
+    for (int s = 1; s < S; ++s) acc += v[s];
+    return acc;
+}
+__device__ __forceinline__ float cp_splitk_sum(const float* p, int S, size_t slice)
+{
+    switch (S) {
+        case 2: return cp_splitk_sum_n<2>(p, slice);
+        case 3: return cp_splitk_sum_n<3>(p, slice);
+        case 4: return cp_splitk_sum_n<4>(p, slice);
+        case 8: return cp_splitk_sum_n<8>(p, slice);
+    }
+    float acc = p[0];
+    for (int s = 1; s < S; ++s) acc += p[(size_t)s * slice];
+    return acc;
+}
+__device__ __forceinline__ float cp_splitk_finish(float sum, float sc, float sh, int act) { return cp_act(__builtin_fmaf(sum, sc, sh), act); }
+template <int S>
+__device__ __forceinline__ float4 cp_splitk_sum4_n(const float* p, size_t slice)
+{
+    float4 v[S];
+#pragma unroll
+    for (int s = 0; s < S; ++s) v[s] = *reinterpret_cast<const float4*>(p + (size_t)s * slice);
+    float4 acc = v[0];
+#pragma unroll
+    for (int s = 1; s < S; ++s) { acc.x += v[s].x; acc.y += v[s].y; acc.z += v[s].z; acc.w += v[s].w; }
+    return acc;
+}
+__device__ __forceinline__ float4 cp_splitk_load4(const float* p, int S, size_t slice, float4 sc, float4 sh, int act)
+{
+    float4 acc;
+    switch (S) {
+        case 2: acc = cp_splitk_sum4_n<2>(p, slice); break;
+        case 3: acc = cp_splitk_sum4_n<3>(p, slice); break;
+        case 4: acc = cp_splitk_sum4_n<4>(p, slice); break;
+        case 8: acc = cp_splitk_sum4_n<8>(p, slice); break;
+        default:
+            acc = *reinterpret_cast<const float4*>(p);
+            for (int s = 1; s < S; ++s) {
+                const float4 v = *reinterpret_cast<const float4*>(p + (size_t)s * slice);
+                acc.x += v.x; acc.y += v.y; acc.z += v.z; acc.w += v.w;
+            }
+    }
+    return make_float4(cp_splitk_finish(acc.x, sc.x, sh.x, act), cp_splitk_finish(acc.y, sc.y, sh.y, act),
+                       cp_splitk_finish(acc.z, sc.z, sh.z, act), cp_splitk_finish(acc.w, sc.w, sh.w, act));
+}
diff --git a/centerpose_amd/csrc/dcn.hip b/centerpose_amd/csrc/dcn.hip
--- a/centerpose_amd/csrc/dcn.hip
+++ b/centerpose_amd/csrc/dcn.hip
@@ -1,7 +1,7 @@
 #include <cstdlib>
 #include "igemm.h"
 
-#define DCN_MAX_TAPS 121
+#define DCN_MAX_TAPS 112
 typedef float dcn_v2 __attribute__((ext_vector_type(2)));
 
 __device__ __forceinline__ void dcn_blend(dcn_v2& r, dcn_v2 wxy, dcn_v2 wzw, dcn_v2 c00, dcn_v2 c01, dcn_v2 c10, dcn_v2 c11)
@@ -10,6 +10,17 @@
     asm("v_pk_fma_f32 %0, %1, %2, %0 op_sel:[1,0,0] op_sel_hi:[1,1,1]" : "+v"(r) : "v"(wxy), "v"(c01));
     asm("v_pk_fma_f32 %0, %1, %2, %0 op_sel_hi:[0,1,1]" : "+v"(r) : "v"(wzw), "v"(c10));
     asm("v_pk_fma_f32 %0, %1, %2, %0 op_sel:[1,0,0] op_sel_hi:[1,1,1]" : "+v"(r) : "v"(wzw), "v"(c11));
+}
+
+template <int S>
+__device__ __forceinline__ void dcn_om3(const float* omp, size_t slice, int c0, int c2, float& dy, float& dx, float& mk)
+{
+    float v0[S], v1[S], v2[S];
+#pragma unroll
+    for (int s = 0; s < S; ++s) { v0[s] = omp[s * slice + c0]; v1[s] = omp[s * slice + c0 + 1]; v2[s] = omp[s * slice + c2]; }
+    dy = v0[0]; dx = v1[0]; mk = v2[0];
+#pragma unroll
+    for (int s = 1; s < S; ++s) { dy += v0[s]; dx += v1[s]; mk += v2[s]; }
 }
 
 template <int BM, int BN, int WAVES_M, int WAVES_N, int MF>
@@ -48,6 +59,8 @@
         const bool live = m < a.M;
         const int b = live ? m / HoWo : 0, p = m - b * HoWo, oy = p / a.Wo, ox = p - oy * a.Wo;
         const float* omp = a.om + (size_t)(live ? m : 0) * a.omLd;
+        const int omS = a.omSplit;
+        const size_t omSl = (size_t)a.omSlice;
         const int by = oy * a.sy - a.py, bx = ox * a.sx - a.px, bpix = b * a.H * a.W;
         const float fH = (float)a.H, fW = (float)a.W;
         const unsigned ld4 = (unsigned)ld >> 2;
@@ -56,8 +69,20 @@
         int t = tap0 + __builtin_amdgcn_readfirstlane(tid / BM);
         int ky = t / a.kw, kx = t - ky * a.kw;
         for (; t < tap1; t += TS) {
-            const float offh = omp[2 * (og + t)], offw = omp[2 * (og + t) + 1];
-            float mk = omp[a.omMaskOff + og + t];
+            const int c0 = 2 * (og + t), c2 = a.omMaskOff + og + t;
+            float offh, offw, mk;
+            if (omS <= 1) { offh = omp[c0]; offw = omp[c0 + 1]; mk = omp[c2]; }
+            else {
+                switch (omS) {
+                    case 2: dcn_om3<2>(omp, omSl, c0, c2, offh, offw, mk); break;
+                    case 4: dcn_om3<4>(omp, omSl, c0, c2, offh, offw, mk); break;
+                    case 8: dcn_om3<8>(omp, omSl, c0, c2, offh, offw, mk); break;
+                    default: offh = cp_splitk_sum(omp + c0, omS, omSl); offw = cp_splitk_sum(omp + c0 + 1, omS, omSl); mk = cp_splitk_sum(omp + c2, omS, omSl);
+                }
+                offh = cp_splitk_finish(offh, a.omScale[c0], a.omShift[c0], CP_ACT_NONE_);
+                offw = cp_splitk_finish(offw, a.omScale[c0 + 1], a.omShift[c0 + 1], CP_ACT_NONE_);
+                mk = cp_splitk_finish(mk, a.omScale[c2], a.omShift[c2], CP_ACT_NONE_);
+            }
             if (a.omSigmoid) mk = __builtin_amdgcn_rcpf(1.0f + __expf(-mk));
             const float h_im = (float)(by + ky * a.dily) + offh;
             const float w_im = (float)(bx + kx * a.dilx) + offw;
@@ -208,15 +233,25 @@
     int tile;
     int ksplit;
     int dg;
+    int omSplit;
+    int omSlice;
 };
 
 extern "C" int cp_sizeof_dcn_desc(void) { return (int)sizeof(cp_dcn_desc); }
 
-extern "C" int cp_dcn_v2_f32(const cp_dcn_desc* d, const float* x, const float* om, const float* w, const float* scale,
-                             const float* shift, float* out, void* stream)
+extern "C" int cp_dcn_fold_split_default(void)
+{
+    static const int on = !(getenv("CP_DCN_FOLD_SPLIT") && getenv("CP_DCN_FOLD_SPLIT")[0] == '0');
+    return on;
+}
+
+extern "C" int cp_dcn_v2_fold_f32(const cp_dcn_desc* d, const float* x, const float* om, const float* omScale, const float* omShift,
+                                  const float* w, const float* scale, const float* shift, float* out, void* stream)
 {
     CP_CHECK_ARG(d && x && om && w && scale && shift && out, "dcn_v2: null pointer");
-    CP_CHECK_ARG(d->kh > 0 && d->kw > 0 && d->kh * d->kw <= DCN_MAX_TAPS, "dcn_v2: 1..%d taps (kh=%d kw=%d)", DCN_MAX_TAPS, d->kh, d->kw);
+    CP_CHECK_ARG(d->kh > 0 && d->kw > 0 && d->kh * d->kw <= DCN_MAX_TAPS,
+                 "dcn_v2: 1..%d taps (kh=%d kw=%d): the sampling records take dg * kh * kw * BM * 20 B of LDS beside the GEMM tiles, 160 KB in all -- "
+                 "112 taps on the 64 x 64 tile, 104 on 64 x 128, 54 on 128 x 32, divided by the deformable groups", DCN_MAX_TAPS, d->kh, d->kw);
     CP_CHECK_ARG(d->sy > 0 && d->sx > 0 && d->dily > 0 && d->dilx > 0 && d->py >= 0 && d->px >= 0, "dcn_v2: stride / dilation > 0, pad >= 0");
     CP_CHECK_ARG(d->C % 16 == 0 && d->srcLd % 4 == 0 && d->srcLd >= d->C, "dcn_v2: C%%16==0, ld%%4==0 required");
     CP_CHECK_ARG(d->K == d->kh * d->kw * d->C, "dcn_v2: K=%d != kh*kw*C", d->K);
@@ -237,6 +272,13 @@
     a.om = om; a.omLd = d->omLd; a.omMaskOff = 2 * dgv * d->kh * d->kw; a.omSigmoid = d->omSigmoid; a.dg = dgv;
     a.dily = d->dily; a.dilx = d->dilx; a.nsub = 1;
     a.ksplit = d->ksplit > 1 ? d->ksplit : 1;
+    a.omSplit = d->omSplit > 1 ? d->omSplit : 1;
+    a.omSlice = d->omSlice > 0 ? d->omSlice : (int)((long long)a.M * d->omLd);
+    a.omScale = omScale; a.omShift = omShift;
+    CP_CHECK_ARG(a.omSplit == 1 || (omScale && omShift), "dcn_v2: omSplit=%d needs the offset convolution's scale / shift", a.omSplit);
+    CP_CHECK_ARG(a.omSplit == 1 || ((long long)a.M * d->omLd <= 0x7fffffffll / a.omSplit && (long long)a.omSlice >= (long long)a.M * d->omLd &&
+                                    (long long)a.omSlice * a.omSplit <= 0x7fffffffll),
+                 "dcn_v2: omSplit=%d slices of %d floats (M * omLd = %lld)", a.omSplit, a.omSlice, (long long)a.M * d->omLd);
     CP_CHECK_ARG(a.ksplit <= d->kh * d->kw, "dcn_v2: ksplit=%d exceeds the %d taps", a.ksplit, d->kh * d->kw);
     CP_CHECK_ARG(a.ksplit == 1 || (!d->outNCHW && d->act == CP_ACT_NONE && d->outLd == d->ldw && d->Cout == d->ldw),
                  "dcn_v2: split-K writes raw NHWC partial sums (outLd == Cout == ldw, no activation)");
@@ -268,3 +310,10 @@
     CP_CHECK_LAUNCH("dcn_igemm_kernel");
     return 0;
 }
+
+extern "C" int cp_dcn_v2_f32(const cp_dcn_desc* d, const float* x, const float* om, const float* w, const float* scale,
+                             const float* shift, float* out, void* stream)
+{
+    CP_CHECK_ARG(d && d->omSplit <= 1, "dcn_v2: omSplit > 1 goes through cp_dcn_v2_fold_f32 (it needs the offset convolution's scale / shift)");
+    return cp_dcn_v2_fold_f32(d, x, om, nullptr, nullptr, w, scale, shift, out, stream);
+}
diff --git a/centerpose_amd/csrc/elementwise.hip b/centerpose_amd/csrc/elementwise.hip
--- a/centerpose_amd/csrc/elementwise.hip
+++ b/centerpose_amd/csrc/elementwise.hip
@@ -59,9 +59,11 @@
     return 0;
 }
 
+struct EwSplit { int S; long long slice; const float* scale; const float* shift; int act; };
+template <bool SPLIT>
 __global__ void dw_deconv_add_kernel(const float* __restrict__ in, int inLd, const float* __restrict__ w,
                                      const float* add, int addLd, float* out, int outLd, EwRow r,
-                                     int H, int W, int f, int p)
+                                     int H, int W, int f, int p, EwSplit sp)
 {
     const int k = 2 * f, Ho = H * f, Wo = W * f, C = r.C4 * 4;
     const int e = blockIdx.x * EW_THREADS + threadIdx.x;
@@ -69,6 +71,8 @@
     int ox, c4;
     ew_split(r, e, ox, c4);
     const int rx = (ox + p) % f;
+    float4 ssc = make_float4(0.f, 0.f, 0.f, 0.f), ssh = ssc;
+    if (SPLIT) { ssc = *reinterpret_cast<const float4*>(sp.scale + c4 * 4); ssh = *reinterpret_cast<const float4*>(sp.shift + c4 * 4); }
     for (int row = blockIdx.y; row < r.rows; row += gridDim.y) {
         const int b = row / Ho, oy = row - b * Ho;
         float4 acc = make_float4(0.f, 0.f, 0.f, 0.f);
@@ -81,7 +85,8 @@
             for (int tx = 0; tx < 2; ++tx) {
                 const int kx = rx + tx * f, ix = (ox + p - kx) / f;
                 if (ox + p - kx < 0 || ix >= W) continue;
-                const float4 v = *reinterpret_cast<const float4*>(in + ((size_t)(b * H + iy) * W + ix) * inLd + c4 * 4);
+                const float* ip = in + ((size_t)(b * H + iy) * W + ix) * inLd + c4 * 4;
+                const float4 v = SPLIT ? cp_splitk_load4(ip, sp.S, (size_t)sp.slice, ssc, ssh, sp.act) : *reinterpret_cast<const float4*>(ip);
                 const float4 ww = *reinterpret_cast<const float4*>(w + (size_t)(ky * k + kx) * C + c4 * 4);
                 acc.x += v.x * ww.x; acc.y += v.y * ww.y; acc.z += v.z * ww.z; acc.w += v.w * ww.w;
             }
@@ -95,9 +100,10 @@
     }
 }
 
+template <bool SPLIT>
 __global__ __launch_bounds__(EW_THREADS) void dw_deconv2_add_kernel(const float* __restrict__ in, int inLd, const float* __restrict__ w,
                                                                    const float* add, int addLd, float* out,
-                                                                   int outLd, EwRow r, int H, int W)
+                                                                   int outLd, EwRow r, int H, int W, EwSplit sp)
 {
     const int C = r.C4 * 4, Wo = 2 * W;
     const int e = blockIdx.x * EW_THREADS + threadIdx.x;
@@ -109,6 +115,8 @@
     for (int t = 0; t < 16; ++t) wt[t] = *reinterpret_cast<const float4*>(w + (size_t)t * C + c4 * 4);
     const bool lok = ix > 0, rok = ix + 1 < W;
     const float4 z = make_float4(0.f, 0.f, 0.f, 0.f);
+    float4 ssc = z, ssh = z;
+    if (SPLIT) { ssc = *reinterpret_cast<const float4*>(sp.scale + c4 * 4); ssh = *reinterpret_cast<const float4*>(sp.shift + c4 * 4); }
     for (int row = blockIdx.y; row < r.rows; row += gridDim.y) {
         const int b = row / H, iy = row - b * H;
         const float* base = in + ((size_t)row * W + ix) * inLd + c4 * 4;
@@ -121,7 +129,9 @@
 #pragma unroll
             for (int dx = -1; dx <= 1; ++dx) {
                 const bool ok = yok && (dx == 0 || (dx < 0 ? lok : rok));
-                v[dy + 1][dx + 1] = ok ? *reinterpret_cast<const float4*>(base + dy * (long long)rs + dx * inLd) : z;
+                const float* ip = base + dy * (long long)rs + dx * inLd;
+                if (SPLIT) v[dy + 1][dx + 1] = ok ? cp_splitk_load4(ip, sp.S, (size_t)sp.slice, ssc, ssh, sp.act) : z;
+                else v[dy + 1][dx + 1] = ok ? *reinterpret_cast<const float4*>(ip) : z;
             }
         }
 #pragma unroll
@@ -149,28 +159,45 @@
     }
 }
 
-extern "C" int cp_dw_deconv_add_nhwc_f32(const float* in, int inLd, const float* w, const float* add, int addLd, float* out,
-                                         int outLd, int B, int H, int W, int C, int f, void* stream)
+static int dw_deconv_add_impl(const float* in, int inLd, const float* w, const float* add, int addLd, float* out, int outLd, int B, int H,
+                              int W, int C, int f, int splits, const float* scale, const float* shift, int act, hipStream_t stream)
 {
     CP_CHECK_ARG(in && w && out && C % 4 == 0 && inLd % 4 == 0 && outLd % 4 == 0 && (!add || addLd % 4 == 0),
                  "dw_deconv_add: C, ld must be multiples of 4");
     CP_CHECK_ARG(f >= 1, "dw_deconv_add: f=%d", f);
     CP_CHECK_ARG((long long)W * f * (C / 4) * (C / 4) < (1ll << 32) && (long long)B * H * f < (1ll << 31), "dw_deconv_add: row too large");
+    const bool split = splits > 1;
+    CP_CHECK_ARG(!split || (scale && shift && C <= inLd), "dw_deconv_add: %d input slices need scale / shift and C <= inLd", splits);
+    const EwSplit sp = {split ? splits : 1, (long long)B * H * W * inLd, scale, shift, act};
     const char* sw = getenv("CP_DWDECONV2");
     if (f == 2 && !(sw && sw[0] == '0') && (long long)W * (C / 4) * (C / 4) < (1ll << 32)) {
         const EwRow r2 = ew_row(B * H, W, C / 4);
-        hipLaunchKernelGGL(dw_deconv2_add_kernel, ew_row_grid(r2), dim3(EW_THREADS), 0, (hipStream_t)stream, in, inLd, w, add, addLd, out,
-                           outLd, r2, H, W);
-        cp_note_kernel("dw_deconv2_add_kernel");
+        if (split) hipLaunchKernelGGL(dw_deconv2_add_kernel<true>, ew_row_grid(r2), dim3(EW_THREADS), 0, stream, in, inLd, w, add, addLd, out, outLd, r2, H, W, sp);
+        else hipLaunchKernelGGL(dw_deconv2_add_kernel<false>, ew_row_grid(r2), dim3(EW_THREADS), 0, stream, in, inLd, w, add, addLd, out, outLd, r2, H, W, sp);
+        cp_note_kernel(split ? "dw_deconv2_add_kernel<split>" : "dw_deconv2_add_kernel");
         CP_CHECK_LAUNCH("dw_deconv2_add_kernel");
         return 0;
     }
     const EwRow r = ew_row(B * H * f, W * f, C / 4);
-    hipLaunchKernelGGL(dw_deconv_add_kernel, ew_row_grid(r), dim3(EW_THREADS), 0, (hipStream_t)stream, in, inLd, w, add,
-                       addLd, out, outLd, r, H, W, f, f / 2);
-    cp_note_kernel("dw_deconv_add_kernel");
+    if (split) hipLaunchKernelGGL(dw_deconv_add_kernel<true>, ew_row_grid(r), dim3(EW_THREADS), 0, stream, in, inLd, w, add, addLd, out, outLd, r, H, W, f, f / 2, sp);
+    else hipLaunchKernelGGL(dw_deconv_add_kernel<false>, ew_row_grid(r), dim3(EW_THREADS), 0, stream, in, inLd, w, add, addLd, out, outLd, r, H, W, f, f / 2, sp);
+    cp_note_kernel(split ? "dw_deconv_add_kernel<split>" : "dw_deconv_add_kernel");
     CP_CHECK_LAUNCH("dw_deconv_add_kernel");
     return 0;
+}
+
+extern "C" int cp_dw_deconv_add_nhwc_f32(const float* in, int inLd, const float* w, const float* add, int addLd, float* out,
+                                         int outLd, int B, int H, int W, int C, int f, void* stream)
+{
+    return dw_deconv_add_impl(in, inLd, w, add, addLd, out, outLd, B, H, W, C, f, 1, nullptr, nullptr, CP_ACT_NONE_, (hipStream_t)stream);
+}
+
+extern "C" int cp_dw_deconv_add_split_nhwc_f32(const float* ws, int wsLd, int splits, const float* scale, const float* shift, int act,
+                                               const float* w, const float* add, int addLd, float* out, int outLd, int B, int H, int W,
+                                               int C, int f, void* stream)
+{
+    CP_CHECK_ARG(splits >= 1, "dw_deconv_add_split: splits=%d", splits);
+    return dw_deconv_add_impl(ws, wsLd, w, add, addLd, out, outLd, B, H, W, C, f, splits, scale, shift, act, (hipStream_t)stream);
 }
 
 __global__ void splitk_reduce_kernel(const float* __restrict__ ws, int S, long long slice, int ldw4, const float* __restrict__ scale,
@@ -181,15 +208,8 @@
     const long long m = i / ldw4;
     const int n = (int)(i - m * ldw4) * 4;
     if (n >= Cout) return;
-    float4 acc = *reinterpret_cast<const float4*>(ws + i * 4);
-    for (int s = 1; s < S; ++s) {
-        const float4 v = *reinterpret_cast<const float4*>(ws + (size_t)s * slice + i * 4);
-        acc.x += v.x; acc.y += v.y; acc.z += v.z; acc.w += v.w;
-    }
     const float4 sc = *reinterpret_cast<const float4*>(scale + n), sh = *reinterpret_cast<const float4*>(shift + n);
-    acc.x = cp_act(acc.x * sc.x + sh.x, act); acc.y = cp_act(acc.y * sc.y + sh.y, act);
-    acc.z = cp_act(acc.z * sc.z + sh.z, act); acc.w = cp_act(acc.w * sc.w + sh.w, act);
-    *reinterpret_cast<float4*>(out + (size_t)m * outLd + n) = acc;
+    *reinterpret_cast<float4*>(out + (size_t)m * outLd + n) = cp_splitk_load4(ws + i * 4, S, (size_t)slice, sc, sh, act);
 }
 
 extern "C" int cp_splitk_reduce_f32(const float* ws, int splits, int M, int ldw, const float* scale, const float* shift, int act, float* out,
diff --git a/centerpose_amd/csrc/igemm.h b/centerpose_amd/csrc/igemm.h
--- a/centerpose_amd/csrc/igemm.h
+++ b/centerpose_amd/csrc/igemm.h
@@ -38,6 +38,9 @@
     int ksplit;
     int dg;
     int nsub;
+    int omSplit = 0, omSlice = 0;
+    const float* omScale = nullptr;
+    const float* omShift = nullptr;
 };
 
 int cp_launch_conv3x3_patch(const ConvArgs& a, int in_nchw, hipStream_t s, int variant = 0);
diff --git a/centerpose_amd/csrc/plan_runtime.cpp b/centerpose_amd/csrc/plan_runtime.cpp
--- a/centerpose_amd/csrc/plan_runtime.cpp
+++ b/centerpose_amd/csrc/plan_runtime.cpp
@@ -12,6 +12,9 @@
 int cp_conv2d_f32(const cp_conv_desc*, const float* const*, const float*, const float*, const float*, const float*, float*, void*);
 int cp_conv3x3_winograd_f32(const cp_conv_desc*, const float*, const float*, const float*, const float*, const float*, float*, void*);
 int cp_dcn_v2_f32(const cp_dcn_desc*, const float*, const float*, const float*, const float*, const float*, float*, void*);
+int cp_dcn_v2_fold_f32(const cp_dcn_desc*, const float*, const float*, const float*, const float*, const float*, const float*, const float*, float*, void*);
+int cp_dw_deconv_add_split_nhwc_f32(const float*, int, int, const float*, const float*, int, const float*, const float*, int, float*, int, int, int, int, int,
+                                    int, void*);
 int cp_conv3x3_winograd24_group_f32(const cp_conv_desc*, int, const float* const*, const float* const*, const float* const*, const float* const*,
                                     const float* const*, float* const*, void*);
 int cp_conv2d_group_f32(const cp_conv_desc*, int, const float* const*, const float* const*, const float* const*, const float* const*,
@@ -44,7 +47,7 @@
 
 enum { FN_CONV = 1, FN_WINO = 2, FN_DCN = 3, FN_STEM7 = 4, FN_POOL = 5, FN_UPADD = 6, FN_SUMUP = 7, FN_DWCONV = 8, FN_AVGPOOL = 9,
        FN_SCALEADD = 10, FN_SHUFFLE = 11, FN_HEAD = 12, FN_TOPK = 13, FN_ASSIGN = 14, FN_SPLITK = 15, FN_WINO24G = 16, FN_CONVG = 17, FN_SUMUPG = 18,
-       FN_POINTS = 19, FN_FLIPPAIRS = 20 };
+       FN_POINTS = 19, FN_FLIPPAIRS = 20, FN_DCNFOLD = 21, FN_UPADDSPLIT = 22 };
 enum { REF_NULL = 0, REF_BUF = 1, REF_CONST = 2 };
 
 struct Op {
@@ -113,6 +116,10 @@
             return cp_conv3x3_winograd_f32(reinterpret_cast<const cp_conv_desc*>(o.desc.data()), P[0], P[1], P[2], P[3], P[4], P[5], s);
         case FN_DCN:
             return cp_dcn_v2_f32(reinterpret_cast<const cp_dcn_desc*>(o.desc.data()), P[0], P[1], P[2], P[3], P[4], P[5], s);
+        case FN_DCNFOLD:
+            return cp_dcn_v2_fold_f32(reinterpret_cast<const cp_dcn_desc*>(o.desc.data()), P[0], P[1], P[2], P[3], P[4], P[5], P[6], P[7], s);
+        case FN_UPADDSPLIT:
+            return cp_dw_deconv_add_split_nhwc_f32(P[0], I[0], I[1], P[1], P[2], I[2], P[3], P[4], I[3], P[5], I[4], I[5], I[6], I[7], I[8], I[9], s);
         case FN_WINO24G:
             return cp_conv3x3_winograd24_group_f32(reinterpret_cast<const cp_conv_desc*>(o.desc.data()), I[0], reinterpret_cast<const float* const*>(P.data()),
                                                    reinterpret_cast<const float* const*>(P.data() + 4), reinterpret_cast<const float* const*>(P.data() + 8),
@@ -168,6 +175,8 @@
         case FN_CONV: return o.ptrs.size() == 9 && (int)o.desc.size() == cp_sizeof_conv_desc();
         case FN_WINO: return o.ptrs.size() == 6 && (int)o.desc.size() == cp_sizeof_conv_desc();
         case FN_DCN: return o.ptrs.size() == 6 && (int)o.desc.size() == cp_sizeof_dcn_desc();
+        case FN_DCNFOLD: return o.ptrs.size() == 8 && (int)o.desc.size() == cp_sizeof_dcn_desc();
+        case FN_UPADDSPLIT: return o.ptrs.size() == 6 && o.ints.size() == 10;
         case FN_WINO24G: return o.ptrs.size() == 25 && o.ints.size() == 1 && o.ints[0] >= 1 && o.ints[0] <= 4 && (int)o.desc.size() == 4 * cp_sizeof_conv_desc();
         case FN_CONVG: return o.ptrs.size() == 49 && o.ints.size() == 1 && o.ints[0] >= 1 && o.ints[0] <= 8 && (int)o.desc.size() == 8 * cp_sizeof_conv_desc();
         case FN_STEM7: return o.ptrs.size() == 5 && o.ints.size() == 7;
diff --git a/centerpose_amd/engine.py b/centerpose_amd/engine.py
--- a/centerpose_amd/engine.py
+++ b/centerpose_amd/engine.py
@@ -53,8 +53,9 @@
 
 
 class PlanBuilder(nets.Graph):
-    def __init__(self, sd, B, device, sigmoid_heads=True, const_cache=None, dets_only=False):
+    def __init__(self, sd, B, device, sigmoid_heads=True, const_cache=None, dets_only=False, dcn_fold=None):
         super().__init__()
+        self.dcn_fold = ops.dcn_fold_split_default() if dcn_fold is None else bool(dcn_fold)
         self.dets_only = dets_only
         self.points = None
         self.sd, self.B, self.dev = sd, B, device
@@ -149,7 +150,7 @@
             hit = self.const_cache[("unit", n)] = (torch.ones(n, device=self.dev), torch.zeros(n, device=self.dev))
         return hit
 
-    def add_wino(self, name, flops, x, wp, u, sc, sh, out, cout, act, res=None):
+    def add_wino(self, name, flops, x, wp, u, sc, sh, out, cout, act, res=None, raw_ok=False):
         B, H, W, cin = x.shape
         if isinstance(u, tuple):
             self.add("wino24", name, flops, ops.conv2d_launch([x], wp, sc, sh, out, kh=3, kw=3, stride=1, pad=1, cout=cout, act=act,
@@ -157,12 +158,14 @@
             return
         S = ops.wino_ksplit(B, H, W, cin, cout) if (self.wino_splitc and res is None) else 1
         if S > 1:
-            ld, M = out.shape[3], B * H * W
+            ld, M = (out.shape[3] if out is not None else cout), B * H * W
             ws = self.pool.take(S * M * ld)
             wst = ws[: S * M * ld].view(S, M, ld)
             ones, zeros = self.unit_scale(sc.numel())
             self.add("wino", name, flops, ops.conv2d_launch([x], wp, ones, zeros, wst, kh=3, kw=3, stride=1, pad=1, cout=cout, wino=u,
                                                             ksplit=S))
+            if raw_ok:
+                return ws, wst
             self.add("sum", name + ".splitc", 0, ops.splitk_reduce_launch(wst, sc, sh, out, cout=cout, act=act))
             self.pool.give(ws)
             return
@@ -276,20 +279,26 @@
         self._pool_cache[key] = (weakref.ref(x), weakref.ref(out))
         return out
 
-    def emit_dcn(self, x, conv, bn, co):
-        om = self.buf(x.H, x.W, 32)
+    def emit_dcn(self, x, conv, bn, co, raw_ok=False):
         wom = ops.pack_conv_weight(self.expand_in(self.w(conv + ".conv_offset_mask.weight"), [x]))
         som, hom = ops.fold_bn(27, None, self.w(conv + ".conv_offset_mask.bias"), self.dev)
         som[27:] = 0.0
-        out = self.buf(x.H, x.W, co)
+        out = None if (raw_ok and self.dcn_fold) else self.buf(x.H, x.W, co)
         wp = ops.pack_conv_weight(self.expand_in(self.w(conv + ".weight"), [x]))
         sc, sh = ops.fold_bn(co, self.bn(bn), self.w(conv + ".bias"), self.dev)
         uom = self.wino(wom, x.t.shape[3], 32, key=conv + ".conv_offset_mask", hw=(x.H, x.W))
+        om_split = self.dcn_fold and uom is not None and not isinstance(uom, tuple) and self.wino_splitc and \
+            ops.wino_ksplit(self.B, x.H, x.W, x.t.shape[3], 32) > 1
+        om = None if om_split else self.buf(x.H, x.W, 32)
+        om_raw = None
         if uom is not None:
-            self.add_wino(conv + ".conv_offset_mask", 2 * x.H * x.W * 27 * x.C * 9, x.t, wom, uom, som, hom, om.t, 32, ops.ACT_NONE)
+            om_raw = self.add_wino(conv + ".conv_offset_mask", 2 * x.H * x.W * 27 * x.C * 9, x.t, wom, uom, som, hom,
+                                   None if om_split else om.t, 32, ops.ACT_NONE, raw_ok=om_split)
+            assert (om_raw is not None) == om_split
         else:
             self.add("conv", conv + ".conv_offset_mask", 2 * x.H * x.W * 27 * x.C * 9,
                      ops.conv2d_launch([x.t], wom, som, hom, om.t, kh=3, kw=3, stride=1, pad=1, cout=32))
+        omt, om_fold = (om.t, None) if om_raw is None else (om_raw[1], (som, hom))
         flops = 2 * x.H * x.W * co * x.C * 9
         S = ops.dcn_ksplit(ops.rule_batch(self.B) * x.H * x.W, wp.shape[0]) if self.dcn_splitk else 1
         if S > 1:
@@ -297,19 +306,36 @@
             ws = self.pool.take(S * self.B * x.H * x.W * ldw)
             wst = ws[: S * self.B * x.H * x.W * ldw].view(S, self.B * x.H * x.W, ldw)
             ones, zeros = self.unit_scale(ldw)
-            self.add("dcn", conv, flops, ops.dcn_v2_launch(x.t, om.t, wp, ones, zeros, wst, cout=ldw, om_sigmoid=True, ksplit=S))
+            self.add("dcn", conv, flops, ops.dcn_v2_launch(x.t, omt, wp, ones, zeros, wst, cout=ldw, om_sigmoid=True, ksplit=S, om_fold=om_fold))
+            if om_raw is not None:
+                self.pool.give(om_raw[0])
+            if out is None:
+                out = Act(x.H, x.W, co)
+                out.raw = (wst, sc, sh, ops.ACT_RELU)
+                weakref.finalize(out, self.pool.give, ws)
+                return out
             self.add("sum", conv + ".splitk", 0, ops.splitk_reduce_launch(wst, sc, sh, out.t, cout=out.t.shape[3], act=ops.ACT_RELU))
             self.pool.give(ws)
             return out
+        if out is None:
+            out = self.buf(x.H, x.W, co)
         self.add("dcn", conv, flops,
-                 ops.dcn_v2_launch(x.t, om.t, wp, sc, sh, out.t, cout=out.t.shape[3], om_sigmoid=True, act=ops.ACT_RELU))
+                 ops.dcn_v2_launch(x.t, omt, wp, sc, sh, out.t, cout=out.t.shape[3], om_sigmoid=True, act=ops.ACT_RELU, om_fold=om_fold))
+        if om_raw is not None:
+            self.pool.give(om_raw[0])
         return out
 
     def emit_up_add(self, x, wname, f, add):
         out = self.buf(x.H * f, x.W * f, x.C)
         wk = ops.pack_dw_deconv_weight(self.w(wname + ".weight"))
-        if wk.shape[1] != x.t.shape[3]:
-            wk = torch.cat([wk, wk.new_zeros((wk.shape[0], x.t.shape[3] - wk.shape[1]))], 1).contiguous()
+        cp = ops.round_up(x.C, 16) if x.raw is not None else x.t.shape[3]
+        if wk.shape[1] != cp:
+            wk = torch.cat([wk, wk.new_zeros((wk.shape[0], cp - wk.shape[1]))], 1).contiguous()
+        if x.raw is not None:
+            wst, sc, sh, act = x.raw
+            self.add("up", wname, 2 * out.H * out.W * x.C * 4,
+                     ops.dw_deconv_add_split_launch(wst, sc, sh, act, wk, add.t, out.t, f, B=self.B, H=x.H, W=x.W, C=cp))
+            return out
         self.add("up", wname, 2 * out.H * out.W * x.C * 4, ops.dw_deconv_add_launch(x.t, wk, add.t, out.t, f))
         return out
 
@@ -499,7 +525,7 @@
 
     def __init__(self, arch, state_dict, batch, height=512, width=512, device="cuda", head_conv=None,
                  sigmoid_heads=True, use_graph=True, decode_k=None, const_cache=None, sched_cache=None, dets_only=False,
-                 flip_test=False):
+                 flip_test=False, dcn_fold=None):
         if dets_only and not decode_k:
             raise ValueError("dets_only=True needs decode_k: the sparse heads are evaluated at the peaks of the plan's own decode")
         if flip_test:
@@ -526,7 +552,7 @@
                 raise ValueError("parameter %s has shape %s, expected %s" % (k, tuple(sd[k].shape), shp))
         with torch.cuda.device(self.device):
             self.input = torch.zeros((batch, 3, height, width), dtype=torch.float32, device=self.device)
-            pb = PlanBuilder(sd, batch, self.device, sigmoid_heads, const_cache, dets_only=bool(dets_only))
+            pb = PlanBuilder(sd, batch, self.device, sigmoid_heads, const_cache, dets_only=bool(dets_only), dcn_fold=dcn_fold)
             pb.network(self.arch, Act(height, width, 3, self.input), head_conv)
         self.launches = pb.launches
         self.emission = pb.launches
diff --git a/centerpose_amd/nets.py b/centerpose_amd/nets.py
--- a/centerpose_amd/nets.py
+++ b/centerpose_amd/nets.py
@@ -8,11 +8,12 @@
 
 
 class Act:
-    __slots__ = ("H", "W", "C", "t", "split", "parent", "__weakref__")
+    __slots__ = ("H", "W", "C", "t", "split", "parent", "raw", "__weakref__")
 
     def __init__(self, H, W, C, t=None, split=None, parent=None):
         self.H, self.W, self.C, self.t, self.split = H, W, C, t, split
         self.parent = parent
+        self.raw = None
 
 
 class Graph:
@@ -44,7 +45,7 @@
     def emit_conv_batch(self, members):
         return [self.emit_conv([x], conv, bn, False, co, k, stride, pad, relu, None, False) for x, conv, bn, co, k, stride, pad, relu in members]
 
-    def emit_dcn(self, x, conv, bn, co):
+    def emit_dcn(self, x, conv, bn, co, raw_ok=False):
         return Act(x.H, x.W, co)
 
     def emit_up_add(self, x, wname, f, add):
@@ -87,14 +88,14 @@
         self.flops += 2 * out.H * out.W * co * ci * k * k
         return out
 
-    def deform(self, x, name, co):
-        return self.dcn_bn_relu(x, name + ".conv", name + ".actf.0", co)
-
-    def dcn_bn_relu(self, x, conv, bn, co):
+    def deform(self, x, name, co, raw_ok=False):
+        return self.dcn_bn_relu(x, name + ".conv", name + ".actf.0", co, raw_ok)
+
+    def dcn_bn_relu(self, x, conv, bn, co, raw_ok=False):
         self.p_bn(bn, co)
         self.p_conv(conv, co, x.C, 3, True)
         self.p_conv(conv + ".conv_offset_mask", 27, x.C, 3, True)
-        out = self.emit_dcn(x, conv, bn, co)
+        out = self.emit_dcn(x, conv, bn, co, raw_ok) if raw_ok else self.emit_dcn(x, conv, bn, co)
         self.flops += 2 * x.H * x.W * x.C * 9 * (27 + co)
         return out
 
@@ -165,7 +166,7 @@
         for i in range(startp + 1, endp):
             j = i - startp
             f = 2 if up_f is None else up_f[j]
-            t = self.deform(layers[i], "%s.proj_%d" % (p, j), o)
+            t = self.deform(layers[i], "%s.proj_%d" % (p, j), o, raw_ok=(f == 2))
             u = self.up_add(t, "%s.up_%d" % (p, j), f, layers[i - 1])
             layers[i] = self.deform(u, "%s.node_%d" % (p, j), o)
 
diff --git a/centerpose_amd/ops.py b/centerpose_amd/ops.py
--- a/centerpose_amd/ops.py
+++ b/centerpose_amd/ops.py
@@ -19,7 +19,7 @@
 class DcnDesc(ctypes.Structure):
     _fields_ = [(n, ctypes.c_int) for n in ("B", "H", "W", "C", "srcLd", "Ho", "Wo", "kh", "kw", "sy", "sx", "py", "px",
                                             "dily", "dilx", "K", "ldw", "Cout", "omLd", "omSigmoid", "outLd",
-                                            "outNCHW", "act", "tile", "ksplit", "dg")]
+                                            "outNCHW", "act", "tile", "ksplit", "dg", "omSplit", "omSlice")]
 
 
 def round_up(x, m):
@@ -63,8 +63,10 @@
     if fn == "cp_conv2d_f32":
         srcs = (ctypes.c_void_p * 4)(*[p.value for p in ptrs[:4]])
         return [d, srcs] + ptrs[4:]
-    if fn in ("cp_conv3x3_winograd_f32", "cp_dcn_v2_f32"):
+    if fn in ("cp_conv3x3_winograd_f32", "cp_dcn_v2_f32", "cp_dcn_v2_fold_f32"):
         return [d] + ptrs
+    if fn == "cp_dw_deconv_add_split_nhwc_f32":
+        return [ptrs[0], ints[0], ints[1], ptrs[1], ptrs[2], ints[2], ptrs[3], ptrs[4], ints[3], ptrs[5]] + ints[4:]
     if fn == "cp_conv3x3_winograd24_group_f32":
         arr = lambda k: (ctypes.c_void_p * 4)(*[p.value for p in ptrs[4 * k:4 * k + 4]])
         return [d, ints[0]] + [arr(k) for k in range(6)]
@@ -118,7 +120,7 @@
           "cp_global_avgpool_nhwc_f32": 9, "cp_scale_add_nhwc_f32": 10, "cp_shuffle_concat_nhwc_f32": 11, "cp_head3x3_1x1_f32": 12,
           "cp_decode_topk_f32": 13, "cp_decode_assign_f32": 14, "cp_splitk_reduce_f32": 15, "cp_conv3x3_winograd24_group_f32": 16, "cp_conv2d_group_f32": 17,
           "cp_sum_up_group_nhwc_f32": 18, "cp_head_points_f32": 19,
-          "cp_flip_merge_pairs_f32": 20}
+          "cp_flip_merge_pairs_f32": 20, "cp_dcn_v2_fold_f32": 21, "cp_dw_deconv_add_split_nhwc_f32": 22}
 
 
 def pad_rows(t, ldw):
@@ -392,17 +394,23 @@
 
 
 def dcn_v2_launch(x, om, wp, scale, shift, out, *, cout, kh=3, kw=3, stride=1, pad=1, dil=1, om_sigmoid=True,
-                  act=ACT_NONE, out_nchw=False, tile=0, ksplit=0, dg=1):
+                  act=ACT_NONE, out_nchw=False, tile=0, ksplit=0, dg=1, om_fold=None):
     B, H, W, C = x.shape
     d = DcnDesc()
     (sy, sx), (py, px), (dy, dx) = _pair(stride), _pair(pad), _pair(dil)
     Ho = (H + 2 * py - (dy * (kh - 1) + 1)) // sy + 1
     Wo = (W + 2 * px - (dx * (kw - 1) + 1)) // sx + 1
-    assert om.shape[:3] == (B, Ho, Wo)
+    if om_fold is None:
+        assert om.shape[:3] == (B, Ho, Wo)
+    else:
+        assert om.dim() == 3 and om.is_contiguous() and om.shape[0] > 1 and om.shape[1] == B * Ho * Wo
+        assert all(v.numel() >= 3 * dg * kh * kw for v in om_fold)
     d.B, d.H, d.W, d.C, d.srcLd, d.Ho, d.Wo = B, H, W, C, _ld(x), Ho, Wo
     d.kh, d.kw, d.sy, d.sx, d.py, d.px, d.dily, d.dilx = kh, kw, sy, sx, py, px, dy, dx
     d.K, d.ldw, d.Cout = wp.shape[1], wp.shape[0], cout
-    d.omLd, d.omSigmoid = _ld(om), 1 if om_sigmoid else 0
+    d.omLd, d.omSigmoid = (om.shape[2] if om_fold is not None else _ld(om)), 1 if om_sigmoid else 0
+    if om_fold is not None:
+        d.omSplit, d.omSlice = om.shape[0], om.shape[1] * om.shape[2]
     d.outNCHW = 1 if out_nchw else 0
     d.act, d.tile, d.ksplit, d.dg = act, tile, ksplit, dg
     if ksplit > 1:
@@ -410,7 +418,13 @@
         d.outLd = wp.shape[0]
     else:
         d.outLd = 0 if out_nchw else _ld(out)
+    if om_fold is not None:
+        return Launch("cp_dcn_v2_fold_f32", d, [x, om, om_fold[0], om_fold[1], wp, scale, shift, out])
     return Launch("cp_dcn_v2_f32", d, [x, om, wp, scale, shift, out])
+
+
+def dcn_fold_split_default():
+    return bool(_lib.lib().cp_dcn_fold_split_default())
 
 
 def wino_ksplit(B, H, W, cin, cout):
@@ -467,6 +481,13 @@
     assert wk.is_contiguous()
     return Launch("cp_dw_deconv_add_nhwc_f32", None, [x, wk, add, out],
                   [_ld(x), _ld(add) if add is not None else 0, _ld(out), B, H, W, C, f])
+
+
+def dw_deconv_add_split_launch(ws, scale, shift, act, wk, add, out, f, *, B, H, W, C):
+    S, M, ldw = ws.shape
+    assert ws.is_contiguous() and wk.is_contiguous() and M == B * H * W and C <= ldw and scale.numel() >= C and shift.numel() >= C
+    return Launch("cp_dw_deconv_add_split_nhwc_f32", None, [ws, scale, shift, wk, add, out],
+                  [ldw, S, act, _ld(add) if add is not None else 0, _ld(out), B, H, W, C, f])
 
 
 def dw_deconv_add(x, wk, add, out, f):
diff --git a/centerpose_amd/plan.py b/centerpose_amd/plan.py
--- a/centerpose_amd/plan.py
+++ b/centerpose_amd/plan.py
@@ -27,6 +27,7 @@
 REF_NULL, REF_BUF, REF_CONST = 0, 1, 2
 FN_NAMES = {v: k for k, v in ops.FN_IDS.items()}
 DESC_TYPES = {"cp_conv2d_f32": ops.ConvDesc, "cp_conv3x3_winograd_f32": ops.ConvDesc, "cp_dcn_v2_f32": ops.DcnDesc,
+              "cp_dcn_v2_fold_f32": ops.DcnDesc,
               "cp_conv3x3_winograd24_group_f32": ops.ConvDesc4, "cp_conv2d_group_f32": ops.ConvDesc8,
               "cp_head3x3_1x1_f32": ops.ConvDesc}
 
diff --git a/include/centerpose_hip.h b/include/centerpose_hip.h
--- a/include/centerpose_hip.h
+++ b/include/centerpose_hip.h
@@ -63,9 +63,14 @@
     int tile;
     int ksplit;
     int dg;
+    int omSplit;
+    int omSlice;
 } cp_dcn_desc;
 int cp_dcn_v2_f32(const cp_dcn_desc* d, const float* x, const float* om, const float* w, const float* scale,
                   const float* shift, float* out, void* stream);
+int cp_dcn_v2_fold_f32(const cp_dcn_desc* d, const float* x, const float* om, const float* omScale, const float* omShift,
+                       const float* w, const float* scale, const float* shift, float* out, void* stream);
+int cp_dcn_fold_split_default(void);
 int cp_dcn_pack_weights_f32(const float* w, const float* bias, int Co, int C, int kh, int kw, int dg, int Cp, int ldw, float* wp,
                             float* scale, float* shift, void* stream);
 int cp_sizeof_conv_desc(void);
@@ -81,6 +86,9 @@
                           void* stream);
 int cp_dw_deconv_add_nhwc_f32(const float* in, int inLd, const float* w, const float* add, int addLd, float* out, int outLd,
                               int B, int H, int W, int C, int f, void* stream);
+int cp_dw_deconv_add_split_nhwc_f32(const float* ws, int wsLd, int splits, const float* scale, const float* shift, int act,
+                                    const float* w, const float* add, int addLd, float* out, int outLd, int B, int H, int W, int C, int f,
+                                    void* stream);
 int cp_sum_up_nhwc_f32(int n, const float* const* src, const int* ld, const int* shift, float* out, int outLd, int B, int H,
                        int W, int C, int relu, void* stream);
 int cp_sum_up_group_nhwc_f32(int n, const float* const* src, const int* meta, float* const* out, int relu, void* stream);
```

Result: slower. 2214 (-1.0%).
